# sdmiller/cpu_tsdf

Measured on AMD Instinct MI355X. Metric: integrateCloud throughput, Scene A turntable depth frames, 640x480 -> voxel grid, higher is better.
Workload: dtype f32

## Files before the change

cpu_tsdf_amd/csrc/tsdf_buffer.h:

```cpp
#pragma once

#include <hip/hip_runtime.h>
#include <stdint.h>

typedef __amdgpu_buffer_rsrc_t rsrc_t;
typedef unsigned u4 __attribute__((ext_vector_type(4)));

#ifndef TSDF_STREAM_LD_AUX
#define TSDF_STREAM_LD_AUX 2
#endif
#ifndef TSDF_STREAM_ST_AUX
#define TSDF_STREAM_ST_AUX 2
#endif

static __device__ __forceinline__ rsrc_t make_rsrc(const void *p, unsigned bytes) {
  return __builtin_amdgcn_make_buffer_rsrc(const_cast<void *>(p), (short)0, (int)bytes, 0x00020000);
}
static __device__ __forceinline__ uint32_t bload32(rsrc_t r, unsigned voff, unsigned soff) {
  return __builtin_amdgcn_raw_buffer_load_b32(r, (int)voff, (int)soff, 0);
}
static __device__ __forceinline__ u4 bload128(rsrc_t r, unsigned voff, unsigned soff) {
  return __builtin_amdgcn_raw_buffer_load_b128(r, (int)voff, (int)soff, TSDF_STREAM_LD_AUX);
}
static __device__ __forceinline__ void bstore32(rsrc_t r, unsigned voff, unsigned soff, uint32_t v) {
  __builtin_amdgcn_raw_buffer_store_b32(v, r, (int)voff, (int)soff, TSDF_STREAM_ST_AUX);
}
static __device__ __forceinline__ uint32_t bload8(rsrc_t r, unsigned voff, unsigned soff) {
  return (uint32_t)__builtin_amdgcn_raw_buffer_load_b8(r, (int)voff, (int)soff, 0) & 0xffu;
}
static __device__ __forceinline__ void bstore128(rsrc_t r, unsigned voff, unsigned soff, u4 v) {
  __builtin_amdgcn_raw_buffer_store_b128(v, r, (int)voff, (int)soff, TSDF_STREAM_ST_AUX);
}

typedef int i4_rsrc __attribute__((ext_vector_type(4)));
__device__ unsigned tsdf_struct_buffer_load_u32(i4_rsrc rsrc, int vindex, int voffset, int soffset, int aux)
    __asm("llvm.amdgcn.struct.buffer.load.i32");

static __device__ __forceinline__ i4_rsrc make_rsrc_2d(const void *p, unsigned row_bytes, unsigned rows) {
  const unsigned long long a = (unsigned long long)p;
  i4_rsrc r;
  r.x = (int)(a & 0xffffffffull);
  r.y = (int)(((a >> 32) & 0xffffull) | ((unsigned long long)(row_bytes & 0x3fffu) << 16));
  r.z = (int)rows;
  r.w = 0x00020000;
  return r;
}
```

cpu_tsdf_amd/csrc/tsdf_common.h:

```cpp
#pragma once

#include <hip/hip_runtime.h>
#include <stdint.h>
#include <cmath>
#include <string>
#include <vector>

#include "tsdf_hip.h"

struct tsdf_hip_pipeline;
struct tsdf_hip_multi;
struct tsdf_occ_state;
struct tsdf_meshpost_state;
struct tsdf_flatten_state;
struct tsdf_esdf_state;

struct tsdf_hip_volume {
  tsdf_hip_multi *multi = nullptr;
  tsdf_params p;
  int device = 0;
  int nx = 0, ny = 0, nz = 0;
  int z_begin = 0, z_end = 0;
  int z_first = 0;
  int nz_alloc = 0;
  int64_t pitch = 0;
  int levels[3] = {0, 0, 0};
  float *d = nullptr, *w = nullptr;
  uint32_t *rgb = nullptr;
  uint8_t *k8 = nullptr;
  float *cn[4] = {nullptr, nullptr, nullptr, nullptr};
  float *lab_lut = nullptr;
  float4 *lab_img = nullptr;
  float *vm = nullptr;
  int32_t *vn = nullptr;
  int expf_fused_r = 0;
  float alloc_probe_ms[8] = {-1.f, -1.f, -1.f, -1.f, -1.f, -1.f, -1.f, -1.f};
  int alloc_tried = 0, alloc_chosen = 0;
  int packed = 0;
  unsigned kmax = 0;
  int weight_by_depth = 0, weight_by_variance = 0;
  float *ctr[3] = {nullptr, nullptr, nullptr};
  std::vector<float> h_ctr[3];
  float *frame_depth = nullptr;
  uint32_t *frame_bgra = nullptr;
  char *bounce = nullptr;
  hipEvent_t bounce_ev[2] = {nullptr, nullptr};
  bool bounce_busy[2] = {false, false};
  unsigned bounce_turn = 0;
  double *cam64 = nullptr;
  tsdf_hip_pipeline *pipe = nullptr;
  int frame_staged = 0;
  uint8_t *band = nullptr;
  int band_fx = 0, band_fy = 0;
  bool band_exact = false;
  int rest_state = 0;
  uint32_t rest_bits = 0;
  unsigned long long last_implied = 0, last_read_bytes = 0;
  bool last_implied_on = false;
  uint8_t *live = nullptr;
  size_t live_cap = 0;
  uint32_t *row_iv = nullptr;
  size_t row_iv_cap = 0;
  bool ctr_increasing[3] = {false, false, false};
  unsigned long long *counter = nullptr;
  unsigned long long last_observed = 0, last_changed_bytes = 0;
  bool ref_cull = false;
  float cull_planes[24] = {0};
  int last_launch[4] = {0, 0, 0, 0};
  bool pair_pending = false;
  bool pair_fused = false;
  unsigned long long pair_first_observed = 0, pair_first_changed = 0, pair_first_implied = 0, pair_first_read = 0;
  int count_slots = 0;
  bool count_ran = false;
  hipStream_t stream = nullptr;
  float *mc_verts = nullptr;
  uint8_t *mc_rgb = nullptr;
  uint64_t *mc_cell = nullptr;
  uint64_t mc_ntri = 0;
  bool mc_valid = false;
  size_t mc_cap = 0;
  bool mc_has_rgb = false;
  uint64_t *mc_keys = nullptr, *mc_vals = nullptr;
  size_t mc_cells_cap = 0;
  uint8_t *mc_need = nullptr;
  size_t mc_need_cap = 0;
  hipEvent_t mc_ev[4] = {nullptr, nullptr, nullptr, nullptr};
  float mc_ms[3] = {0.f, 0.f, 0.f};
  uint64_t mc_ncells = 0;
  uint64_t mc_d_bytes = 0;
  bool mc_skipped = false;
  bool mc_counts_pass = false;
  bool mc_halo_vouched = false;
  hipEvent_t align_ev[2] = {nullptr, nullptr};
  uint64_t align_stats[4] = {0, 0, 0, 0};
  hipEvent_t shift_ev[2] = {nullptr, nullptr};
  bool shift_timed = false;
  uint64_t shift_stats[3] = {0, 0, 0};
  hipEvent_t merge_ev[3] = {nullptr, nullptr, nullptr};
  bool merge_timed = false;
  unsigned long long *merge_count = nullptr;
  uint64_t merge_stats[3] = {0, 0, 0};
  bool merge_count_pending = false;
  void *scratch = nullptr;
  size_t scratch_bytes = 0;
  tsdf_occ_state *occ = nullptr;
  tsdf_meshpost_state *mp = nullptr;
  tsdf_flatten_state *fl = nullptr;
  tsdf_esdf_state *esdf = nullptr;
};

void tsdf_multi_free(tsdf_hip_volume *v);
int tsdf_multi_reset(tsdf_handle h);
int tsdf_multi_synchronize(tsdf_handle h);
int tsdf_multi_set_weighting(tsdf_handle h, int by_depth, int by_variance);
int tsdf_multi_set_reference_cull(tsdf_handle h, const float planes[24]);
int tsdf_multi_variance_block(tsdf_handle h, bool down, int x0, int y0, int z0, int nx, int ny, int nz, float *M, int32_t *nsample);
int tsdf_multi_integrate(tsdf_handle h, const float *depth, const uint8_t *bgra, const float T[12], uint64_t *n_observed,
                         bool asynchronous);
int tsdf_multi_integrate_device(tsdf_handle h, const float *d_depth, const uint32_t *d_bgra, const float T[12],
                                uint64_t *n_observed);
int tsdf_multi_organize(tsdf_handle h, const float *xyz, size_t xyz_stride, const uint8_t *bgra, size_t bgra_stride, size_t n,
                        float cloud_units, int zero_nans, const double world_to_cam[12], float *depth_out, uint8_t *bgra_out,
                        uint64_t *n_valid);
int tsdf_multi_integrate_staged(tsdf_handle h, const float T[12], uint64_t *n_observed);
int tsdf_multi_last_count_detail(tsdf_handle h, uint64_t out[2]);
int tsdf_multi_last_read_detail(tsdf_handle h, uint64_t out[3]);
int tsdf_multi_block(tsdf_handle h, bool down, int x0, int y0, int z0, int nx, int ny, int nz, float *d, float *w, uint8_t *rgb);
int tsdf_multi_sample(tsdf_handle h, const float *xyz, size_t n, float *val, float *grad, float *hess, uint8_t *ok);
int tsdf_multi_align_system(tsdf_handle h, const float *xyz, size_t n, const double vol_from_src[12], float min_weight, float r_max,
                            double out[29], uint8_t *used, float *xyz_vol);
int tsdf_multi_lookup_rgb(tsdf_handle h, const float *xyz, size_t n, uint8_t *rgb, uint8_t *found);
int tsdf_multi_raycast(tsdf_handle h, const float rot[9], const float origin[3], int downsample, const double *inv, float *out);
int tsdf_multi_march(tsdf_handle h, float w_min, int color_mode, uint64_t *n_tri);
int tsdf_multi_march_fetch(tsdf_handle h, float *verts, uint8_t *rgb, uint64_t *cell);
int tsdf_multi_march_timing(tsdf_handle h, float ms[3], uint64_t *n_cells);
int tsdf_multi_march_stats(tsdf_handle h, uint64_t out[4]);
tsdf_handle tsdf_multi_first(tsdf_handle h);
tsdf_handle tsdf_multi_slab(tsdf_handle h, int k);
int tsdf_multi_march_cleanup(tsdf_handle h, float face_dist, int min_neighbors, uint64_t *n_tri);
void tsdf_multi_mesh(tsdf_handle h, const float **verts, const uint8_t **rgb, const uint64_t **cell);
int tsdf_multi_flush(tsdf_handle h);
int tsdf_multi_set_frame_pairing(tsdf_handle h, int on);
int tsdf_multi_shift(tsdf_handle h, const int32_t shift[3]);
int tsdf_multi_integrate_device2(tsdf_handle h, const float *da, const uint32_t *ca, const float TA[12], const float *planes_a, const float *db,
                                 const uint32_t *cb, const float TB[12], const float *planes_b, uint64_t *n_observed, int32_t *fused);
#define TSDF_NOT_ON_MULTI(h, what)                                                                          \
  do {                                                                                                      \
    if ((h) && (h)->multi) {                                                                                \
      tsdf_set_error(what " works on ONE slab handle; this handle is a multi-GPU set (tsdf_hip_create_multi)"); \
      return TSDF_HIP_E_UNSUPPORTED;                                                                        \
    }                                                                                                       \
  } while (0)

int tsdf_integrate_launch(tsdf_handle h, const float *d_depth, const uint32_t *d_bgra, const float T[12], bool count);
int tsdf_integrate_collect(tsdf_handle h, uint64_t *n_observed);
int tsdf_integrate_launch2(tsdf_handle h, const float *dA, const uint32_t *cA, const float TA[12], const float *planesA,
                           const float *dB, const uint32_t *cB, const float TB[12], const float *planesB, bool count, bool *fused);
int tsdf_integrate_collect2(tsdf_handle h, uint64_t n_observed[2]);

#define TSDF_MAX_SLABS 64
#define TSDF_RAY_FIN_INTS 9
unsigned tsdf_ray_list_share(int64_t n_rays, int rank, int world);
int tsdf_ray_list_begin(tsdf_handle s, const float rot[9], const float origin[3], int downsample, int rank, int world,
                        int32_t *d_list, unsigned *count);
int tsdf_ray_list_advance(tsdf_handle s, const float rot[9], const float origin[3], int downsample, int rank, int world,
                          int32_t *d_list, unsigned count, unsigned *d_incomplete);
int tsdf_ray_list_route(tsdf_handle s, const int32_t *d_list, unsigned count, int n_slab, const int *z_end,
                        unsigned *d_counters, int32_t *d_outbox, int32_t *d_finbox);
int tsdf_ray_deliver(tsdf_handle s, const int32_t *d_fin, unsigned count, float *d_out, int64_t n_pix, const double *inv);

void tsdf_set_error(const std::string &msg);
int tsdf_hip_fail(hipError_t e, const char *what, const char *file, int line);

#define TSDF_HIP_TRY(expr)                                              \
  do {                                                                  \
    hipError_t _e = (expr);                                             \
    if (_e != hipSuccess) return tsdf_hip_fail(_e, #expr, __FILE__, __LINE__); \
  } while (0)

struct TsdfDeviceScope {
  int prev = -1;
  hipError_t err;
  explicit TsdfDeviceScope(int dev) {
    err = hipGetDevice(&prev);
    if (err != hipSuccess || prev == dev)
      prev = -1;
    else
      err = hipSetDevice(dev);
  }
  ~TsdfDeviceScope() {
    if (prev >= 0) (void)hipSetDevice(prev);
  }
  TsdfDeviceScope(const TsdfDeviceScope &) = delete;
  TsdfDeviceScope &operator=(const TsdfDeviceScope &) = delete;
};
#define TSDF_ON_DEVICE(dev)          \
  TsdfDeviceScope _device_scope(dev); \
  TSDF_HIP_TRY(_device_scope.err)
int tsdf_pipeline_flush(tsdf_hip_volume *v);
#define TSDF_ENTER(h)                                  \
  TSDF_ON_DEVICE((h)->device);                         \
  if ((h)->pair_pending) {                             \
    const int _rc_flush = tsdf_pipeline_flush(h);      \
    if (_rc_flush) return _rc_flush;                   \
  }

void tsdf_build_centers(int res, float size, std::vector<float> &out, int *levels);
static inline void tsdf_lab_curve(float lut[256]) {
  for (int v = 0; v < 256; ++v) {
    float f = ((float)v / 255.);
    if (f > 0.0405)
      f = std::pow(((f + 0.055) / 1.055), 2.4);
    else
      f /= 12.92;
    f *= 100;
    lut[v] = f;
  }
}

static inline uint8_t tsdf_u8_of_float(float v) {
  const int i = (v > -2147483904.f && v < 2147483648.f) ? (int)v : (int)0x80000000;
  return (uint8_t)(i & 255);
}
static inline uint32_t tsdf_lab2rgb_host(float L, float A, float B) {
  float Y = (L + 16) / 116.;
  float X = A / 500. + Y;
  float Z = Y - (B / 200.);
  if (std::pow((double)X, 3.0) > 0.008856) X = std::pow((double)X, 3.0); else X = (X - 16 / 116.) / 7.787;
  if (std::pow((double)Y, 3.0) > 0.008856) Y = std::pow((double)Y, 3.0); else Y = (Y - 16 / 116.) / 7.787;
  if (std::pow((double)Z, 3.0) > 0.008856) Z = std::pow((double)Z, 3.0); else Z = (Z - 16 / 116.) / 7.787;
  X *= 95.047;
  Y *= 100.;
  Z *= 108.883;
  X /= 100;
  Y /= 100;
  Z /= 100;
  float rf = X * +3.2406 + Y * -1.5372 + Z * -0.4986;
  float gf = X * -0.9689 + Y * +1.8758 + Z * +0.0415;
  float bf = X * +0.0557 + Y * -0.2040 + Z * +1.0570;
  if (rf > 0.0031308) rf = 1.055 * std::pow(static_cast<double>(rf), 1. / 2.4) - 0.055; else rf *= 12.92;
  if (gf > 0.0031308) gf = 1.055 * std::pow(static_cast<double>(gf), 1. / 2.4) - 0.055; else gf *= 12.92;
  if (bf > 0.0031308) bf = 1.055 * std::pow(static_cast<double>(bf), 1. / 2.4) - 0.055; else bf *= 12.92;
  return (uint32_t)tsdf_u8_of_float(rf * 255) | ((uint32_t)tsdf_u8_of_float(gf * 255) << 8) | ((uint32_t)tsdf_u8_of_float(bf * 255) << 16);
}
void tsdf_lab2rgb_host_many(const float *L, const float *A, const float *B, size_t n, uint32_t *out);
int tsdf_lab_exact_colors(tsdf_hip_volume *v, const int64_t *d_idx, size_t n, uint32_t *host_rgb, bool write_plane);

static inline float tsdf_node_size(const tsdf_params &p, int axis) {
  const int r = p.res[0];
  const bool cubic_pow2 = r > 0 && (r & (r - 1)) == 0 && p.res[1] == r && p.res[2] == r;
  return cubic_pow2 ? p.size[0] : p.size[axis];
}
static inline float tsdf_voxel_edge(const tsdf_params &p) { return p.size[0] / p.res[0]; }
int tsdf_ensure_scratch(tsdf_hip_volume *v, size_t bytes);
int tsdf_to_host(tsdf_hip_volume *v, void *dst, const void *dev_src, size_t bytes);
int tsdf_to_device(tsdf_hip_volume *v, void *dev_dst, const void *src, size_t bytes);
bool tsdf_is_pinned_host(const void *p);
void tsdf_pipeline_destroy(tsdf_hip_volume *v);
void tsdf_occupied_release(tsdf_hip_volume *v);
void tsdf_meshpost_release(tsdf_hip_volume *v);
void tsdf_flatten_release(tsdf_hip_volume *v);
void tsdf_flatten_invalidate(tsdf_hip_volume *v);
void tsdf_occupied_invalidate(tsdf_hip_volume *v);
void tsdf_esdf_release(tsdf_hip_volume *v);
void tsdf_esdf_drop(tsdf_hip_volume *v);
void tsdf_esdf_invalidate(tsdf_hip_volume *v);
int tsdf_shift_planes(tsdf_hip_volume *v, int sx, int sy, int sz, int dz0, int dz1);
int tsdf_shift_band(tsdf_hip_volume *v, int sx, int sy, int sz);
int tsdf_shift_mark(tsdf_hip_volume *v, int which);
void tsdf_shift_clamp(const tsdf_hip_volume *v, const int32_t shift[3], int s[3]);
void tsdf_shift_count(int nx, int ny, int nz, const int s[3], uint64_t *kept, uint64_t *reset);

struct TsdfTuning {
  int rows_per_block;
  int blocks_per_cu;
  int fast_projection;
  int mc_flush_at;
  int mc_skip;
  int cull;
  int vol_chunk;
  int plain_kernel;
  int alloc_tries;
  int allin;
  int refcull_plain;
  int live_log2tx;
  int zfast;
  int fuse2;
  int implied_d;
  int pipe;
  int lab_chunk;
};
const TsdfTuning &tsdf_tuning();
int tsdf_vol_chunk();

struct PlaneView {
  const float *d, *w;
  const uint32_t *rgb;
  const uint8_t *k8;
  float wmax;
  unsigned kmax;
  int packed;
};

static inline PlaneView tsdf_plane_view(const tsdf_hip_volume *v) {
  return PlaneView{v->d, v->w, v->rgb, v->k8, v->p.max_weight, v->kmax, v->packed};
}

static __device__ __forceinline__ float tsdf_decode_w(unsigned k, float wmax) {
  const float kf = (float)k;
  return kf > wmax ? wmax : kf;
}

static __device__ __forceinline__ bool tsdf_encode_w(float w, float wmax, unsigned kmax, unsigned &k) {
  if (w == wmax) {
    k = kmax;
    return true;
  }
  if (w >= 0.f && w < (float)kmax && w == floorf(w)) {
    k = (unsigned)w;
    return true;
  }
  k = 0;
  return false;
}

static __device__ __forceinline__ float tsdf_load_w(const PlaneView &v, int64_t i) {
  if (!v.packed) return v.w[i];
  const unsigned k = v.rgb ? (v.rgb[i] >> 24) : (unsigned)v.k8[i];
  return tsdf_decode_w(k, v.wmax);
}

static __device__ __forceinline__ uint32_t tsdf_load_rgb(const PlaneView &v, int64_t i) {
  return v.rgb[i] & 0xffffffu;
}

static inline __host__ __device__ int64_t tsdf_index(int64_t pitch, int ny, int z_first, int x, int y,
                                                      int zg) {
  return ((int64_t)(zg - z_first) * ny + y) * pitch + x;
}
```

cpu_tsdf_amd/csrc/tsdf_core.hip:

```cpp
#include <math.h>

#include <string>
#include <stdlib.h>
#include <stdio.h>

#include <algorithm>
#include <thread>
#include <string.h>

#include "tsdf_common.h"
#ifdef TSDF_HIP_TEST_HOOKS
#include "tsdf_hip_test.h"
#endif

static thread_local std::string g_last_error;

void tsdf_set_error(const std::string &msg) { g_last_error = msg; }

int tsdf_hip_fail(hipError_t e, const char *what, const char *file, int line) {
  char buf[512];
  snprintf(buf, sizeof buf, "%s:%d: %s -> %s", file, line, what, hipGetErrorString(e));
  g_last_error = buf;
  (void)hipGetLastError();
  return e == hipErrorOutOfMemory ? TSDF_HIP_E_NOMEM : TSDF_HIP_E_HIP;
}

extern "C" const char *tsdf_hip_last_error(void) { return g_last_error.c_str(); }

extern "C" const char *tsdf_hip_error_string(int code) {
  switch (code) {
    case TSDF_HIP_OK: return "ok";
    case TSDF_HIP_E_INVALID: return "invalid argument";
    case TSDF_HIP_E_NOMEM: return "out of device memory";
    case TSDF_HIP_E_HIP: return "HIP runtime error";
    case TSDF_HIP_E_NODEVICE: return "no HIP device";
    case TSDF_HIP_E_UNSUPPORTED: return "unsupported";
    case TSDF_HIP_E_IO: return "file error";
    case TSDF_HIP_ALIGN_NO_POINTS: return "alignment: no point passed the gate";
    case TSDF_HIP_ALIGN_RANK_DEFICIENT: return "alignment: the cloud does not constrain all six freedoms";
  }
  return "unknown";
}

static int env_int(const char *name, int dflt) {
  const char *e = getenv(name);
  return (e && *e) ? atoi(e) : dflt;
}

static TsdfTuning &tuning_storage() {
  static TsdfTuning t = {std::max(1, env_int("TSDF_HIP_ROWS_PER_BLOCK", 64)),
                         std::max(1, env_int("TSDF_HIP_BLOCKS_PER_CU", 8)),
                         env_int("TSDF_HIP_FAST_PROJECTION", -1), env_int("TSDF_HIP_MC_FLUSH_AT", 512), env_int("TSDF_HIP_MC_SKIP", 1),
                         env_int("TSDF_HIP_CULL", 1), std::max(1, env_int("TSDF_HIP_VOL_CHUNK", 256)),
                         env_int("TSDF_HIP_PLAIN_KERNEL", 0), env_int("TSDF_HIP_ALLOC_TRIES", 3), env_int("TSDF_HIP_ALLIN", 1),
                         env_int("TSDF_HIP_REFCULL_PLAIN", 0), env_int("TSDF_HIP_LIVE_LOG2TX", 5), env_int("TSDF_HIP_ZFAST", 1), env_int("TSDF_HIP_FUSE2", 1), env_int("TSDF_HIP_IMPLIED_D", 1),
                         env_int("TSDF_HIP_PIPE", 1), std::max(1, env_int("TSDF_HIP_LAB_CHUNK", 16 << 20))};
  return t;
}

const TsdfTuning &tsdf_tuning() { return tuning_storage(); }

int tsdf_vol_chunk() {
  const int live = env_int("TSDF_HIP_VOL_CHUNK", 0);
  return live > 0 ? live : tsdf_tuning().vol_chunk;
}

#ifdef TSDF_HIP_TEST_HOOKS
extern "C" int tsdf_hip_set_tuning(const char *name, int value) {
  if (!name) return TSDF_HIP_E_INVALID;
  TsdfTuning &t = tuning_storage();
  const std::string n(name);
  if (n == "rows_per_block")
    t.rows_per_block = std::max(1, value);
  else if (n == "blocks_per_cu")
    t.blocks_per_cu = std::max(1, value);
  else if (n == "fast_projection")
    t.fast_projection = value;
  else if (n == "mc_flush_at")
    t.mc_flush_at = value;
  else if (n == "mc_skip")
    t.mc_skip = value;
  else if (n == "cull")
    t.cull = value;
  else if (n == "vol_chunk")
    t.vol_chunk = std::max(1, value);
  else if (n == "plain_kernel")
    t.plain_kernel = value;
  else if (n == "alloc_tries")
    t.alloc_tries = std::max(1, value);
  else if (n == "allin")
    t.allin = value;
  else if (n == "refcull_plain")
    t.refcull_plain = value;
  else if (n == "fuse2")
    t.fuse2 = value;
  else if (n == "implied_d")
    t.implied_d = value;
  else if (n == "pipe")
    t.pipe = value;
  else if (n == "live_log2tx")
    t.live_log2tx = value;
  else if (n == "zfast")
    t.zfast = value;
  else if (n == "lab_chunk")
    t.lab_chunk = std::max(1, value);
  else
    return TSDF_HIP_E_INVALID;
  return TSDF_HIP_OK;
}
#endif

extern "C" int tsdf_hip_abi_version(void) { return TSDF_HIP_ABI_VERSION; }

extern "C" int tsdf_hip_host_alloc(size_t bytes, void **out) {
  if (!out || !bytes) return TSDF_HIP_E_INVALID;
  *out = nullptr;
  TSDF_HIP_TRY(hipHostMalloc(out, bytes, hipHostMallocPortable));
  return TSDF_HIP_OK;
}

extern "C" int tsdf_hip_host_free(void *p) {
  if (!p) return TSDF_HIP_OK;
  TSDF_HIP_TRY(hipHostFree(p));
  return TSDF_HIP_OK;
}

extern "C" int tsdf_hip_device_count(void) {
  int n = 0;
  if (hipGetDeviceCount(&n) != hipSuccess) {
    (void)hipGetLastError();
    return 0;
  }
  return n;
}

extern "C" void tsdf_hip_default_params(tsdf_params *p) {
  memset(p, 0, sizeof *p);
  p->res[0] = p->res[1] = p->res[2] = 512;
  p->size[0] = p->size[1] = p->size[2] = 3.0f;
  p->max_dist_pos = 0.03f;
  p->max_dist_neg = 0.03f;
  p->max_weight = 100.f;
  p->min_sensor_dist = 0.3f;
  p->max_sensor_dist = 3.0f;
  p->fx = p->fy = 525.;
  p->cx = 320;
  p->cy = 240;
  p->image_width = 640;
  p->image_height = 480;
  p->integrate_color = 0;
  p->xform_order = TSDF_XFORM_PCL_SSE;
  p->z_begin = p->z_end = 0;
  p->halo = 0;
  p->device = -1;
  p->layout = TSDF_LAYOUT_AUTO;
  p->color_mode = TSDF_COLOR_RGB;
}

static int ilog2_exact(int v) {
  if (v <= 0 || (v & (v - 1))) return -1;
  int l = 0;
  while ((1 << l) < v) ++l;
  return l;
}

void tsdf_build_centers(int res, float size, std::vector<float> &out, int *levels) {
  out.resize(res);
  const int L = ilog2_exact(res);
  *levels = L;
  if (L >= 0) {
    for (int i = 0; i < res; ++i) {
      float c = 0.f;
      float s = size;
      for (int l = L - 1; l >= 0; --l) {
        const float off = s / 4;
        c = ((i >> l) & 1) ? c + off : c - off;
        s = s / 2;
      }
      out[i] = c;
    }
  } else {
    const float off = size / 2.0;
    for (int i = 0; i < res; ++i) out[i] = (float)((i + 0.5) * size / (double)res - off);
  }
}

static __global__ void __launch_bounds__(256)
k_fill_u32(uint32_t *__restrict__ p, uint32_t value, int64_t n4 ) {
  const uint4 v4 = make_uint4(value, value, value, value);
  uint4 *q = reinterpret_cast<uint4 *>(p);
  for (int64_t i = (int64_t)blockIdx.x * blockDim.x + threadIdx.x; i < n4;
       i += (int64_t)gridDim.x * blockDim.x)
    q[i] = v4;
}

static int fill_u32(tsdf_hip_volume *v, void *p, uint32_t value, int64_t n) {
  const int64_t n4 = n / 4;
  int64_t blocks = (n4 + 255) / 256;
  if (blocks > 256 * 16) blocks = 256 * 16;
  if (blocks < 1) blocks = 1;
  hipLaunchKernelGGL(k_fill_u32, dim3((unsigned)blocks), dim3(256), 0, v->stream, (uint32_t *)p, value, n4);
  TSDF_HIP_TRY(hipGetLastError());
  return TSDF_HIP_OK;
}

int tsdf_ensure_scratch(tsdf_hip_volume *v, size_t bytes) {
  if (bytes <= v->scratch_bytes) return TSDF_HIP_OK;
  if (v->scratch) {
    TSDF_HIP_TRY(hipStreamSynchronize(v->stream));
    TSDF_HIP_TRY(hipFree(v->scratch));
    v->scratch = nullptr;
    v->scratch_bytes = 0;
  }
  TSDF_HIP_TRY(hipMalloc(&v->scratch, bytes));
  v->scratch_bytes = bytes;
  return TSDF_HIP_OK;
}

void tsdf_lab2rgb_host_many(const float *L, const float *A, const float *B, size_t n, uint32_t *out) {
  const unsigned hw = std::max(1u, std::min(64u, std::thread::hardware_concurrency()));
  const unsigned nt = n < 4096 ? 1u : hw;
  auto work = [&](size_t lo, size_t hi) {
    for (size_t i = lo; i < hi; ++i) out[i] = tsdf_lab2rgb_host(L[i], A[i], B[i]);
  };
  if (nt == 1) return work(0, n);
  std::vector<std::thread> th;
  for (unsigned t = 0; t < nt; ++t) th.emplace_back(work, n * t / nt, n * (t + 1) / nt);
  for (auto &t : th) t.join();
}

static __global__ void __launch_bounds__(256)
k_lab_gather(const int64_t *__restrict__ idx, size_t n, const float *__restrict__ L, const float *__restrict__ A,
             const float *__restrict__ B, float *__restrict__ out) {
  const size_t i = (size_t)blockIdx.x * blockDim.x + threadIdx.x;
  if (i >= n) return;
  const int64_t v = idx[i];
  out[i] = v >= 0 ? L[v] : 0.f;
  out[n + i] = v >= 0 ? A[v] : 0.f;
  out[2 * n + i] = v >= 0 ? B[v] : 0.f;
}

static __global__ void __launch_bounds__(256)
k_rgb_scatter(const int64_t *__restrict__ idx, size_t n, const uint32_t *__restrict__ words, uint32_t *__restrict__ plane) {
  const size_t i = (size_t)blockIdx.x * blockDim.x + threadIdx.x;
  if (i >= n) return;
  const int64_t v = idx[i];
  if (v >= 0) plane[v] = (plane[v] & 0xff000000u) | (words[i] & 0xffffffu);
}

int tsdf_lab_exact_colors(tsdf_hip_volume *v, const int64_t *d_idx, size_t n, uint32_t *host_rgb, bool write_plane) {
  if (!n) return TSDF_HIP_OK;
  if (!v->lab_img || !v->cn[0] || !v->cn[1] || !v->cn[2]) return TSDF_HIP_E_INVALID;
  const size_t chunk = (size_t)tsdf_tuning().lab_chunk;
  float *d_lab = nullptr;
  uint32_t *d_words = nullptr;
  const size_t m = std::min(n, chunk);
  TSDF_HIP_TRY(hipMalloc(&d_lab, m * 3 * sizeof(float)));
  if (write_plane && hipMalloc(&d_words, m * sizeof(uint32_t)) != hipSuccess) {
    (void)hipFree(d_lab);
    return tsdf_hip_fail(hipErrorOutOfMemory, "hipMalloc", __FILE__, __LINE__);
  }
  std::vector<float> lab(m * 3);
  std::vector<uint32_t> words(m);
  int rc = TSDF_HIP_OK;
  for (size_t off = 0; off < n && !rc; off += chunk) {
    const size_t c = std::min(chunk, n - off);
    hipLaunchKernelGGL(k_lab_gather, dim3((unsigned)((c + 255) / 256)), dim3(256), 0, v->stream, d_idx + off, c, v->cn[0], v->cn[1],
                       v->cn[2], d_lab);
    if ((rc = tsdf_to_host(v, lab.data(), d_lab, c * 3 * sizeof(float)))) break;
    tsdf_lab2rgb_host_many(lab.data(), lab.data() + c, lab.data() + 2 * c, c, words.data());
    if (host_rgb) memcpy(host_rgb + off, words.data(), c * sizeof(uint32_t));
    if (write_plane) {
      if ((rc = tsdf_to_device(v, d_words, words.data(), c * sizeof(uint32_t)))) break;
      hipLaunchKernelGGL(k_rgb_scatter, dim3((unsigned)((c + 255) / 256)), dim3(256), 0, v->stream, d_idx + off, c, d_words, v->rgb);
      if (hipStreamSynchronize(v->stream) != hipSuccess) rc = TSDF_HIP_E_HIP;
    }
  }
  (void)hipFree(d_lab);
  if (d_words) (void)hipFree(d_words);
  return rc;
}

static const size_t kBounceChunk = 2u << 20;

static int bounce_ready(tsdf_hip_volume *v) {
  if (!v->bounce) {
    TSDF_HIP_TRY(hipHostMalloc((void **)&v->bounce, 2 * kBounceChunk, hipHostMallocDefault));
    for (int i = 0; i < 2; ++i) TSDF_HIP_TRY(hipEventCreateWithFlags(&v->bounce_ev[i], hipEventDisableTiming));
  }
  return TSDF_HIP_OK;
}

static int bounce_wait(tsdf_hip_volume *v, int slot) {
  if (v->bounce_busy[slot]) {
    TSDF_HIP_TRY(hipEventSynchronize(v->bounce_ev[slot]));
    v->bounce_busy[slot] = false;
  }
  return TSDF_HIP_OK;
}

bool tsdf_is_pinned_host(const void *p) {
  hipPointerAttribute_t attr;
  if (hipPointerGetAttributes(&attr, p) != hipSuccess) {
    (void)hipGetLastError();
    return false;
  }
  return attr.type == hipMemoryTypeHost;
}

int tsdf_to_host(tsdf_hip_volume *v, void *dst, const void *dev_src, size_t bytes) {
  if (!bytes) return TSDF_HIP_OK;
  if (bytes >= (64u << 10) && tsdf_is_pinned_host(dst)) {
    TSDF_HIP_TRY(hipMemcpyAsync(dst, dev_src, bytes, hipMemcpyDeviceToHost, v->stream));
    TSDF_HIP_TRY(hipStreamSynchronize(v->stream));
    return TSDF_HIP_OK;
  }
  int rc = bounce_ready(v);
  if (rc) return rc;
  const size_t chunks = (bytes + kBounceChunk - 1) / kBounceChunk;
  const unsigned turn = v->bounce_turn;
  v->bounce_turn += (unsigned)chunks;
  for (size_t k = 0; k <= chunks; ++k) {
    if (k < chunks) {
      const int slot = (int)((turn + k) & 1);
      if ((rc = bounce_wait(v, slot))) return rc;
      const size_t off = k * kBounceChunk, len = std::min(kBounceChunk, bytes - off);
      TSDF_HIP_TRY(hipMemcpyAsync(v->bounce + slot * kBounceChunk, (const char *)dev_src + off, len, hipMemcpyDeviceToHost,
                                  v->stream));
      TSDF_HIP_TRY(hipEventRecord(v->bounce_ev[slot], v->stream));
      v->bounce_busy[slot] = true;
    }
    if (k > 0) {
      const int slot = (int)((turn + k - 1) & 1);
      if ((rc = bounce_wait(v, slot))) return rc;
      const size_t off = (k - 1) * kBounceChunk, len = std::min(kBounceChunk, bytes - off);
      memcpy((char *)dst + off, v->bounce + slot * kBounceChunk, len);
    }
  }
  return TSDF_HIP_OK;
}

int tsdf_to_device(tsdf_hip_volume *v, void *dev_dst, const void *src, size_t bytes) {
  if (!bytes) return TSDF_HIP_OK;
  if (bytes >= (64u << 10) && tsdf_is_pinned_host(src)) {
    TSDF_HIP_TRY(hipMemcpyAsync(dev_dst, src, bytes, hipMemcpyHostToDevice, v->stream));
    TSDF_HIP_TRY(hipStreamSynchronize(v->stream));
    return TSDF_HIP_OK;
  }
  int rc = bounce_ready(v);
  if (rc) return rc;
  const size_t chunks = (bytes + kBounceChunk - 1) / kBounceChunk;
  const unsigned turn = v->bounce_turn;
  v->bounce_turn += (unsigned)chunks;
  for (size_t k = 0; k < chunks; ++k) {
    const int slot = (int)((turn + k) & 1);
    if ((rc = bounce_wait(v, slot))) return rc;
    const size_t off = k * kBounceChunk, len = std::min(kBounceChunk, bytes - off);
    memcpy(v->bounce + slot * kBounceChunk, (const char *)src + off, len);
    TSDF_HIP_TRY(hipMemcpyAsync((char *)dev_dst + off, v->bounce + slot * kBounceChunk, len, hipMemcpyHostToDevice, v->stream));
    TSDF_HIP_TRY(hipEventRecord(v->bounce_ev[slot], v->stream));
    v->bounce_busy[slot] = true;
  }
  return TSDF_HIP_OK;
}

static void free_volume(tsdf_hip_volume *v) {
  if (!v) return;
  tsdf_occupied_release(v);
  tsdf_meshpost_release(v);
  tsdf_flatten_release(v);
  tsdf_esdf_release(v);
  if (v->multi) tsdf_multi_free(v);
  TsdfDeviceScope scope(v->device);
  tsdf_pipeline_destroy(v);
  if (v->d) (void)hipFree(v->d);
  if (v->w) (void)hipFree(v->w);
  if (v->rgb) (void)hipFree(v->rgb);
  if (v->k8) (void)hipFree(v->k8);
  for (int c = 0; c < 4; ++c)
    if (v->cn[c]) (void)hipFree(v->cn[c]);
  if (v->vm) (void)hipFree(v->vm);
  if (v->vn) (void)hipFree(v->vn);
  if (v->lab_lut) (void)hipFree(v->lab_lut);
  if (v->lab_img) (void)hipFree(v->lab_img);
  for (int a = 0; a < 3; ++a)
    if (v->ctr[a]) (void)hipFree(v->ctr[a]);
  if (v->frame_depth) (void)hipFree(v->frame_depth);
  if (v->bounce) (void)hipHostFree(v->bounce);
  for (int i = 0; i < 2; ++i)
    if (v->bounce_ev[i]) (void)hipEventDestroy(v->bounce_ev[i]);
  if (v->cam64) (void)hipFree(v->cam64);
  if (v->live) (void)hipFree(v->live);
  if (v->row_iv) (void)hipFree(v->row_iv);
  if (v->band) (void)hipFree(v->band);
  if (v->counter) (void)hipFree(v->counter);
  if (v->mc_verts) (void)hipFree(v->mc_verts);
  if (v->mc_rgb) (void)hipFree(v->mc_rgb);
  if (v->mc_cell) (void)hipFree(v->mc_cell);
  if (v->mc_keys) (void)hipFree(v->mc_keys);
  if (v->mc_vals) (void)hipFree(v->mc_vals);
  if (v->mc_need) (void)hipFree(v->mc_need);
  for (int i = 0; i < 4; ++i)
    if (v->mc_ev[i]) (void)hipEventDestroy(v->mc_ev[i]);
  for (int i = 0; i < 2; ++i)
    if (v->align_ev[i]) (void)hipEventDestroy(v->align_ev[i]);
  for (int i = 0; i < 2; ++i)
    if (v->shift_ev[i]) (void)hipEventDestroy(v->shift_ev[i]);
  for (int i = 0; i < 3; ++i)
    if (v->merge_ev[i]) (void)hipEventDestroy(v->merge_ev[i]);
  if (v->merge_count) (void)hipFree(v->merge_count);
  if (v->scratch) (void)hipFree(v->scratch);
  delete v;
}

struct PlaneSet {
  float *d = nullptr, *w = nullptr;
  uint32_t *rgb = nullptr;
  uint8_t *k8 = nullptr;
};

static __global__ void __launch_bounds__(256)
k_probe_rmw(uint4 *__restrict__ a, uint4 *__restrict__ b, uint4 *__restrict__ c, int64_t n4, unsigned zero) {
  typedef unsigned v4u __attribute__((ext_vector_type(4)));
  v4u *pa = reinterpret_cast<v4u *>(a), *pb = reinterpret_cast<v4u *>(b), *pc = reinterpret_cast<v4u *>(c);
  for (int64_t i = (int64_t)blockIdx.x * blockDim.x + threadIdx.x; i < n4; i += (int64_t)gridDim.x * blockDim.x) {
    v4u x = __builtin_nontemporal_load(pa + i);
    x ^= zero;
    __builtin_nontemporal_store(x, pa + i);
    if (b) {
      v4u y = __builtin_nontemporal_load(pb + i);
      y ^= zero;
      __builtin_nontemporal_store(y, pb + i);
    }
    if (c) {
      v4u z = __builtin_nontemporal_load(pc + i);
      z ^= zero;
      __builtin_nontemporal_store(z, pc + i);
    }
  }
}

static void release_planes(PlaneSet &s) {
  if (s.d) (void)hipFree(s.d);
  if (s.w) (void)hipFree(s.w);
  if (s.rgb) (void)hipFree(s.rgb);
  if (s.k8) (void)hipFree(s.k8);
  s = PlaneSet();
}

static float probe_planes(const PlaneSet &s, int64_t n, hipStream_t stream) {
  hipEvent_t e0 = nullptr, e1 = nullptr;
  if (hipEventCreate(&e0) != hipSuccess || hipEventCreate(&e1) != hipSuccess) return -1.f;
  float ms = -1.f;
  const int64_t n4 = n / 4;
  const unsigned grid = 256u * (unsigned)tsdf_tuning().blocks_per_cu;
  bool ok = true;
  for (int pass = 0; pass < 2 && ok; ++pass) {
    ok &= hipEventRecord(e0, stream) == hipSuccess;
    hipLaunchKernelGGL(k_probe_rmw, dim3(grid), dim3(256), 0, stream, (uint4 *)s.d, (uint4 *)s.w, (uint4 *)s.rgb, n4, 0u);
    ok &= hipGetLastError() == hipSuccess;
    ok &= hipEventRecord(e1, stream) == hipSuccess;
    ok &= hipEventSynchronize(e1) == hipSuccess;
    if (ok) ok &= hipEventElapsedTime(&ms, e0, e1) == hipSuccess;
  }
  (void)hipEventDestroy(e0);
  (void)hipEventDestroy(e1);
  return ok ? ms : -1.f;
}

extern "C" int tsdf_hip_reference_cull_is_noop(const tsdf_params *p) {
  if (!p || !(p->fx > 0.0) || !(p->fy > 0.0) || p->image_width <= 0 || p->image_height <= 0) return 0;
  if (!(p->max_sensor_dist > 0.f) || !(p->max_sensor_dist < 1e15f)) return 0;
  const double W = p->image_width, H = p->image_height;
  const double th = tan(1.1 * atan(0.5 * W / p->fx)) * (1.0 - 1e-5), tv = tan(1.1 * atan(0.5 * H / p->fy)) * (1.0 - 1e-5);
  if (!(th > 0.0) || !(tv > 0.0)) return 0;
  return (p->cx + 1.0) / p->fx <= th && (W - p->cx) / p->fx <= th && (p->cy + 1.0) / p->fy <= tv && (H - p->cy) / p->fy <= tv;
}

extern "C" int tsdf_hip_reference_cull_planes(const tsdf_params *p, const double trans[16], float planes[24]) {
  if (!p || !trans || !planes) return TSDF_HIP_E_INVALID;
  struct V3 { float v[3]; };
  auto axis = [&](int col, float sign) { V3 o; for (int r = 0; r < 3; ++r) o.v[r] = sign * (float)trans[4 * r + col]; return o; };
  const V3 view = axis(2, 1.f), up = axis(1, -1.f), right = axis(0, 1.f), T = axis(3, 1.f);
  const float hfov = (float)(1.1 * 2 * fabs(atan((double)(0.5 * p->image_width / p->fx)) * 180 / M_PI));
  const float vfov = (float)(1.1 * 2 * fabs(atan((double)(0.5 * p->image_height / p->fy)) * 180 / M_PI));
  const float vrad = (float)(vfov * M_PI / 180), hrad = (float)(hfov * M_PI / 180);
  const float dist[2] = {p->max_sensor_dist, p->min_sensor_dist};
  V3 centre[2], corner[2][4];
  for (int f = 0; f < 2; ++f) {
    const float hgt = (float)(2 * tan((double)(vrad / 2)) * dist[f]), wid = (float)(2 * tan((double)(hrad / 2)) * dist[f]);
    for (int i = 0; i < 3; ++i) {
      const float c = T.v[i] + view.v[i] * dist[f], u = up.v[i] * hgt / 2, r = right.v[i] * wid / 2;
      centre[f].v[i] = c;
      corner[f][0].v[i] = c + u - r;
      corner[f][1].v[i] = c + u + r;
      corner[f][2].v[i] = c - u - r;
      corner[f][3].v[i] = c - u + r;
    }
  }
  auto minus = [](const V3 &a, const V3 &b) { V3 o; for (int i = 0; i < 3; ++i) o.v[i] = a.v[i] - b.v[i]; return o; };
  auto put = [&](int k, const V3 &e1, const V3 &e2, const V3 &through) {
    const float n[3] = {e1.v[1] * e2.v[2] - e1.v[2] * e2.v[1], e1.v[2] * e2.v[0] - e1.v[0] * e2.v[2], e1.v[0] * e2.v[1] - e1.v[1] * e2.v[0]};
    planes[4 * k] = n[0], planes[4 * k + 1] = n[1], planes[4 * k + 2] = n[2];
    planes[4 * k + 3] = -(through.v[0] * n[0] + (through.v[1] * n[1] + through.v[2] * n[2]));
  };
  const V3 a = minus(corner[0][2], T), b = minus(corner[0][3], T), c = minus(corner[0][1], T), d = minus(corner[0][0], T);
  put(0, d, a, T);
  put(1, b, c, T);
  put(2, c, d, T);
  put(3, a, b, T);
  put(4, minus(corner[0][2], corner[0][3]), minus(corner[0][1], corner[0][3]), centre[0]);
  put(5, minus(corner[1][1], corner[1][3]), minus(corner[1][2], corner[1][3]), centre[1]);
  return TSDF_HIP_OK;
}

extern "C" int tsdf_hip_create(const tsdf_params *p, tsdf_handle *out) {
  if (!p || !out) return TSDF_HIP_E_INVALID;
  *out = nullptr;
  for (int a = 0; a < 3; ++a)
    if (p->res[a] <= 0 || !(p->size[a] > 0.f)) {
      tsdf_set_error("resolution and grid size must be positive");
      return TSDF_HIP_E_INVALID;
    }
  if (p->image_width <= 0 || p->image_height <= 0 || !(p->max_dist_neg > 0.f) || p->halo < 0 ||
      (p->xform_order != TSDF_XFORM_PCL_SSE && p->xform_order != TSDF_XFORM_LEFT_TO_RIGHT) ||
      p->layout < TSDF_LAYOUT_AUTO || p->layout > TSDF_LAYOUT_PACKED ||
      p->color_mode < TSDF_COLOR_RGB || p->color_mode > TSDF_COLOR_LAB) {
    tsdf_set_error("bad image size / truncation / halo / xform_order / layout / color_mode");
    return TSDF_HIP_E_INVALID;
  }
  const bool lab = p->integrate_color && p->color_mode == TSDF_COLOR_LAB;
  const bool rgbn = (p->integrate_color && p->color_mode == TSDF_COLOR_RGB_NORMALIZED) || lab;
  if (rgbn && p->layout == TSDF_LAYOUT_PACKED) {
    tsdf_set_error("RGB_NORMALIZED / LAB colour keeps float weights: no PACKED layout");
    return TSDF_HIP_E_UNSUPPORTED;
  }
  const bool packable = !rgbn && p->max_weight >= 0.f && p->max_weight <= 255.f;
  if (p->layout == TSDF_LAYOUT_PACKED && !packable) {
    tsdf_set_error("the PACKED layout needs 0 <= max_weight <= 255");
    return TSDF_HIP_E_UNSUPPORTED;
  }
  int zb = p->z_begin, ze = p->z_end;
  if (zb == 0 && ze == 0) ze = p->res[2];
  if (zb < 0 || ze > p->res[2] || zb >= ze) {
    tsdf_set_error("z slab outside the grid");
    return TSDF_HIP_E_INVALID;
  }
  if (tsdf_hip_device_count() <= 0) {
    tsdf_set_error("no HIP device visible");
    return TSDF_HIP_E_NODEVICE;
  }
  int dev = p->device;
  if (dev < 0) TSDF_HIP_TRY(hipGetDevice(&dev));
  TSDF_ON_DEVICE(dev);

  tsdf_hip_volume *v = new tsdf_hip_volume;
  v->p = *p;
  v->p.z_begin = zb;
  v->p.z_end = ze;
  v->device = dev;
  v->nx = p->res[0];
  v->ny = p->res[1];
  v->nz = p->res[2];
  v->z_begin = zb;
  v->z_end = ze;
  v->z_first = zb - p->halo < 0 ? 0 : zb - p->halo;
  const int z_last = ze + p->halo > v->nz ? v->nz : ze + p->halo;
  v->nz_alloc = z_last - v->z_first;
  v->pitch = ((int64_t)v->nx + 3) / 4 * 4;
  const int64_t n = v->pitch * v->ny * v->nz_alloc;
  v->packed = p->layout == TSDF_LAYOUT_PACKED || (p->layout == TSDF_LAYOUT_AUTO && packable);
  v->p.layout = v->packed ? TSDF_LAYOUT_PACKED : TSDF_LAYOUT_F32W;
  v->kmax = v->packed ? (unsigned)ceilf(p->max_weight) : 0u;

  int rc = TSDF_HIP_OK;
  auto bail = [&](int code) {
    free_volume(v);
    return code;
  };
#define TRY_OR_BAIL(expr)                                                  \
  do {                                                                     \
    hipError_t _e = (expr);                                                \
    if (_e != hipSuccess) return bail(tsdf_hip_fail(_e, #expr, __FILE__, __LINE__)); \
  } while (0)
  auto alloc_planes = [&](PlaneSet &s) -> hipError_t {
    hipError_t e = hipMalloc(&s.d, n * sizeof(float));
    if (e == hipSuccess && !v->packed) e = hipMalloc(&s.w, n * sizeof(float));
    if (e == hipSuccess && p->integrate_color) e = hipMalloc(&s.rgb, n * sizeof(uint32_t));
    if (e == hipSuccess && v->packed && !p->integrate_color) e = hipMalloc(&s.k8, n);
    if (e != hipSuccess) release_planes(s);
    return e;
  };
  PlaneSet best;
  TRY_OR_BAIL(alloc_planes(best));
  {
    const size_t plane_bytes = (size_t)n * (4 + (v->packed ? 0 : 4) + (p->integrate_color ? 4 : 0) + (v->packed && !p->integrate_color ? 1 : 0));
    const int tries = plane_bytes >= ((size_t)4 << 30) ? std::max(1, tsdf_tuning().alloc_tries) : 1;
    float best_ms = tries > 1 ? probe_planes(best, n, v->stream) : -1.f;
    v->alloc_probe_ms[0] = best_ms;
    v->alloc_tried = 1;
    const double swept = (double)n * (4 + (v->packed ? 0 : 4) + (p->integrate_color ? 4 : 0));
    auto rate_tbps = [&](float ms) { return ms > 0.f ? 2.0 * swept / ((double)ms * 1e9) : 0.0; };
    for (int t = 1; t < std::min(8, 2 * tries) && best_ms > 0.f && tries > 1; ++t) {
      if (rate_tbps(best_ms) >= 5.55) break;
      if (t >= tries && rate_tbps(best_ms) >= 5.15) break;
      size_t free_b = 0, total_b = 0;
      if (hipMemGetInfo(&free_b, &total_b) != hipSuccess || free_b < plane_bytes + ((size_t)2 << 30)) break;
      PlaneSet cand;
      if (alloc_planes(cand) != hipSuccess) {
        (void)hipGetLastError();
        break;
      }
      const float ms = probe_planes(cand, n, v->stream);
      v->alloc_probe_ms[t < 8 ? t : 7] = ms;
      v->alloc_tried = t + 1;
      if (ms > 0.f && ms < best_ms) {
        release_planes(best);
        best = cand;
        best_ms = ms;
        v->alloc_chosen = t;
      } else {
        release_planes(cand);
      }
    }
  }
  v->d = best.d;
  v->w = best.w;
  v->rgb = best.rgb;
  v->k8 = best.k8;
  if (rgbn)
    for (int c = 0; c < (lab ? 3 : 4); ++c) TRY_OR_BAIL(hipMalloc(&v->cn[c], n * sizeof(float)));
  if (lab) {
    float lut[256];
    tsdf_lab_curve(lut);
    TRY_OR_BAIL(hipMalloc(&v->lab_lut, sizeof lut));
    TRY_OR_BAIL(hipMemcpy(v->lab_lut, lut, sizeof lut, hipMemcpyHostToDevice));
    TRY_OR_BAIL(hipMalloc(&v->lab_img, (size_t)p->image_width * p->image_height * sizeof(float4)));
  }
  for (int a = 0; a < 3; ++a) {
    tsdf_build_centers(p->res[a], tsdf_node_size(*p, a), v->h_ctr[a], &v->levels[a]);
    v->ctr_increasing[a] = true;
    for (size_t i = 1; i < v->h_ctr[a].size(); ++i) v->ctr_increasing[a] &= v->h_ctr[a][i - 1] < v->h_ctr[a][i];
    std::vector<float> padded(v->h_ctr[a]);
    padded.resize((size_t)p->res[a] + 4, NAN);
    TRY_OR_BAIL(hipMalloc(&v->ctr[a], padded.size() * sizeof(float)));
    TRY_OR_BAIL(hipMemcpy(v->ctr[a], padded.data(), padded.size() * sizeof(float), hipMemcpyHostToDevice));
  }
  const size_t npx = (size_t)p->image_width * p->image_height;
  TRY_OR_BAIL(hipMalloc(&v->frame_depth, 2 * npx * sizeof(float)));
  v->frame_bgra = reinterpret_cast<uint32_t *>(v->frame_depth + npx);
  {
    const double cam[4] = {p->fx, p->fy, p->cx, p->cy};
    TRY_OR_BAIL(hipMalloc(&v->cam64, sizeof cam));
    TRY_OR_BAIL(hipMemcpy(v->cam64, cam, sizeof cam, hipMemcpyHostToDevice));
  }
  v->band_fx = (v->nx + 63) / 64;
  v->band_fy = (v->ny + 3) / 4;
  TRY_OR_BAIL(hipMalloc(&v->band, (size_t)v->band_fx * v->band_fy * v->nz_alloc));
  TRY_OR_BAIL(hipMalloc(&v->counter, 4096 * sizeof(unsigned long long)));
  TRY_OR_BAIL(hipMemset(v->counter, 0, 4096 * sizeof(unsigned long long)));
#undef TRY_OR_BAIL
  rc = tsdf_hip_reset(v);
  if (rc != TSDF_HIP_OK) return bail(rc);
  *out = v;
  return TSDF_HIP_OK;
}

extern "C" int tsdf_hip_reset(tsdf_handle h) {
  if (!h) return TSDF_HIP_E_INVALID;
  if (h->multi) return tsdf_multi_reset(h);
  TSDF_ENTER(h);
  const int64_t n = h->pitch * h->ny * h->nz_alloc;
  const float minus_one = -1.f;
  uint32_t bits;
  memcpy(&bits, &minus_one, 4);
  int rc = fill_u32(h, h->d, bits, n);
  if (rc) return rc;
  if (h->w) rc = fill_u32(h, h->w, 0u, n);
  if (rc) return rc;
  if (h->k8) TSDF_HIP_TRY(hipMemsetAsync(h->k8, 0, (size_t)n, h->stream));
  if (h->rgb) rc = fill_u32(h, h->rgb, 0u, n);
  if (rc) return rc;
  for (int c = 0; c < 4 && !rc; ++c)
    if (h->cn[c]) rc = fill_u32(h, h->cn[c], 0u, n);
  if (rc) return rc;
  if (h->vm) rc = fill_u32(h, reinterpret_cast<float *>(h->vm), 0u, n);
  if (!rc && h->vn) rc = fill_u32(h, reinterpret_cast<float *>(h->vn), 0u, n);
  if (rc) return rc;
  TSDF_HIP_TRY(hipMemsetAsync(h->band, 0, (size_t)h->band_fx * h->band_fy * h->nz_alloc, h->stream));
  h->band_exact = true;
  h->rest_state = 0;
  h->frame_staged = 0;
  TSDF_HIP_TRY(hipStreamSynchronize(h->stream));
  tsdf_esdf_drop(h);
  return TSDF_HIP_OK;
}

extern "C" int tsdf_hip_destroy(tsdf_handle h) {
  if (!h) return TSDF_HIP_E_INVALID;
  TsdfDeviceScope scope(h->device);
  (void)hipStreamSynchronize(h->stream);
  free_volume(h);
  return TSDF_HIP_OK;
}

extern "C" int tsdf_hip_set_stream(tsdf_handle h, void *hip_stream) {
  if (!h) return TSDF_HIP_E_INVALID;
  TSDF_NOT_ON_MULTI(h, "tsdf_hip_set_stream (a stream belongs to one device)");
  {
    TSDF_ENTER(h);
  }
  h->stream = (hipStream_t)hip_stream;
  return TSDF_HIP_OK;
}

extern "C" int tsdf_hip_synchronize(tsdf_handle h) {
  if (!h) return TSDF_HIP_E_INVALID;
  if (h->multi) return tsdf_multi_synchronize(h);
  TSDF_ENTER(h);
  TSDF_HIP_TRY(hipStreamSynchronize(h->stream));
  return TSDF_HIP_OK;
}

extern "C" int tsdf_hip_centers(tsdf_handle h, int axis, float *out) {
  if (!h || axis < 0 || axis > 2 || !out) return TSDF_HIP_E_INVALID;
  memcpy(out, h->h_ctr[axis].data(), h->h_ctr[axis].size() * sizeof(float));
  return TSDF_HIP_OK;
}

extern "C" int tsdf_hip_alloc_probe(tsdf_handle h, float ms[8], int32_t *chosen) {
  if (!h) return 0;
  const tsdf_hip_volume *s = h->multi ? tsdf_multi_first(h) : h;
  if (ms)
    for (int i = 0; i < 8; ++i) ms[i] = s->alloc_probe_ms[i];
  if (chosen) *chosen = s->alloc_chosen;
  return s->alloc_tried;
}

extern "C" int tsdf_hip_layout(tsdf_handle h) {
  return !h ? -1 : (h->packed ? TSDF_LAYOUT_PACKED : TSDF_LAYOUT_F32W);
}

extern "C" int tsdf_hip_device_planes(tsdf_handle h, float **d, float **w, uint32_t **rgb, int64_t *pitch,
                                      int32_t *z_first, int32_t *nz_alloc) {
  if (!h) return TSDF_HIP_E_INVALID;
  TSDF_NOT_ON_MULTI(h, "tsdf_hip_device_planes");
  {
    TSDF_ENTER(h);
  }
  h->band_exact = false;
  if (d) *d = h->d;
  if (w) *w = h->w;
  if (rgb) *rgb = h->rgb;
  if (pitch) *pitch = h->pitch;
  if (z_first) *z_first = h->z_first;
  if (nz_alloc) *nz_alloc = h->nz_alloc;
  return TSDF_HIP_OK;
}

struct BlockArgs {
  int x0, y0, zl0;
  int bx, by, bz;
  int ny;
  int64_t pitch;
};

template <bool TO_BLOCK>
static __global__ void __launch_bounds__(256)
k_block_f32(BlockArgs a, float *__restrict__ vol, float *__restrict__ blk) {
  const int64_t n = (int64_t)a.bx * a.by * a.bz;
  for (int64_t i = (int64_t)blockIdx.x * blockDim.x + threadIdx.x; i < n; i += (int64_t)gridDim.x * blockDim.x) {
    const int x = (int)(i % a.bx);
    const int64_t r = i / a.bx;
    const int y = (int)(r % a.by);
    const int z = (int)(r / a.by);
    const int64_t vi = ((int64_t)(a.zl0 + z) * a.ny + (a.y0 + y)) * a.pitch + (a.x0 + x);
    if (TO_BLOCK)
      blk[i] = vol[vi];
    else
      vol[vi] = blk[i];
  }
}

template <bool TO_BLOCK>
static __global__ void __launch_bounds__(256)
k_block_w(BlockArgs a, PlaneView pv, float *__restrict__ blk, unsigned *__restrict__ bad) {
  const int64_t n = (int64_t)a.bx * a.by * a.bz;
  for (int64_t i = (int64_t)blockIdx.x * blockDim.x + threadIdx.x; i < n; i += (int64_t)gridDim.x * blockDim.x) {
    const int x = (int)(i % a.bx);
    const int64_t r = i / a.bx;
    const int y = (int)(r % a.by);
    const int z = (int)(r / a.by);
    const int64_t vi = ((int64_t)(a.zl0 + z) * a.ny + (a.y0 + y)) * a.pitch + (a.x0 + x);
    if (TO_BLOCK) {
      blk[i] = tsdf_load_w(pv, vi);
    } else if (!pv.packed) {
      const_cast<float *>(pv.w)[vi] = blk[i];
    } else {
      unsigned k;
      if (!tsdf_encode_w(blk[i], pv.wmax, pv.kmax, k)) {
        atomicAdd(bad, 1u);
      } else if (pv.rgb) {
        uint32_t *c = const_cast<uint32_t *>(pv.rgb) + vi;
// ... 360 lines not shown
```

cpu_tsdf_amd/csrc/tsdf_integrate.hip:

```cpp
#include <limits.h>
#include <string.h>
#include <math.h>

#include <algorithm>
#include <cmath>
#include <type_traits>

#include "tsdf_common.h"
#include "tsdf_div.h"
#include "tsdf_buffer.h"
#ifdef TSDF_HIP_TEST_HOOKS
#include "tsdf_hip_test.h"
#endif

#ifndef TSDF_WPE_MAX
#define TSDF_WPE_MAX 8
#endif
#ifndef TSDF_WPE_PACKED
#define TSDF_WPE_PACKED 7
#endif
#ifndef TSDF_WPE_PACKED_COLOR
#define TSDF_WPE_PACKED_COLOR 8
#endif
#ifndef TSDF_WPE_GENERAL
// ... 131 lines not shown
  if (abstop >= (0x42b00000u >> 20)) {
    if (ix == 0xff800000u) return 0.f;
    if (abstop >= (0x7f800000u >> 20)) return x + x;
    if (x > 0x1.62e42ep6f) return INFINITY;
    if (x < -0x1.9fe368p6f) return 0.f;
    if (x < -0x1.9d1d9ep6f) return 0x1p-149f;
  }
  const double N = 32., InvLn2N = 0x1.71547652b82fep+0 * N, SHIFT = 0x1.8p+52;
  const double C0 = 0x1.c6af84b912394p-5 / N / N / N, C1 = 0x1.ebfce50fac4f3p-3 / N / N, C2 = 0x1.62e42ff0c52d6p-1 / N;
  const double xd = (double)x;
  double z = InvLn2N * xd;
  double kd = z + SHIFT;
  const uint64_t ki = (uint64_t)__double_as_longlong(kd);
  kd -= SHIFT;
  const double r = fused_r ? __builtin_fma(InvLn2N, xd, -kd) : z - kd;
  const uint64_t t = k_exp2f_tab[ki & 31u] + (ki << 47);
  const double s = __longlong_as_double((long long)t);
  z = C0 * r + C1;
  const double r2 = r * r;
  double y = C2 * r + 1.;
  y = z * r2 + y;
  y = y * s;
  return (float)y;
}

static __device__ __forceinline__ bool reference_cull_keeps(const IntegrateArgs &a, float x, float y, float z) {
  bool keep = true;
#pragma unroll
  for (int k = 0; k < 6; ++k) {
    const float *pl = a.cull + 4 * k;
    keep = keep && ((x * pl[0] + y * pl[1]) + (z * pl[2] + 1.0f * pl[3]) <= 0.f);
  }
  return keep;
}

static __device__ __forceinline__ float div32_fast(float a, const Rcp32 &r) {
  const float q0 = a * r.y;
  const float r0 = __builtin_fmaf(r.nb, q0, a);
  const float q1 = __builtin_fmaf(r0, r.y, q0);
  const float r1 = __builtin_fmaf(r.nb, q1, a);
  return __builtin_fmaf(r1, r.y, q1);
}

static __device__ __forceinline__ bool numerator_ok(float v) {
  const float m = fabsf(v);
  return (m >= 0x1p-100f && m <= 0x1p40f) || __float_as_uint(v) == 0u;
}

template <bool COLOR>
static __device__ __forceinline__ void add_observation_ieee(float &d, float &w, uint32_t &rgb, float dn,
                                                            uint32_t bgra, float wmax) {
  const float wn = 1.f;
  const float wsum = w + wn;
  if (COLOR) {
    uint32_t out = 0;
#pragma unroll
    for (int ch = 0; ch < 3; ++ch) {
      const float c_old = (float)((rgb >> (8 * ch)) & 255u);
      const float c_new = (float)((bgra >> (16 - 8 * ch)) & 255u);
      const float num = w * c_old + wn * c_new;
      out |= ((uint32_t)(uint8_t)(num / wsum)) << (8 * ch);
    }
    rgb = out;
  }
  d = (d * w + dn * wn) / wsum;
  w = wsum;
  if (w > wmax) w = wmax;
}

template <bool COLOR, bool DIST = true>
static __device__ __forceinline__ void add_observation_fast(float &d, float &w, uint32_t &rgb, float dn,
                                                            uint32_t bgra, float wmax, const Rcp32 &rs, uint32_t base = 0u,
                                                            const float *hy_tab = nullptr) {
  const float wsum = w + 1.f;
  if (COLOR) {
    const float hy = hy_tab ? *hy_tab : __builtin_fmaf(0.5f, rs.y, -0.5f);
    const float t0 = __builtin_fmaf(__builtin_fmaf(w, (float)(rgb & 255u), (float)((bgra >> 16) & 255u)), rs.y, hy);
    const float t1 = __builtin_fmaf(__builtin_fmaf(w, (float)((rgb >> 8) & 255u), (float)((bgra >> 8) & 255u)), rs.y, hy);
    const float t2 = __builtin_fmaf(__builtin_fmaf(w, (float)((rgb >> 16) & 255u), (float)(bgra & 255u)), rs.y, hy);
    rgb = __builtin_amdgcn_cvt_pk_u8_f32(t0, 0u, __builtin_amdgcn_cvt_pk_u8_f32(t1, 1u, __builtin_amdgcn_cvt_pk_u8_f32(t2, 2u, base)));
  }
  if (DIST) d = div32_fast(d * w + dn, rs);
  w = wsum;
  if (w > wmax) w = wmax;
}

static __device__ __forceinline__ bool update_is_safe(float d, float w, float dn) {
  const bool w_ok = fabsf(w - 512.f) <= 512.f && __builtin_amdgcn_fractf(w) == 0.f;
  return w_ok && numerator_ok(d * w + dn);
}


struct BlockCoords {
  unsigned bx, by, bz, gdx, gdy;
};
static __device__ __forceinline__ BlockCoords tsdf_block_coords(int zfast) {
  BlockCoords c;
  c.by = blockIdx.y, c.gdy = gridDim.y;
  c.bx = zfast ? blockIdx.z : blockIdx.x;
  c.bz = zfast ? blockIdx.x : blockIdx.z;
  c.gdx = zfast ? gridDim.z : gridDim.x;
  return c;
}

static __device__ __forceinline__ void tsdf_flags_before(const IntegrateArgs &a, const BlockCoords &bc, const uint8_t *band,
                                                         uint8_t *s_bin, unsigned tid) {
  const int row0 = (int)bc.by * a.rpb * a.TY;
  const int rows = min(a.rpb * a.TY, a.ny - row0);
  const int lf = max(0, a.log2TX - 4), fxb = 1 << lf;
  const int yg0 = (a.y_abs0 + row0) >> 2, yg1 = (a.y_abs0 + row0 + max(rows, 1) - 1) >> 2;
  const int xc0 = (a.x_abs0 + (int)bc.bx * a.TX * 4) >> 6;
  const int n_fl = (yg1 - yg0 + 1) << lf;
  const int n_all = ((a.rpb * a.TY + 3) >> 2) << lf;
  for (int i = (int)tid; i < n_all; i += 256) {
    const int yg = yg0 + (i >> lf), xc = xc0 + (i & (fxb - 1));
    s_bin[i] = i < n_fl && yg < a.band_fy && xc < a.band_fx ? band[((int64_t)(a.zl0 + (int)bc.bz) * a.band_fy + yg) * a.band_fx + xc] : (uint8_t)0;
  }
}
static __device__ __forceinline__ uint64_t tsdf_quiet_passes(const IntegrateArgs &a, const uint8_t *s_bin, unsigned tid) {
  const int lane = (int)(tid & 63u), w0 = (int)(tid & ~63u);
  const int fxb = max(1, a.TX >> 4);
  const int rows_w = max(1, 64 >> a.log2TX), ncell = max(1, min(a.TX, 64) >> 4);
  const int ty0 = w0 >> a.log2TX, c0 = (w0 & (a.TX - 1)) >> 4;
  bool q = lane < a.rpb;
  if (q) {
    for (int rr = 0; rr < rows_w; ++rr)
      for (int c = 0; c < ncell; ++c) q &= s_bin[((ty0 + rr + lane * a.TY) >> 2) * fxb + c0 + c] == 0;
  }
  return __builtin_amdgcn_ballot_w64(q);
}

struct __attribute__((aligned(16))) KEntry {
  float w;
  float y;
  float hy;
  uint32_t k1;
};
static __device__ __forceinline__ KEntry tsdf_ktab_entry(const IntegrateArgs &a, unsigned k) {
  KEntry e;
  e.w = __builtin_fminf((float)k, a.wmax);
  e.y = rcp32_prepare((float)(k + 1u)).y;
  e.hy = __builtin_fmaf(0.5f, e.y, -0.5f);
  e.k1 = min(k << 24, a.kcap) + a.kinc;
  return e;
}
#define TSDF_BAND_DECL                                                                                     \
  __shared__ __attribute__((aligned(16))) uint8_t s_band_sets[4][1024];                                    \
  reinterpret_cast<u4 *>(&s_band_sets[0][0])[tid] = (u4){0u, 0u, 0u, 0u}
#define TSDF_BAND(i) s_band_sets[threadIdx.x >> 6][i]
#define TSDF_BAND_FIRST ((int)(tid & 63u))
#define TSDF_BAND_STEP 64
#define TSDF_WPE_OF(ORDER, COLOR, FASTPROJ, COUNT, PACKED, ALLIN) \
  ((ALLIN) && !(COUNT) && (PACKED) && (COLOR) && (FASTPROJ) ? TSDF_WPE_PACKED_COLOR : (ALLIN) && !(COUNT) && ((PACKED) || !(COLOR)) ? TSDF_WPE_PACKED : TSDF_WPE_GENERAL)
template <int ORDER, bool COLOR, bool FASTPROJ, bool COUNT, bool PACKED, bool ALLIN = false, bool LIVE = false>
static __global__ void __launch_bounds__(256) __attribute__((amdgpu_waves_per_eu(TSDF_WPE_OF(ORDER, COLOR, FASTPROJ, COUNT, PACKED, ALLIN) < TSDF_WPE_MAX ? TSDF_WPE_OF(ORDER, COLOR, FASTPROJ, COUNT, PACKED, ALLIN) : TSDF_WPE_MAX, TSDF_WPE_MAX)))
k_integrate(const IntegrateArgs a, float *__restrict__ D, float *__restrict__ Wt, uint32_t *__restrict__ RGB,
            uint8_t *__restrict__ K8, const float *__restrict__ depth, const double *__restrict__ cam,
            const float *__restrict__ ctrx, const float *__restrict__ ctry, const float *__restrict__ ctrz,
            unsigned long long *__restrict__ n_obs, const uint8_t *__restrict__ live, uint8_t *__restrict__ band,
            const uint32_t *__restrict__ row_iv) {
  static_assert(!(ALLIN && LIVE), "the ALLIN instance knows no row intervals");
  const BlockCoords bc = tsdf_block_coords(a.zfast);
  bool strad = false;
  if (LIVE) {
    const unsigned flag = live[bc.bx + bc.gdx * (bc.by + bc.gdy * bc.bz)];
    if (flag == 0u) return;
    strad = flag == 2u;
  }
  const unsigned tid = threadIdx.x;
  __shared__ f2 s_rcp[256];
  __shared__ f4 s_yt[256];
  constexpr bool F2 = ALLIN && FASTPROJ;
  constexpr bool LEAN_K1 = PACKED && COLOR;
  __shared__ f4 s_cx[F2 ? 256 : 1];
  __shared__ uint32_t s_iv[LIVE ? 256 : 1];
  TSDF_BAND_DECL;
  if (PACKED) {
    const KEntry e = tsdf_ktab_entry(a, tid);
    s_rcp[tid] = (f2){e.y, e.hy};
  }
  {
    const int yy = (int)bc.by * a.rpb * a.TY + (int)tid;
    {
      const float cy_ = ctry[yy < a.ny ? yy : a.ny - 1], cz_ = ctrz[a.z_global0 + (int)bc.bz];
      f4 t = {0.f, 0.f, 0.f, 0.f};
#pragma unroll
      for (int q = 0; q < 3; ++q)
        t[q] = ORDER == TSDF_XFORM_PCL_SSE ? cy_ * a.m[4 * q + 1] + (cz_ * a.m[4 * q + 2] + a.m[4 * q + 3]) : a.m[4 * q + 1] * cy_;
      s_yt[tid] = t;
    }
    if (F2) {
      const int xq_ = (int)bc.bx * a.TX + (int)(tid & (unsigned)(a.TX - 1));
      if (xq_ < a.qpr) s_cx[tid] = *reinterpret_cast<const f4 *>(ctrx + xq_ * 4);
    }
    if (LIVE && strad) s_iv[tid] = yy < a.ny ? row_iv[(int64_t)bc.bz * a.ny + yy] : 0u;
  }
  __shared__ uint8_t s_bin[PACKED ? 1024 : 1];
  if (PACKED && a.implied_d) tsdf_flags_before(a, bc, band, s_bin, tid);
  __syncthreads();
  const uint64_t quiet = PACKED && a.implied_d ? tsdf_quiet_passes(a, s_bin, tid) : 0ull;
  const int tx = (int)(tid & (unsigned)(a.TX - 1));
  const int ty = (int)(tid >> a.log2TX);
  const int xq = (int)bc.bx * a.TX + tx;
  const int zl = (int)bc.bz;
  const Rcp32 rneg = rcp32_prepare(a.neg);
  unsigned cnt = 0, chg = 0, imp = 0, rdb = 0;
  const int row0 = (int)bc.by * a.rpb * a.TY;
  const int rows = min(a.rpb * a.TY, a.ny - row0);
  const int64_t e0 = ((int64_t)(a.zl0 + zl) * a.plane_rows + row0) * a.pitch;
  const unsigned span = (unsigned)rows * (unsigned)a.pitch;
  const rsrc_t rsD = make_rsrc(D + e0, span * 4u);
  const rsrc_t rsW = make_rsrc(PACKED ? D : Wt + e0, PACKED ? 0u : span * 4u);
  const rsrc_t rsC = make_rsrc(COLOR ? RGB + e0 : (uint32_t *)D, COLOR ? span * 4u : 0u);
  const rsrc_t rsK = make_rsrc(PACKED && !COLOR ? K8 + e0 : (uint8_t *)D, PACKED && !COLOR ? span : 0u);
  const unsigned npix = (unsigned)a.W * (unsigned)a.H;
  const rsrc_t rsF = make_rsrc(depth, COLOR ? a.bgra_off + npix * 4u : npix * 4u);
  const i4_rsrc rsFi = make_rsrc_2d(depth, 4u, 0xffffffffu);
  if (xq < a.qpr) {
    const int x4 = xq * 4;
    const float cz = ctrz[a.z_global0 + zl];
    const float4 cx4 = *reinterpret_cast<const float4 *>(ctrx + x4);
    const float cxs[4] = {cx4.x, cx4.y, cx4.z, cx4.w};
    float px_[4][3], zt[3];
#pragma unroll
    for (int r = 0; r < 3; ++r) {
#pragma unroll
      for (int j = 0; j < 4; ++j) px_[j][r] = cxs[j] * a.m[4 * r];
      zt[r] = ORDER == TSDF_XFORM_PCL_SSE ? cz * a.m[4 * r + 2] + a.m[4 * r + 3] : a.m[4 * r + 2] * cz;
    }
    const unsigned voff = (unsigned)(ty * (int)a.pitch + x4) * 4u;
    const unsigned row_step = (unsigned)a.TY * (unsigned)a.pitch * 4u;
    bool pred_obs = true;
    for (int r = 0; r < a.rpb; ++r) {
      const int y = row0 + ty + r * a.TY;
      if (y >= a.ny) break;
      unsigned iv_lo = 0u, iv_len = 0u;
      if (LIVE && strad) {
        const uint32_t iv = s_iv[ty + r * a.TY];
        iv_lo = iv & 0xffffu, iv_len = iv >> 16;
        if (!((unsigned)(x4 + 3) - iv_lo < iv_len + 3u)) continue;
      }
      const unsigned soff = (unsigned)r * row_step;
      const f4 ytv = s_yt[ty + r * a.TY];
      const float yt[3] = {ytv.x, ytv.y, ytv.z};
      float px[4][3];
      if constexpr (!F2) {
        float cxr[4] = {cxs[0], cxs[1], cxs[2], cxs[3]};
#pragma unroll
        for (int j = 0; j < 4; ++j) asm volatile("" : "+v"(cxr[j]));
#pragma unroll
        for (int q = 0; q < 3; ++q)
#pragma unroll
          for (int j = 0; j < 4; ++j) px[j][q] = cxr[j] * a.m[4 * q];
      }
      auto transform = [&](int j, int q) -> float {
        if (ORDER == TSDF_XFORM_PCL_SSE) return px[j][q] + yt[q];
        return ((px[j][q] + yt[q]) + zt[q]) + a.m[4 * q + 3];
      };
      int pix[4];
      float gzs[4];
      bool any = false, lowz = false;
      if constexpr (F2) {
        asm volatile("" ::: "memory");
        project_quad_allin<ORDER>(a, a.m, cam, s_cx[tid], ytv, zt, pix, gzs);
      } else {
      unsigned amb_mask = 0;
      uint32_t margin[4] = {0u, 0u, 0u, 0u};
#pragma unroll
      for (int j = 0; j < 4; ++j) {
        const float gx = transform(j, 0), gy = transform(j, 1), gz = transform(j, 2);
        const bool in = ALLIN || (gz > a.zlo && !(gz > a.zmax) && (!LIVE || !strad || (unsigned)(x4 + j) - iv_lo < iv_len));
        gzs[j] = gz;
        if (!ALLIN) lowz |= in && gz < 0x1p-14f;
        int p;
        if (FASTPROJ) {
          bool amb;
          p = project_fast<ALLIN>(a, gx, gy, gz, amb, &margin[j]);
          if (amb && in) amb_mask |= 1u << j;
        } else {
          p = project_exact(a, cam, gx, gy, in ? gz : 1.f);
        }
        pix[j] = in ? p : -1;
        any |= in;
      }
      if (!ALLIN && !any) continue;
      if (ALLIN && FASTPROJ) {
        const uint32_t hb = __float_as_uint(a.hb_max);
        if (!(min(min(margin[0], margin[1]), min(margin[2], margin[3])) > hb)) {
#pragma unroll
          for (int j = 0; j < 4; ++j)
            if (!(margin[j] > hb)) amb_mask |= 1u << j;
        }
      }
      if (FASTPROJ && amb_mask) {
#pragma unroll
        for (int j = 0; j < 4; ++j)
          if (amb_mask >> j & 1u) pix[j] = project_exact(a, cam, transform(j, 0), transform(j, 1), transform(j, 2));
      }
      }
      constexpr bool EARLY = PACKED;
      const bool d_read = !PACKED || !(r < 64 && (quiet >> r & 1ull));
      u4 d4;
      asm volatile("" : "=v"(d4));
      u4 w4 = {0u, 0u, 0u, 0u}, c4 = {0u, 0u, 0u, 0u};
      uint32_t k4 = 0u;
      const bool ask_early = EARLY && pred_obs;
      if (ask_early) {
        if (d_read) d4 = bload128(rsD, voff, soff);
        if (COLOR) c4 = bload128(rsC, voff, soff);
        if (!COLOR) k4 = bload32(rsK, voff >> 2, soff >> 2);
        if (COUNT) rdb += (d_read ? 16u : 0u) + (COLOR ? 16u : 4u);
      }
      float zs[4];
      uint32_t cs[4] = {0u, 0u, 0u, 0u};
#pragma unroll
      for (int j = 0; j < 4; ++j) {
        if (ALLIN) {
          zs[j] = __uint_as_float(tsdf_struct_buffer_load_u32(rsFi, pix[j], 0, 0, TSDF_GATHER_AUX));
          if (COLOR) cs[j] = tsdf_struct_buffer_load_u32(rsFi, pix[j], 0, (int)a.bgra_off, TSDF_GATHER_AUX);
        } else {
          zs[j] = __uint_as_float(bload32(rsF, (unsigned)pix[j] << 2, 0u));
          if (COLOR) cs[j] = bload32(rsF, (unsigned)pix[j] << 2, a.bgra_off);
        }
      }
      float dn[4], raw[4];
      bool act[4];
      any = false;
      bool any_div = false;
#pragma unroll
      for (int j = 0; j < 4; ++j) {
        raw[j] = zs[j] - gzs[j];
        act[j] = (ALLIN || pix[j] >= 0) && raw[j] >= -a.neg;
        dn[j] = a.pos_over_neg;
        any |= act[j];
      }
      if (__builtin_fminf(__builtin_fminf(raw[0], raw[1]), __builtin_fminf(raw[2], raw[3])) <= a.pos) {
#pragma unroll
        for (int j = 0; j < 4; ++j) any_div |= act[j] && !(raw[j] > a.pos);
      }
      if (COLOR) asm volatile("" ::"v"(cs[0]), "v"(cs[1]), "v"(cs[2]), "v"(cs[3]));
      if (EARLY) {
        if (COLOR)
          asm volatile("" ::"v"(d4), "v"(c4));
        else
          asm volatile("" ::"v"(d4), "v"(k4));
      }
      const bool asked_early = ask_early;
      pred_obs = any;
      if (!any) continue;
      if (EARLY && !asked_early) {
        if (d_read) d4 = bload128(rsD, voff, soff);
        if (COLOR) c4 = bload128(rsC, voff, soff);
        if (!COLOR) k4 = bload32(rsK, voff >> 2, soff >> 2);
        if (COUNT) rdb += (d_read ? 16u : 0u) + (COLOR ? 16u : 4u);
      }
      if (any_div) {
#pragma unroll
        for (int j = 0; j < 4; ++j) dn[j] = raw[j] > a.pos ? a.pos_over_neg : div32_fast(raw[j], rneg);
      }
      if (lowz || !a.neg_in_window) {
        asm volatile("");
#pragma unroll
        for (int j = 0; j < 4; ++j)
          if (act[j] && !(raw[j] > a.pos)) dn[j] = raw[j] / a.neg;
      }
      if (!EARLY) {
        if (d_read) d4 = bload128(rsD, voff, soff);
        if (!PACKED) w4 = bload128(rsW, voff, soff);
        if (COLOR) c4 = bload128(rsC, voff, soff);
        if (PACKED && !COLOR) k4 = bload32(rsK, voff >> 2, soff >> 2);
        if (COUNT) rdb += (d_read ? 16u : 0u) + (!PACKED ? 16u : 0u) + (COLOR ? 16u : 0u) + (PACKED && !COLOR ? 4u : 0u);
      }
      uint32_t d0u[4] = {d4.x, d4.y, d4.z, d4.w};
      const uint32_t c0[4] = {c4.x, c4.y, c4.z, c4.w};
      const uint32_t w0u[4] = {w4.x, w4.y, w4.z, w4.w};
      float d0[4], w0[4];
      uint32_t kw[4];
      float dv[4], wv[4];
      uint32_t cv[4], k1[4];
      float khy[4] = {0.f, 0.f, 0.f, 0.f};
#pragma unroll
      for (int j = 0; j < 4; ++j) {
        d0[j] = __uint_as_float(d0u[j]);
        w0[j] = __uint_as_float(w0u[j]);
        kw[j] = 0u;
        k1[j] = 0u;
        if (PACKED) {
          kw[j] = COLOR ? c0[j] : (k4 << (24 - 8 * j));
          if (ALLIN) {
            w0[j] = (float)(kw[j] >> 24);
            if (COLOR) asm volatile("" : "+v"(w0[j]));
          } else {
            w0[j] = __builtin_fminf((float)(kw[j] >> 24), a.wmax);
          }
          k1[j] = LEAN_K1 ? min(kw[j], a.kcap | 0xffffffu) + a.kinc : min(kw[j] & 0xff000000u, a.kcap) + a.kinc;
        }
      }
      bool safe = true;
      if (!PACKED) {
#pragma unroll
        for (int j = 0; j < 4; ++j) safe &= !act[j] || update_is_safe(d0[j], w0[j], dn[j]);
      }
      bool d_moves = true;
      if (PACKED && a.hinge_fixed) {
        bool off_hinge = any_div;
        if (d_read) {
#pragma unroll
          for (int j = 0; j < 4; ++j) off_hinge |= (ALLIN || act[j]) && d0u[j] != __float_as_uint(a.pos_over_neg);
        } else {
#pragma unroll
          for (int j = 0; j < 4; ++j) off_hinge |= (ALLIN || act[j]) && kw[j] < 0x01000000u;
          if (ALLIN && !COLOR) off_hinge = any_div || ((k4 - 0x01010101u) & ~k4 & 0x80808080u) != 0u;
        }
        d_moves = __builtin_amdgcn_ballot_w64(off_hinge) != 0ull;
      }
      if (PACKED && !d_read && d_moves) {
#pragma unroll
        for (int j = 0; j < 4; ++j) {
          d0u[j] = kw[j] < 0x01000000u ? 0xbf800000u : __float_as_uint(a.pos_over_neg);
          d0[j] = __uint_as_float(d0u[j]);
        }
      }
      bool d_touched = false;
      if (safe) {
        Rcp32 rs[4];
#pragma unroll
        for (int j = 0; j < 4; ++j) dv[j] = d0[j], wv[j] = w0[j], cv[j] = c0[j];
        if (COLOR || !PACKED || d_moves)
#pragma unroll
        for (int j = 0; j < 4; ++j) {
          if (PACKED) {
            rs[j].nb = -(w0[j] + 1.f);
            const f2 yh = s_rcp[kw[j] >> 24];
            rs[j].y = yh.x, khy[j] = yh.y;
          } else {
            rs[j] = rcp32_prepare(w0[j] + 1.f);
          }
          add_observation_fast<COLOR, false>(dv[j], wv[j], cv[j], dn[j], cs[j], a.wmax, rs[j], COLOR ? k1[j] : 0u, PACKED ? &khy[j] : nullptr);
        }
        if (d_moves) {
          d_touched = true;
          if (any_div) TSDF_BAND(((ty + r * a.TY) >> 2) * max(1, a.TX >> 4) + (tx >> 4)) = 1;
#pragma unroll
          for (int j = 0; j < 4; ++j) dv[j] = div32_fast(d0[j] * w0[j] + dn[j], rs[j]);
          if (PACKED) {
#pragma unroll
            for (int j = 0; j < 4; ++j)
              safe &= !act[j] || ((ALLIN || a.wmax_is_int || kw[j] < (a.kmax << 24)) && __builtin_amdgcn_classf(dv[j], 0x108));
          }
        }
      }
      if (!safe) {
        d_touched = true;
        if (any_div) TSDF_BAND(((ty + r * a.TY) >> 2) * max(1, a.TX >> 4) + (tx >> 4)) = 1;
        asm volatile("");
#pragma unroll
        for (int j = 0; j < 4; ++j) {
          dv[j] = d0[j];
          wv[j] = w0[j];
          cv[j] = c0[j] & 0xffffffu;
          add_observation_ieee<COLOR>(dv[j], wv[j], cv[j], dn[j], cs[j], a.wmax);
          if (COLOR) cv[j] |= k1[j] & 0xff000000u;
        }
      }
      uint32_t diff_w = 0u, diff_c = 0u, k4n = 0u;
      uint32_t wn_u[4];
      const uint32_t c_before[4] = {c0[0], c0[1], c0[2], c0[3]};
      if (d_touched) {
        uint32_t diff_d = 0u, dn_u[4];
#pragma unroll
// ... 129 lines not shown
        asm volatile("" : "=v"(R.d4));
      R.k4 = bload32(rsK, voff >> 2, soff >> 2);
#pragma unroll
      for (int j = 0; j < 4; ++j) R.z[j] = tsdf_struct_buffer_load_u32(rsFi, pix[j], 0, 0, TSDF_GATHER_AUX);
      if (COUNT) rdb += (d_read ? 16u : 0u) + 4u;
    };

    auto consume = [&](const int r, const PipeRow &R) {
      const unsigned soff = (unsigned)r * row_step;
      const bool d_read = !(r < 64 && (quiet >> r & 1ull));
      float raw[4];
      bool act[4];
      bool any = false;
#pragma unroll
      for (int j = 0; j < 4; ++j) {
        raw[j] = __uint_as_float(R.z[j]) - R.gz[j];
        act[j] = raw[j] >= -a.neg;
        any |= act[j];
      }
      if (__builtin_amdgcn_ballot_w64(any) == 0ull) return;
      bool any_div = false;
      if (__builtin_fminf(__builtin_fminf(raw[0], raw[1]), __builtin_fminf(raw[2], raw[3])) <= a.pos) {
#pragma unroll
        for (int j = 0; j < 4; ++j) any_div |= act[j] && !(raw[j] > a.pos);
      }
      const uint32_t k4 = R.k4;
      uint32_t d0u[4] = {R.d4.x, R.d4.y, R.d4.z, R.d4.w};
      bool off_hinge = any_div;
      if (d_read) {
#pragma unroll
        for (int j = 0; j < 4; ++j) off_hinge |= d0u[j] != pbits;
      } else {
        off_hinge |= ((k4 - 0x01010101u) & ~k4 & 0x80808080u) != 0u;
      }
      const bool d_moves = __builtin_amdgcn_ballot_w64(any && off_hinge) != 0ull;
      const uint32_t km2 = a.kmax * 0x00010001u;
      const uint32_t te = ((k4 & 0x00ff00ffu) | 0x01000100u) - km2, to = (((k4 >> 8) & 0x00ff00ffu) | 0x01000100u) - km2;
      const uint32_t lt = ((~te >> 8) & 0x00010001u) | (((~to >> 8) & 0x00010001u) << 8);
      const uint32_t actb = (act[0] ? 0x00000001u : 0u) | (act[1] ? 0x00000100u : 0u) | (act[2] ? 0x00010000u : 0u) | (act[3] ? 0x01000000u : 0u);
      const uint32_t k4n = k4 + (lt & actb);
      if (d_moves) {
        float dn[4];
#pragma unroll
        for (int j = 0; j < 4; ++j) dn[j] = a.pos_over_neg;
        if (any_div) {
#pragma unroll
          for (int j = 0; j < 4; ++j) dn[j] = raw[j] > a.pos ? a.pos_over_neg : div32_fast(raw[j], rneg);
        }
        float d0[4], w0[4], dv[4];
        uint32_t kw[4];
#pragma unroll
        for (int j = 0; j < 4; ++j) {
          kw[j] = k4 << (24 - 8 * j);
          w0[j] = (float)(kw[j] >> 24);
          if (!d_read) d0u[j] = kw[j] < 0x01000000u ? 0xbf800000u : pbits;
          d0[j] = __uint_as_float(d0u[j]);
        }
        if (any_div) TSDF_BAND(((ty + r * a.TY) >> 2) * max(1, a.TX >> 4) + (tx >> 4)) = 1;
        bool safe = true;
#pragma unroll
        for (int j = 0; j < 4; ++j) {
          Rcp32 rs;
          rs.nb = -(w0[j] + 1.f);
          rs.y = s_rcp[kw[j] >> 24].x;
          dv[j] = div32_fast(d0[j] * w0[j] + dn[j], rs);
          safe &= !act[j] || __builtin_amdgcn_classf(dv[j], 0x108);
        }
        if (!safe) {
          asm volatile("");
#pragma unroll
          for (int j = 0; j < 4; ++j) {
            float wv = w0[j];
            uint32_t cv = 0u;
            dv[j] = d0[j];
            add_observation_ieee<false>(dv[j], wv, cv, dn[j], 0u, a.wmax);
          }
        }
        uint32_t diff_d = 0u, dn_u[4];
#pragma unroll
        for (int j = 0; j < 4; ++j) {
          dn_u[j] = act[j] ? __float_as_uint(dv[j]) : d0u[j];
          diff_d |= dn_u[j] ^ d0u[j];
          if (COUNT) chg += dn_u[j] != d0u[j] ? 4u : 0u;
        }
        if (diff_d) bstore128(rsD, voff, soff, (u4){dn_u[0], dn_u[1], dn_u[2], dn_u[3]});
      }
      if (COUNT) {
#pragma unroll
        for (int j = 0; j < 4; ++j) {
          cnt += act[j] ? 1u : 0u;
          imp += act[j] && !d_read ? 1u : 0u;
        }
        const uint32_t x = k4n ^ k4;
        chg += (unsigned)__popc((x | (x >> 1) | (x >> 2) | (x >> 3) | (x >> 4) | (x >> 5) | (x >> 6) | (x >> 7)) & 0x01010101u);
      }
      if (k4n != k4) bstore32(rsK, voff >> 2, soff >> 2, k4n);
    };

    PipeRow A, B;
    const int nr = rows / a.TY;
    issue(0, A);
    int r = 0;
    for (; r + 2 < nr; r += 2) {
      issue(r + 1, B);
      consume(r, A);
      issue(r + 2, A);
      consume(r + 1, B);
    }
    if (r + 1 < nr) {
      issue(r + 1, B);
      consume(r, A);
      consume(r + 1, B);
    } else {
      consume(r, A);
    }
  }
  if (band) {
    const int lf = max(0, a.log2TX - 4), fxb = 1 << lf;
    const int yg0 = (a.y_abs0 + row0) >> 2, yg1 = (a.y_abs0 + row0 + max(rows, 1) - 1) >> 2;
    const int xc0 = (a.x_abs0 + (int)bc.bx * a.TX * 4) >> 6;
    const int n_fl = (yg1 - yg0 + 1) << lf;
    for (int i = TSDF_BAND_FIRST; i < n_fl; i += TSDF_BAND_STEP) {
      const int yg = yg0 + (i >> lf), xc = xc0 + (i & (fxb - 1));
      if (TSDF_BAND(i) && yg < a.band_fy && xc < a.band_fx) band[((int64_t)(a.zl0 + zl) * a.band_fy + yg) * a.band_fx + xc] = 1;
    }
  }
  if (COUNT) {
    __shared__ unsigned s_cnt, s_chg, s_imp, s_rdb;
    if (tid == 0) s_cnt = s_chg = s_imp = s_rdb = 0;
    __syncthreads();
    if (cnt) atomicAdd(&s_cnt, cnt);
    if (chg) atomicAdd(&s_chg, chg);
    if (imp) atomicAdd(&s_imp, imp);
    if (rdb) atomicAdd(&s_rdb, rdb);
    __syncthreads();
    if (tid == 0 && (s_cnt || s_rdb)) {
      const unsigned b = bc.bx + bc.by * bc.gdx + bc.bz * bc.gdx * bc.gdy;
      if (s_cnt) atomicAdd(n_obs + (b & 1023u), (unsigned long long)s_cnt);
      if (s_chg) atomicAdd(n_obs + 1024u + (b & 1023u), (unsigned long long)s_chg);
      if (s_imp) atomicAdd(n_obs + 2048u + (b & 1023u), (unsigned long long)s_imp);
      if (s_rdb) atomicAdd(n_obs + 3072u + (b & 1023u), (unsigned long long)s_rdb);
    }
  }
}

struct PipeRowC {
  float gz[4];
  uint32_t z[4];
  uint32_t cs[4];
  u4 c4;
  u4 d4;
};

template <int ORDER, bool COUNT>
static __global__ void __launch_bounds__(256) __attribute__((amdgpu_waves_per_eu(TSDF_WPE_PIPEC < TSDF_WPE_MAX ? TSDF_WPE_PIPEC : TSDF_WPE_MAX, TSDF_WPE_MAX)))
k_integrate_pc(const IntegrateArgs a, float *__restrict__ D, uint32_t *__restrict__ RGB, const float *__restrict__ depth,
               const double *__restrict__ cam, const float *__restrict__ ctrx, const float *__restrict__ ctry,
               const float *__restrict__ ctrz, unsigned long long *__restrict__ n_obs, uint8_t *__restrict__ band) {
  const BlockCoords bc = tsdf_block_coords(a.zfast);
  const unsigned tid = threadIdx.x;
  __shared__ f2 s_rcp[256];
  __shared__ f4 s_yt[256];
  __shared__ f4 s_cx[256];
  __shared__ uint8_t s_bin[1024];
  TSDF_BAND_DECL;
  {
    const KEntry e = tsdf_ktab_entry(a, tid);
    s_rcp[tid] = (f2){e.y, e.hy};
    const int yy = (int)bc.by * a.rpb * a.TY + (int)tid;
    const float cy_ = ctry[yy < a.ny ? yy : a.ny - 1], cz_ = ctrz[a.z_global0 + (int)bc.bz];
    f4 t = {0.f, 0.f, 0.f, 0.f};
#pragma unroll
    for (int q = 0; q < 3; ++q)
      t[q] = ORDER == TSDF_XFORM_PCL_SSE ? cy_ * a.m[4 * q + 1] + (cz_ * a.m[4 * q + 2] + a.m[4 * q + 3]) : a.m[4 * q + 1] * cy_;
    s_yt[tid] = t;
    const int xq_ = (int)bc.bx * a.TX + (int)(tid & (unsigned)(a.TX - 1));
    if (xq_ < a.qpr) s_cx[tid] = *reinterpret_cast<const f4 *>(ctrx + xq_ * 4);
  }
  if (a.implied_d) tsdf_flags_before(a, bc, band, s_bin, tid);
  __syncthreads();
  const uint64_t quiet = a.implied_d ? tsdf_quiet_passes(a, s_bin, tid) : 0ull;
  const int tx = (int)(tid & (unsigned)(a.TX - 1));
  const int ty = (int)(tid >> a.log2TX);
  const int xq = (int)bc.bx * a.TX + tx;
  const int zl = (int)bc.bz;
  const Rcp32 rneg = rcp32_prepare(a.neg);
  unsigned cnt = 0, chg = 0, imp = 0, rdb = 0;
  const int row0 = (int)bc.by * a.rpb * a.TY;
  const int rows = min(a.rpb * a.TY, a.ny - row0);
  const int64_t e0 = ((int64_t)(a.zl0 + zl) * a.plane_rows + row0) * a.pitch;
  const unsigned span = (unsigned)rows * (unsigned)a.pitch;
  const rsrc_t rsD = make_rsrc(D + e0, span * 4u);
  const rsrc_t rsC = make_rsrc(RGB + e0, span * 4u);
  const i4_rsrc rsFi = make_rsrc_2d(depth, 4u, 0xffffffffu);
  const uint32_t pbits = __float_as_uint(a.pos_over_neg);
  if (xq < a.qpr) {
    const int x4 = xq * 4;
    const float cz = ctrz[a.z_global0 + zl];
    float zt[3];
#pragma unroll
    for (int q = 0; q < 3; ++q) zt[q] = ORDER == TSDF_XFORM_PCL_SSE ? cz * a.m[4 * q + 2] + a.m[4 * q + 3] : a.m[4 * q + 2] * cz;
    const unsigned voff = (unsigned)(ty * (int)a.pitch + x4) * 4u;
    const unsigned row_step = (unsigned)a.TY * (unsigned)a.pitch * 4u;
    bool obs_a = true, obs_b = true;

    auto issue = [&](const int r, PipeRowC &R, const bool pred) {
      const f4 ytv = s_yt[ty + r * a.TY];
      asm volatile("" ::: "memory");
      int pix[4];
      project_quad_allin<ORDER>(a, a.m, cam, s_cx[tid], ytv, zt, pix, R.gz);
      const unsigned soff = (unsigned)r * row_step;
      const bool d_read = !(r < 64 && (quiet >> r & 1ull));
      const unsigned offp = pred ? voff : 0x7ffffff0u;
      R.d4 = bload128(rsD, d_read ? offp : 0x7ffffff0u, soff);
      R.c4 = bload128(rsC, offp, soff);
#pragma unroll
      for (int j = 0; j < 4; ++j) {
        R.z[j] = tsdf_struct_buffer_load_u32(rsFi, pix[j], 0, 0, TSDF_GATHER_AUX);
        R.cs[j] = tsdf_struct_buffer_load_u32(rsFi, pix[j], 0, (int)a.bgra_off, TSDF_GATHER_AUX);
      }
      if (COUNT) rdb += pred ? (d_read ? 32u : 16u) : 0u;
    };

    auto consume = [&](const int r, PipeRowC &R, const bool pred, bool &obs_out) {
      const unsigned soff = (unsigned)r * row_step;
      const bool d_read = !(r < 64 && (quiet >> r & 1ull));
      float raw[4];
      bool act[4];
      bool any = false;
#pragma unroll
      for (int j = 0; j < 4; ++j) {
        raw[j] = __uint_as_float(R.z[j]) - R.gz[j];
        act[j] = raw[j] >= -a.neg;
        any |= act[j];
      }
      obs_out = any;
      if (__builtin_amdgcn_ballot_w64(any) == 0ull) return;
      if (any && !pred) {
        if (d_read) R.d4 = bload128(rsD, voff, soff);
        R.c4 = bload128(rsC, voff, soff);
        if (COUNT) rdb += d_read ? 32u : 16u;
        asm volatile("" ::"v"(R.d4), "v"(R.c4));
      }
      bool any_div = false;
      if (__builtin_fminf(__builtin_fminf(raw[0], raw[1]), __builtin_fminf(raw[2], raw[3])) <= a.pos) {
#pragma unroll
        for (int j = 0; j < 4; ++j) any_div |= act[j] && !(raw[j] > a.pos);
      }
      const uint32_t c0[4] = {R.c4.x, R.c4.y, R.c4.z, R.c4.w};
      uint32_t d0u[4] = {R.d4.x, R.d4.y, R.d4.z, R.d4.w};
      bool off_hinge = any_div;
      if (d_read) {
#pragma unroll
        for (int j = 0; j < 4; ++j) off_hinge |= d0u[j] != pbits;
      } else {
#pragma unroll
        for (int j = 0; j < 4; ++j) off_hinge |= c0[j] < 0x01000000u;
      }
      const bool d_moves = __builtin_amdgcn_ballot_w64(any && off_hinge) != 0ull;
      uint32_t cv[4];
#pragma unroll
      for (int j = 0; j < 4; ++j) {
        float w = (float)(c0[j] >> 24);
        asm volatile("" : "+v"(w));
        const uint32_t k1 = min(c0[j], a.kcap | 0xffffffu) + a.kinc;
        const f2 yh = s_rcp[c0[j] >> 24];
        Rcp32 rs;
        rs.nb = -(w + 1.f);
        rs.y = yh.x;
        const float hy = yh.y;
        float dd = 0.f;
        cv[j] = c0[j];
        add_observation_fast<true, false>(dd, w, cv[j], 0.f, R.cs[j], a.wmax, rs, k1, &hy);
      }
      if (d_moves) {
        float d0[4], dn[4], dv[4], w0[4];
#pragma unroll
        for (int j = 0; j < 4; ++j) {
          if (!d_read) d0u[j] = c0[j] < 0x01000000u ? 0xbf800000u : pbits;
          d0[j] = __uint_as_float(d0u[j]);
          dn[j] = a.pos_over_neg;
          w0[j] = (float)(c0[j] >> 24);
        }
        if (any_div) {
          TSDF_BAND(((ty + r * a.TY) >> 2) * max(1, a.TX >> 4) + (tx >> 4)) = 1;
#pragma unroll
          for (int j = 0; j < 4; ++j) dn[j] = raw[j] > a.pos ? a.pos_over_neg : div32_fast(raw[j], rneg);
        }
        bool safe = true;
#pragma unroll
        for (int j = 0; j < 4; ++j) {
          Rcp32 rs;
          rs.nb = -(w0[j] + 1.f);
          rs.y = s_rcp[c0[j] >> 24].x;
          dv[j] = div32_fast(d0[j] * w0[j] + dn[j], rs);
          safe &= !act[j] || __builtin_amdgcn_classf(dv[j], 0x108);
        }
        if (!safe) {
          asm volatile("");
#pragma unroll
          for (int j = 0; j < 4; ++j) {
            float wv = w0[j];
            dv[j] = d0[j];
            cv[j] = c0[j] & 0xffffffu;
            add_observation_ieee<true>(dv[j], wv, cv[j], dn[j], R.cs[j], a.wmax);
            cv[j] |= (min(c0[j], a.kcap | 0xffffffu) + a.kinc) & 0xff000000u;
          }
        }
        uint32_t diff_d = 0u, dn_u[4];
#pragma unroll
        for (int j = 0; j < 4; ++j) {
          dn_u[j] = act[j] ? __float_as_uint(dv[j]) : d0u[j];
          diff_d |= dn_u[j] ^ d0u[j];
          if (COUNT) chg += dn_u[j] != d0u[j] ? 4u : 0u;
        }
        if (diff_d) bstore128(rsD, voff, soff, (u4){dn_u[0], dn_u[1], dn_u[2], dn_u[3]});
      }
      uint32_t diff_c = 0u;
#pragma unroll
      for (int j = 0; j < 4; ++j) {
        cv[j] = act[j] ? cv[j] : c0[j];
        diff_c |= cv[j] ^ c0[j];
        if (COUNT) {
          cnt += act[j] ? 1u : 0u;
          imp += act[j] && !d_read ? 1u : 0u;
          chg += cv[j] != c0[j] ? 4u : 0u;
        }
      }
      if (diff_c) bstore128(rsC, voff, soff, (u4){cv[0], cv[1], cv[2], cv[3]});
    };

    PipeRowC A, B;
    const int nr = rows / a.TY;
    issue(0, A, true);
    int r = 0;
    for (; r + 2 < nr; r += 2) {
      const bool pb = obs_b;
      issue(r + 1, B, pb);
      const bool pa = obs_a;
      consume(r, A, pa, obs_a);
      const bool pa2 = obs_a;
      issue(r + 2, A, pa2);
      consume(r + 1, B, pb, obs_b);
    }
    if (r + 1 < nr) {
      const bool pb = obs_b;
      issue(r + 1, B, pb);
      const bool pa = obs_a;
      consume(r, A, pa, obs_a);
      consume(r + 1, B, pb, obs_b);
    } else {
      const bool pa = obs_a;
      consume(r, A, pa, obs_a);
    }
  }
  if (band) {
    const int lf = max(0, a.log2TX - 4), fxb = 1 << lf;
    const int yg0 = (a.y_abs0 + row0) >> 2, yg1 = (a.y_abs0 + row0 + max(rows, 1) - 1) >> 2;
    const int xc0 = (a.x_abs0 + (int)bc.bx * a.TX * 4) >> 6;
    const int n_fl = (yg1 - yg0 + 1) << lf;
    for (int i = TSDF_BAND_FIRST; i < n_fl; i += TSDF_BAND_STEP) {
      const int yg = yg0 + (i >> lf), xc = xc0 + (i & (fxb - 1));
      if (TSDF_BAND(i) && yg < a.band_fy && xc < a.band_fx) band[((int64_t)(a.zl0 + zl) * a.band_fy + yg) * a.band_fx + xc] = 1;
    }
  }
  if (COUNT) {
    __shared__ unsigned s_cnt, s_chg, s_imp, s_rdb;
    if (tid == 0) s_cnt = s_chg = s_imp = s_rdb = 0;
    __syncthreads();
    if (cnt) atomicAdd(&s_cnt, cnt);
    if (chg) atomicAdd(&s_chg, chg);
    if (imp) atomicAdd(&s_imp, imp);
    if (rdb) atomicAdd(&s_rdb, rdb);
    __syncthreads();
    if (tid == 0 && (s_cnt || s_rdb)) {
      const unsigned b = bc.bx + bc.by * bc.gdx + bc.bz * bc.gdx * bc.gdy;
      if (s_cnt) atomicAdd(n_obs + (b & 1023u), (unsigned long long)s_cnt);
      if (s_chg) atomicAdd(n_obs + 1024u + (b & 1023u), (unsigned long long)s_chg);
      if (s_imp) atomicAdd(n_obs + 2048u + (b & 1023u), (unsigned long long)s_imp);
      if (s_rdb) atomicAdd(n_obs + 3072u + (b & 1023u), (unsigned long long)s_rdb);
    }
  }
}

struct Frame2 {
  float m[12];
  unsigned bgra_off;
};

template <int ORDER, bool COLOR, bool COUNT>
static __global__ void __launch_bounds__(256) __attribute__((amdgpu_waves_per_eu(TSDF_WPE_K2, TSDF_WPE_MAX)))
k_integrate2(const IntegrateArgs a, const Frame2 fb, float *__restrict__ D, uint32_t *__restrict__ RGB, uint8_t *__restrict__ K8,
             const float *__restrict__ depthA, const float *__restrict__ depthB, const double *__restrict__ cam,
             const float *__restrict__ ctrx, const float *__restrict__ ctry, const float *__restrict__ ctrz,
             unsigned long long *__restrict__ n_obs, uint8_t *__restrict__ band) {
  const unsigned tid = threadIdx.x;
  const BlockCoords bc = tsdf_block_coords(a.zfast);
  __shared__ KEntry s_tab[256];
  __shared__ f4 s_ytA[256], s_ytB[256];
  __shared__ f4 s_cx[256];
  TSDF_BAND_DECL;
  s_tab[tid] = tsdf_ktab_entry(a, tid);
  {
    const int yy = (int)bc.by * a.rpb * a.TY + (int)tid;
    const float cy_ = ctry[yy < a.ny ? yy : a.ny - 1], cz_ = ctrz[a.z_global0 + (int)bc.bz];
    f4 tA = {0.f, 0.f, 0.f, 0.f}, tB = {0.f, 0.f, 0.f, 0.f};
#pragma unroll
    for (int q = 0; q < 3; ++q) {
      tA[q] = ORDER == TSDF_XFORM_PCL_SSE ? cy_ * a.m[4 * q + 1] + (cz_ * a.m[4 * q + 2] + a.m[4 * q + 3]) : a.m[4 * q + 1] * cy_;
      tB[q] = ORDER == TSDF_XFORM_PCL_SSE ? cy_ * fb.m[4 * q + 1] + (cz_ * fb.m[4 * q + 2] + fb.m[4 * q + 3]) : fb.m[4 * q + 1] * cy_;
    }
    s_ytA[tid] = tA, s_ytB[tid] = tB;
    const int xq_ = (int)bc.bx * a.TX + (int)(tid & (unsigned)(a.TX - 1));
    if (xq_ < a.qpr) s_cx[tid] = *reinterpret_cast<const f4 *>(ctrx + xq_ * 4);
  }
  __syncthreads();
  const int tx = (int)(tid & (unsigned)(a.TX - 1));
  const int ty = (int)(tid >> a.log2TX);
  const int xq = (int)bc.bx * a.TX + tx;
  const int zl = (int)bc.bz;
  const Rcp32 rneg = rcp32_prepare(a.neg);
  unsigned cnt = 0, chg = 0, cntA = 0, cntB = 0, rdb = 0;
  const int row0 = (int)bc.by * a.rpb * a.TY;
  const int rows = min(a.rpb * a.TY, a.ny - row0);
  const int64_t e0 = ((int64_t)(a.zl0 + zl) * a.plane_rows + row0) * a.pitch;
  const unsigned span = (unsigned)rows * (unsigned)a.pitch;
  const rsrc_t rsD = make_rsrc(D + e0, span * 4u);
  const rsrc_t rsC = make_rsrc(COLOR ? RGB + e0 : (uint32_t *)D, COLOR ? span * 4u : 0u);
  const rsrc_t rsK = make_rsrc(!COLOR ? K8 + e0 : (uint8_t *)D, !COLOR ? span : 0u);
  const i4_rsrc rsFA = make_rsrc_2d(depthA, 4u, 0xffffffffu), rsFB = make_rsrc_2d(depthB, 4u, 0xffffffffu);
  const uint32_t hinge_bits = __float_as_uint(a.pos_over_neg);
  if (xq < a.qpr) {
    const int x4 = xq * 4;
    const float cz = ctrz[a.z_global0 + zl];
    float ztA[3], ztB[3];
#pragma unroll
    for (int q = 0; q < 3; ++q) ztA[q] = a.m[4 * q + 2] * cz, ztB[q] = fb.m[4 * q + 2] * cz;
    const unsigned voff = (unsigned)(ty * (int)a.pitch + x4) * 4u;
    const unsigned row_step = (unsigned)a.TY * (unsigned)a.pitch * 4u;
    struct RowLoads {
      float zsA[4], zsB[4], gzA[4], gzB[4];
      uint32_t csA[4], csB[4];
      u4 d4, c4;
      uint32_t k4;
    };
    auto issue = [&](int r, RowLoads &L) {
      const unsigned soff = (unsigned)r * row_step;
      int pixA[4], pixB[4];
      asm volatile("" ::: "memory");
      project_quad_allin<ORDER>(a, a.m, cam, s_cx[tid], s_ytA[ty + r * a.TY], ztA, pixA, L.gzA);
      project_quad_allin<ORDER>(a, fb.m, cam, s_cx[tid], s_ytB[ty + r * a.TY], ztB, pixB, L.gzB);
#pragma unroll
      for (int j = 0; j < 4; ++j) {
        L.zsA[j] = __uint_as_float(tsdf_struct_buffer_load_u32(rsFA, pixA[j], 0, 0, TSDF_GATHER_AUX));
        L.csA[j] = COLOR ? tsdf_struct_buffer_load_u32(rsFA, pixA[j], 0, (int)a.bgra_off, TSDF_GATHER_AUX) : 0u;
      }
#pragma unroll
      for (int j = 0; j < 4; ++j) {
        L.zsB[j] = __uint_as_float(tsdf_struct_buffer_load_u32(rsFB, pixB[j], 0, 0, TSDF_GATHER_AUX));
        L.csB[j] = COLOR ? tsdf_struct_buffer_load_u32(rsFB, pixB[j], 0, (int)fb.bgra_off, TSDF_GATHER_AUX) : 0u;
      }
      L.d4 = bload128(rsD, voff, soff);
      L.c4 = (u4){0u, 0u, 0u, 0u};
      L.k4 = 0u;
      if (COLOR) L.c4 = bload128(rsC, voff, soff);
      if (!COLOR) L.k4 = bload32(rsK, voff >> 2, soff >> 2);
      if (COUNT) rdb += 16u + (COLOR ? 16u : 4u);
    };
    auto retire = [&](int r, const RowLoads &L) {
      const unsigned soff = (unsigned)r * row_step;
      if (COLOR)
        asm volatile("" ::"v"(L.csA[0]), "v"(L.csA[1]), "v"(L.csA[2]), "v"(L.csA[3]), "v"(L.csB[0]), "v"(L.csB[1]), "v"(L.csB[2]),
                     "v"(L.csB[3]), "v"(L.d4), "v"(L.c4));
      else
        asm volatile("" ::"v"(L.d4), "v"(L.k4));
      auto finish = [&](const float (&zs)[4], const float (&gzs)[4], float (&dn)[4]) -> unsigned {
        unsigned obs = 0;
        float raw[4];
#pragma unroll
        for (int j = 0; j < 4; ++j) {
          raw[j] = zs[j] - gzs[j];
          const bool act = raw[j] >= -a.neg;
          dn[j] = a.pos_over_neg;
          obs |= act ? 1u << j : 0u;
          obs |= act && !(raw[j] > a.pos) ? 16u : 0u;
        }
        if (obs & 16u) {
#pragma unroll
          for (int j = 0; j < 4; ++j) dn[j] = raw[j] > a.pos ? a.pos_over_neg : div32_fast(raw[j], rneg);
        }
        if (!a.neg_in_window) {
          asm volatile("");
#pragma unroll
          for (int j = 0; j < 4; ++j)
            if ((obs >> j & 1u) && !(raw[j] > a.pos)) dn[j] = raw[j] / a.neg;
        }
        return obs;
      };
      float dnA[4], dnB[4];
      const unsigned obsA = finish(L.zsA, L.gzA, dnA);
      const unsigned obsB = finish(L.zsB, L.gzB, dnB);
      if (!((obsA | obsB) & 15u)) return;
      const u4 d4 = L.d4, c4 = L.c4;
      const uint32_t k4 = L.k4;
      const uint32_t d0u[4] = {d4.x, d4.y, d4.z, d4.w};
      const uint32_t c0[4] = {c4.x, c4.y, c4.z, c4.w};
      uint32_t du[4], kw[4];
#pragma unroll
      for (int j = 0; j < 4; ++j) {
        kw[j] = COLOR ? c0[j] : ((k4 << (24 - 8 * j)) & 0xff000000u);
        du[j] = d0u[j];
      }
      auto apply = [&](unsigned obs, const float (&dn)[4], const uint32_t (&cs)[4]) {
        if (!(obs & 15u)) return;
        const bool any_div = (obs & 16u) != 0u;
        float d0[4], w0[4], dv[4], wv[4], ky[4], khy[4];
        uint32_t cv[4], k1[4];
#pragma unroll
        for (int j = 0; j < 4; ++j) {
          d0[j] = __uint_as_float(du[j]);
          const KEntry e = s_tab[kw[j] >> 24];
          w0[j] = e.w, ky[j] = e.y, khy[j] = e.hy, k1[j] = e.k1;
        }
        bool d_moves = true;
        if (a.hinge_fixed) {
          bool off_hinge = any_div;
#pragma unroll
          for (int j = 0; j < 4; ++j) off_hinge |= du[j] != hinge_bits;
          d_moves = __builtin_amdgcn_ballot_w64(off_hinge) != 0ull;
        }
        bool safe = true, d_touched = false;
        {
          Rcp32 rs[4];
#pragma unroll
          for (int j = 0; j < 4; ++j) {
            dv[j] = d0[j];
            wv[j] = w0[j];
            cv[j] = kw[j];
            rs[j].nb = -(w0[j] + 1.f);
            rs[j].y = ky[j];
            add_observation_fast<COLOR, false>(dv[j], wv[j], cv[j], dn[j], cs[j], a.wmax, rs[j], COLOR ? k1[j] : 0u, &khy[j]);
          }
          if (d_moves) {
            d_touched = true;
            if (any_div) TSDF_BAND(((ty + r * a.TY) >> 2) * max(1, a.TX >> 4) + (tx >> 4)) = 1;
#pragma unroll
            for (int j = 0; j < 4; ++j) dv[j] = div32_fast(d0[j] * w0[j] + dn[j], rs[j]);
#pragma unroll
            for (int j = 0; j < 4; ++j) safe &= !(obs >> j & 1u) || __builtin_amdgcn_classf(dv[j], 0x108);
          }
        }
        if (!safe) {
          asm volatile("");
#pragma unroll
          for (int j = 0; j < 4; ++j) {
            dv[j] = d0[j];
            wv[j] = w0[j];
            cv[j] = kw[j] & 0xffffffu;
            add_observation_ieee<COLOR>(dv[j], wv[j], cv[j], dn[j], cs[j], a.wmax);
            if (COLOR) cv[j] |= k1[j];
          }
        }
#pragma unroll
        for (int j = 0; j < 4; ++j) {
          const bool act = (obs >> j & 1u) != 0u;
          if (d_touched) du[j] = act ? __float_as_uint(dv[j]) : du[j];
          kw[j] = act ? (COLOR ? cv[j] : k1[j]) : kw[j];
        }
      };
      apply(obsA, dnA, L.csA);
      apply(obsB, dnB, L.csB);
      uint32_t diff_d = 0u, diff_c = 0u, k4n = 0u;
#pragma unroll
      for (int j = 0; j < 4; ++j) {
        diff_d |= du[j] ^ d0u[j];
        if (COLOR) diff_c |= kw[j] ^ c0[j];
        if (!COLOR) k4n |= (kw[j] & 0xff000000u) >> (24 - 8 * j);
        cnt += ((obsA | obsB) >> j & 1u);
        if (COUNT) cntA += (obsA >> j & 1u), cntB += (obsB >> j & 1u);
        if (COUNT) chg += (du[j] != d0u[j] ? 4u : 0u) + (COLOR && kw[j] != c0[j] ? 4u : 0u);
      }
      if (COUNT && !COLOR) chg += (unsigned)__popc(((k4n ^ k4) | ((k4n ^ k4) >> 1) | ((k4n ^ k4) >> 2) | ((k4n ^ k4) >> 3) |
                                                   ((k4n ^ k4) >> 4) | ((k4n ^ k4) >> 5) | ((k4n ^ k4) >> 6) | ((k4n ^ k4) >> 7)) & 0x01010101u);
      if (diff_d) bstore128(rsD, voff, soff, (u4){du[0], du[1], du[2], du[3]});
      if (COLOR && diff_c) bstore128(rsC, voff, soff, (u4){kw[0], kw[1], kw[2], kw[3]});
      if (!COLOR && k4n != k4) bstore32(rsK, voff >> 2, soff >> 2, k4n);
    };
    const int left = a.ny - row0 - ty;
    const int nrows = left <= 0 ? 0 : min(a.rpb, (left + a.TY - 1) / a.TY);
    for (int r = 0; r < nrows; ++r) {
      RowLoads L;
      issue(r, L);
      retire(r, L);
    }
  }
  if (band) {
    const int lf = max(0, a.log2TX - 4), fxb = 1 << lf;
    const int yg0 = (a.y_abs0 + row0) >> 2, yg1 = (a.y_abs0 + row0 + max(rows, 1) - 1) >> 2;
    const int xc0 = (a.x_abs0 + (int)bc.bx * a.TX * 4) >> 6;
    const int n_fl = (yg1 - yg0 + 1) << lf;
    for (int i = TSDF_BAND_FIRST; i < n_fl; i += TSDF_BAND_STEP) {
      const int yg = yg0 + (i >> lf), xc = xc0 + (i & (fxb - 1));
      if (TSDF_BAND(i) && yg < a.band_fy && xc < a.band_fx) band[((int64_t)(a.zl0 + zl) * a.band_fy + yg) * a.band_fx + xc] = 1;
    }
  }
  if (COUNT) {
    __shared__ unsigned s_cnt, s_chg, s_cntA, s_cntB, s_rdb;
    if (tid == 0) s_cnt = s_chg = s_cntA = s_cntB = s_rdb = 0;
    __syncthreads();
    if (cnt) atomicAdd(&s_cnt, cnt);
    if (chg) atomicAdd(&s_chg, chg);
    if (cntA) atomicAdd(&s_cntA, cntA);
    if (cntB) atomicAdd(&s_cntB, cntB);
// ... 514 lines not shown

template <class Args>
static void fill_camera(Args &c, const tsdf_params &p, const float T[12]) {
  for (int i = 0; i < 12; ++i) c.m[i] = T[i];
  c.fx = p.fx, c.fy = p.fy, c.cx = p.cx, c.cy = p.cy;
  c.zlo = p.min_sensor_dist > 0 ? p.min_sensor_dist : 0;
  c.zmax = p.max_sensor_dist;
  c.W = p.image_width, c.H = p.image_height;
}

static bool fast_projection_ok(const IntegrateHost &a, bool color, bool force = false) {
  const int knob = tsdf_tuning().fast_projection;
  (void)color;
  const bool want = force || knob != 0;
  return want && std::isfinite(a.band_u) && std::isfinite(a.band_v) &&
         a.band_u < 0.05f && a.band_v < 0.05f && fabs(a.fx) < 1e6 && fabs(a.fy) < 1e6 && a.a.W < (1 << 23) &&
         a.a.H < (1 << 23);
}

static int implied_distances(tsdf_handle h, const IntegrateArgs &a, bool flags_kept) {
  if (!flags_kept) return 0;
  uint32_t bits;
  memcpy(&bits, &a.pos_over_neg, 4);
  if (!(h->packed && a.hinge_fixed && h->kmax >= 1u))
    h->rest_state = 2;
  else if (h->rest_state == 0)
    h->rest_state = 1, h->rest_bits = bits;
  else if (h->rest_state == 1 && h->rest_bits != bits)
    h->rest_state = 2;
  return h->rest_state == 1 && tsdf_tuning().implied_d ? 1 : 0;
}


static bool observable_index_box(const tsdf_hip_volume *h, const float T[12], int lo[3], int hi[3], bool *empty) {
  const tsdf_params &p = h->p;
  *empty = false;
  if (!(p.max_sensor_dist > 0.f)) {
    *empty = true;
    return true;
  }
  if (!std::isfinite(p.max_sensor_dist) || !(p.fx > 0) || !(p.fy > 0) || !std::isfinite(p.cx) || !std::isfinite(p.cy))
    return false;
  double A[9], t[3];
  for (int r = 0; r < 3; ++r) {
    for (int c = 0; c < 3; ++c) A[3 * r + c] = T[4 * r + c];
    t[r] = T[4 * r + 3];
  }
  const double det = A[0] * (A[4] * A[8] - A[5] * A[7]) - A[1] * (A[3] * A[8] - A[5] * A[6]) + A[2] * (A[3] * A[7] - A[4] * A[6]);
  double scale = 0;
  for (int i = 0; i < 9; ++i) scale = std::max(scale, fabs(A[i]));
  if (!std::isfinite(det) || !(fabs(det) > 1e-9 * scale * scale * scale)) return false;
  const double inv[9] = {(A[4] * A[8] - A[5] * A[7]) / det, (A[2] * A[7] - A[1] * A[8]) / det, (A[1] * A[5] - A[2] * A[4]) / det,
                         (A[5] * A[6] - A[3] * A[8]) / det, (A[0] * A[8] - A[2] * A[6]) / det, (A[2] * A[3] - A[0] * A[5]) / det,
                         (A[3] * A[7] - A[4] * A[6]) / det, (A[1] * A[6] - A[0] * A[7]) / det, (A[0] * A[4] - A[1] * A[3]) / det};
  const double zf = (double)p.max_sensor_dist * (1.0 + 1e-6) + 1e-9;
  double mn[3] = {1e300, 1e300, 1e300}, mx[3] = {-1e300, -1e300, -1e300}, big = 0;
  for (int k = 0; k < 5; ++k) {
    double g[3] = {0, 0, 0};
    if (k < 4) {
      const double u = (k & 1) ? p.image_width + 1.0 : -2.0, v = (k & 2) ? p.image_height + 1.0 : -2.0;
      g[0] = (u - p.cx) / p.fx * zf;
      g[1] = (v - p.cy) / p.fy * zf;
      g[2] = zf;
    }
    for (int r = 0; r < 3; ++r) {
      const double c = inv[3 * r] * (g[0] - t[0]) + inv[3 * r + 1] * (g[1] - t[1]) + inv[3 * r + 2] * (g[2] - t[2]);
      if (!std::isfinite(c)) return false;
      mn[r] = std::min(mn[r], c);
      mx[r] = std::max(mx[r], c);
      big = std::max(big, fabs(c));
    }
  }
  for (int a = 0; a < 3; ++a) {
    const std::vector<float> &ctr = h->h_ctr[a];
    const int n = (int)ctr.size();
    const double margin = 2.0 * (double)p.size[a] / (double)p.res[a] + 1e-5 * (big + fabs((double)p.size[a]));
    if (mx[a] + margin < (double)ctr.front() || mn[a] - margin > (double)ctr.back()) *empty = true;
    lo[a] = (int)(std::lower_bound(ctr.begin(), ctr.end(), (float)(mn[a] - margin)) - ctr.begin());
    hi[a] = (int)(std::upper_bound(ctr.begin(), ctr.end(), (float)(mx[a] + margin)) - ctr.begin()) - 1;
    if (lo[a] > 0) --lo[a];
    if (hi[a] < n - 1) ++hi[a];
    if (lo[a] > hi[a]) *empty = true;
  }
  return true;
}

static bool zlo_margin_ok(const float T[12], const tsdf_hip_volume *h) {
  double big = 0, zmin = 1e300;
  for (int k = 0; k < 8; ++k) {
    const double x = h->h_ctr[0][(k & 1) ? h->nx - 1 : 0], y = h->h_ctr[1][(k & 2) ? h->ny - 1 : 0],
                 z = h->h_ctr[2][(k & 4) ? h->z_end - 1 : h->z_begin];
    for (int r = 0; r < 3; ++r) {
      const double g = fabs((double)T[4 * r] * x) + fabs((double)T[4 * r + 1] * y) + fabs((double)T[4 * r + 2] * z) + fabs((double)T[4 * r + 3]);
      big = std::max(big, g);
    }
    zmin = std::min(zmin, (double)T[8] * x + (double)T[9] * y + (double)T[10] * z + (double)T[11]);
  }
  const double err = 8.0 * 6e-8 * big;
  const double f = std::max(fabs(h->p.fx), fabs(h->p.fy));
  return err < 1e-4 && zmin > 0.05 && f * err * (1.0 + big / zmin) / zmin < 0.05;
}

static bool reference_cull_keeps_whole_slab(const tsdf_hip_volume *h, const float *planes) {
  for (int k = 0; k < 6; ++k) {
    const float *pl = planes + 4 * k;
    double worst = -1e300, mag = 0;
    for (int c = 0; c < 8; ++c) {
      const double x = h->h_ctr[0][(c & 1) ? h->nx - 1 : 0], y = h->h_ctr[1][(c & 2) ? h->ny - 1 : 0],
                   z = h->h_ctr[2][(c & 4) ? h->z_end - 1 : h->z_begin];
      const double v = (double)pl[0] * x + (double)pl[1] * y + (double)pl[2] * z + (double)pl[3];
      if (!std::isfinite(v)) return false;
      worst = std::max(worst, v);
      mag = std::max(mag, fabs((double)pl[0] * x) + fabs((double)pl[1] * y) + fabs((double)pl[2] * z) + fabs((double)pl[3]));
    }
    if (!(worst + 8.0 * 4.0 * 5.97e-8 * mag <= 0.0)) return false;
  }
  return true;
}

static bool row_intervals_usable(const tsdf_hip_volume *h, bool planes) {
  if (h->pitch > 0xfff0 || !h->ctr_increasing[0]) return false;
  if (planes)
    for (int i = 0; i < 24; ++i)
      if (!(fabsf(h->cull_planes[i]) < 1e30f)) return false;
  return true;
}

static bool slab_all_inside(const tsdf_hip_volume *h, const float T[12]) {
  const tsdf_params &p = h->p;
  bool all_inside = true;
  for (int k = 0; k < 8 && all_inside; ++k) {
    const double x = h->h_ctr[0][(k & 1) ? h->nx - 1 : 0], y = h->h_ctr[1][(k & 2) ? h->ny - 1 : 0],
                 z = h->h_ctr[2][(k & 4) ? h->z_end - 1 : h->z_begin];
    double g[3];
    for (int r = 0; r < 3; ++r) g[r] = (double)T[4 * r] * x + (double)T[4 * r + 1] * y + (double)T[4 * r + 2] * z + (double)T[4 * r + 3];
    const double u = p.fx * g[0] / g[2] + p.cx, v = p.fy * g[1] / g[2] + p.cy;
    const double zlo = p.min_sensor_dist > 0 ? p.min_sensor_dist : 0;
    all_inside = g[2] > zlo + 1e-3 && g[2] > 1e-3 && g[2] < p.max_sensor_dist - 1e-3 && u > 1 && u < p.image_width - 2 && v > 1 &&
                 v < p.image_height - 2;
  }
  return all_inside;
}

static bool frame_bgra_offset(const tsdf_params &p, const float *d_depth, const uint32_t *d_bgra, unsigned *off) {
  *off = 0;
  if (!p.integrate_color) return true;
  const size_t npx = (size_t)p.image_width * p.image_height;
  const char *zd = (const char *)d_depth, *cb = (const char *)d_bgra;
  if (!(cb >= zd + npx * 4 && (size_t)(cb - zd) + npx * 4 < (1ull << 31))) return false;
  *off = (unsigned)(cb - zd);
  return true;
}

static int stage_frame(tsdf_handle h, const float **d_depth, const uint32_t *d_bgra, unsigned *bgra_off) {
  if (frame_bgra_offset(h->p, *d_depth, d_bgra, bgra_off)) return TSDF_HIP_OK;
  const size_t npx = (size_t)h->p.image_width * h->p.image_height;
  h->frame_staged = 0;
  if (*d_depth != h->frame_depth)
    TSDF_HIP_TRY(hipMemcpyAsync(h->frame_depth, *d_depth, npx * 4, hipMemcpyDeviceToDevice, h->stream));
  if (d_bgra != h->frame_bgra)
    TSDF_HIP_TRY(hipMemcpyAsync(h->frame_bgra, d_bgra, npx * 4, hipMemcpyDeviceToDevice, h->stream));
  *d_depth = h->frame_depth;
  *bgra_off = (unsigned)(npx * 4);
  return TSDF_HIP_OK;
}

static int zfast_for(const tsdf_params &p, unsigned gx) {
  const size_t frame_bytes = (size_t)p.image_width * p.image_height * (p.integrate_color ? 8 : 4);
  return tsdf_tuning().zfast < 0 ? (frame_bytes > (3u << 20) && gx <= 65535u) : (tsdf_tuning().zfast != 0 && gx <= 65535u);
}

static uint8_t *band_flags_for(tsdf_handle h, const IntegrateArgs &a) {
  uint8_t *band = h->band_exact && ((a.rpb * a.TY) & 3) == 0 && (a.y_abs0 & 3) == 0 ? h->band : nullptr;
  if (!band) h->band_exact = false;
  return band;
}

static bool pipelined_rows_apply(tsdf_handle h, const IntegrateArgs &a, bool color, bool fastproj, bool allin, bool live) {
  return (tsdf_tuning().pipe & (color ? 2 : 1)) && fastproj && allin && !live && h->packed && a.hinge_fixed && a.neg_in_window &&
         a.ny % a.TY == 0;
}

static int launch_plain_family(tsdf_handle h, const IntegrateArgs &a, unsigned gz, int plain_mode, const float *d_depth,
                               const uint32_t *d_bgra, const float T[12], bool count) {
  const tsdf_params &p = h->p;
  if (plain_mode && ((h->packed && plain_mode != 3) || h->cn[0])) {
    tsdf_set_error("weight_by_depth needs the F32W layout and TSDF_COLOR_RGB");
    return TSDF_HIP_E_UNSUPPORTED;
  }
  if (count) TSDF_HIP_TRY(hipMemsetAsync(h->counter, 0, 1024 * sizeof(unsigned long long), h->stream));
  const bool pose_ok = pose_is_finite(T);
  if (pose_ok) {
    const dim3 grid((unsigned)((h->pitch + 255) / 256), (unsigned)h->ny, gz), block(256);
    if (grid.y > 65535u) {
      tsdf_set_error("grid too large for one launch");
      return TSDF_HIP_E_UNSUPPORTED;
    }
    unsigned long long *n_obs = count ? h->counter : nullptr;
    const bool sse = p.xform_order == TSDF_XFORM_PCL_SSE, by_depth = plain_mode == 2;
    if (plain_mode) {
      float *vm = h->weight_by_variance ? h->vm : nullptr;
      int32_t *vn = h->weight_by_variance ? h->vn : nullptr;
      with_consts(
          [&](auto SSE, auto COLOR, auto BY_DEPTH, auto PACKED) {
            if constexpr (!(BY_DEPTH && PACKED))
              hipLaunchKernelGGL((k_integrate_plain<xform_order_of(SSE), COLOR, BY_DEPTH, PACKED>), grid, block, 0, h->stream, a,
                                 h->d, h->w, h->rgb, h->k8, vm, vn, d_depth, d_bgra, h->cam64, h->ctr[0], h->ctr[1], h->ctr[2], n_obs);
          },
          sse, p.integrate_color != 0, by_depth, !by_depth && h->packed);
    } else if (h->lab_img) {
      const int npx = p.image_width * p.image_height;
      hipLaunchKernelGGL(k_lab_image, dim3((unsigned)((npx + 255) / 256)), dim3(256), 0, h->stream, d_bgra, h->lab_lut, h->lab_img, npx);
      with_consts(
          [&](auto SSE) {
            hipLaunchKernelGGL((k_integrate_lab<xform_order_of(SSE)>), grid, block, 0, h->stream, a, h->d, h->w, h->rgb, h->cn[0],
                               h->cn[1], h->cn[2], d_depth, h->lab_img, h->cam64, h->ctr[0], h->ctr[1], h->ctr[2], n_obs);
          },
          sse);
    } else {
      with_consts(
          [&](auto SSE) {
            hipLaunchKernelGGL((k_integrate_rgbn<xform_order_of(SSE)>), grid, block, 0, h->stream, a, h->d, h->w, h->rgb, h->cn[0],
                               h->cn[1], h->cn[2], h->cn[3], d_depth, d_bgra, h->cam64, h->ctr[0], h->ctr[1], h->ctr[2], n_obs);
          },
          sse);
    }
    TSDF_HIP_TRY(hipGetLastError());
  }
  h->count_slots = count ? 1024 : 0;
  h->count_ran = pose_ok;
  return TSDF_HIP_OK;
}

struct LaunchPlan {
  IntegrateArgs a;
  unsigned gx, gy, gz;
  float *D, *Wt;
  uint32_t *RGB;
  uint8_t *K8;
  const float *ctrx, *ctry;
  const uint8_t *live;
  bool nothing_observable;
};

static LaunchPlan whole_slab_plan(tsdf_handle h, const IntegrateHost &hh) {
  LaunchPlan pl;
  const IntegrateArgs &a = pl.a = hh.a;
  pl.gx = (unsigned)((a.qpr + a.TX - 1) / a.TX);
  pl.gy = (unsigned)((a.ny + a.rpb * a.TY - 1) / (a.rpb * a.TY));
  pl.gz = (unsigned)hh.planes;
  pl.D = h->d, pl.Wt = h->w, pl.RGB = h->rgb, pl.K8 = h->k8;
  pl.ctrx = h->ctr[0], pl.ctry = h->ctr[1];
  pl.live = nullptr;
  pl.nothing_observable = false;
  return pl;
}

struct LaunchKind {
  bool all_inside;
  bool allin;
  bool live;
};

static LaunchKind launch_kind(tsdf_handle h, const float T[12], const IntegrateArgs &a, bool rc, bool rc_rows) {
  LaunchKind k = {false, false, false};
  if (tsdf_tuning().cull) {
    k.all_inside = tsdf_tuning().cull != 2 && slab_all_inside(h, T);
    k.allin = k.all_inside && tsdf_tuning().allin && (h->nx & 3) == 0 && zlo_margin_ok(T, h) &&
              (!h->packed || (a.wmax_is_int && (float)h->kmax == h->p.max_weight));
  }
  if (rc) k.allin = false;
  k.live = (tsdf_tuning().cull && !k.all_inside && row_intervals_usable(h, false)) || rc_rows;
  return k;
}

static void narrow_live_blocks(LaunchPlan &pl) {
  IntegrateArgs &a = pl.a;
  const int ltx = std::max(4, std::min(8, tsdf_tuning().live_log2tx));
  if (a.TX <= (1 << ltx)) return;
  a.TX = 1 << ltx, a.log2TX = ltx, a.TY = 256 >> ltx;
  a.rpb = std::max(1, std::min(2 * tsdf_tuning().rows_per_block, 64) / a.TY);
  pl.gx = (unsigned)((a.qpr + a.TX - 1) / a.TX);
  pl.gy = (unsigned)((a.ny + a.rpb * a.TY - 1) / (a.rpb * a.TY));
}

static void shrink_to_index_box(tsdf_handle h, const float T[12], LaunchPlan &pl) {
  IntegrateArgs &a = pl.a;
  int lo[3], hi[3];
  bool empty = false;
  if (!observable_index_box(h, T, lo, hi, &empty)) return;
  lo[2] = std::max(lo[2], h->z_begin);
  hi[2] = std::min(hi[2], h->z_end - 1);
  if (empty || lo[2] > hi[2]) {
    pl.nothing_observable = true;
    return;
  }
  const int bxv = a.TX * 4, byr = a.rpb * a.TY;
  const int bx0 = lo[0] / bxv, bx1 = hi[0] / bxv, by0 = lo[1] / byr, by1 = hi[1] / byr;
  const int x_off = bx0 * bxv, y_off = by0 * byr, z_off = lo[2] - h->z_begin;
  const int64_t e_off = (int64_t)y_off * h->pitch + x_off;
  pl.D += e_off;
  if (pl.Wt) pl.Wt += e_off;
  if (pl.RGB) pl.RGB += e_off;
  if (pl.K8) pl.K8 += e_off;
  pl.ctrx += x_off;
  pl.ctry += y_off;
  a.qpr -= x_off / 4;
  a.ny -= y_off;
  a.x_abs0 = x_off;
  a.y_abs0 = y_off;
  a.z_global0 += z_off;
  a.zl0 += z_off;
  pl.gx = (unsigned)(bx1 - bx0 + 1);
  pl.gy = (unsigned)(by1 - by0 + 1);
  pl.gz = (unsigned)(hi[2] - lo[2] + 1);
}

static int grow_live_scratch(tsdf_handle h, size_t nb, size_t nrows) {
  if (nb <= h->live_cap && nrows <= h->row_iv_cap) return TSDF_HIP_OK;
  TSDF_HIP_TRY(hipStreamSynchronize(h->stream));
  if (nb > h->live_cap) {
    if (h->live) TSDF_HIP_TRY(hipFree(h->live));
    h->live = nullptr, h->live_cap = 0;
    TSDF_HIP_TRY(hipMalloc(&h->live, nb));
    h->live_cap = nb;
  }
  if (nrows > h->row_iv_cap) {
    if (h->row_iv) TSDF_HIP_TRY(hipFree(h->row_iv));
    h->row_iv = nullptr, h->row_iv_cap = 0;
    TSDF_HIP_TRY(hipMalloc(&h->row_iv, nrows * sizeof(uint32_t)));
    h->row_iv_cap = nrows;
  }
  return TSDF_HIP_OK;
}

static int launch_rows_and_cull(tsdf_handle h, const float T[12], bool rc_rows, LaunchPlan &pl) {
  IntegrateArgs &a = pl.a;
  const int rows = a.ny = std::min(a.ny, (int)pl.gy * a.rpb * a.TY);
  CullArgs c;
  fill_camera(c, h->p, T);
  c.nx = h->nx - (int)(pl.ctrx - h->ctr[0]), c.ny = rows, c.z_global0 = a.z_global0;
  c.bx_vox = a.TX * 4, c.by_rows = a.rpb * a.TY;
  c.gx = (int)pl.gx, c.gy = (int)pl.gy, c.gz = (int)pl.gz;
  RowArgs ra;
  fill_camera(ra, h->p, T);
  ra.nx = std::min(c.nx, (int)pl.gx * a.TX * 4), ra.ny = rows, ra.nz = (int)pl.gz, ra.z_global0 = a.z_global0;
  ra.rc = rc_rows ? 1 : 0;
  for (int i = 0; i < 24; ++i) ra.cull[i] = rc_rows ? h->cull_planes[i] : 0.f;
  const size_t nb = (size_t)pl.gx * pl.gy * pl.gz, nrows = (size_t)rows * pl.gz;
  if (const int e = grow_live_scratch(h, nb, nrows)) return e;
  const dim3 row_grid((unsigned)((nrows + 255) / 256)), block(256);
  if (ra.nx <= TSDF_ROWS_LDS_NX)
    hipLaunchKernelGGL(k_rows<true>, row_grid, block, 0, h->stream, ra, pl.ctrx, pl.ctry, h->ctr[2], h->row_iv);
  else
    hipLaunchKernelGGL(k_rows<false>, row_grid, block, 0, h->stream, ra, pl.ctrx, pl.ctry, h->ctr[2], h->row_iv);
  hipLaunchKernelGGL(k_cull, dim3((unsigned)((nb + 255) / 256)), block, 0, h->stream, c, pl.ctrx, pl.ctry, h->ctr[2], h->row_iv, h->live);
  TSDF_HIP_TRY(hipGetLastError());
  pl.live = h->live;
  return TSDF_HIP_OK;
}

static int plan_live(tsdf_handle h, const float T[12], bool all_inside, bool rc_rows, LaunchPlan &pl) {
  if (!all_inside) narrow_live_blocks(pl);
  if (tsdf_tuning().cull && !all_inside) shrink_to_index_box(h, T, pl);
  if (pl.gy > 65535u) {
    tsdf_set_error("grid too large for one launch");
    return TSDF_HIP_E_UNSUPPORTED;
  }
  return pl.nothing_observable ? TSDF_HIP_OK : launch_rows_and_cull(h, T, rc_rows, pl);
}

static void dispatch_fast(tsdf_handle h, const LaunchPlan &pl, const float *d_depth, bool count, bool fastproj, bool allin,
                          bool pipe, uint8_t *band_arg) {
  const IntegrateArgs &a = pl.a;
  const dim3 grid(a.zfast ? pl.gz : pl.gx, pl.gy, a.zfast ? pl.gx : pl.gz), block(256);
  const bool sse = h->p.xform_order == TSDF_XFORM_PCL_SSE, color = h->p.integrate_color != 0;
  if (pipe) {
    with_consts(
        [&](auto SSE, auto COUNT) {
          if (color)
            hipLaunchKernelGGL((k_integrate_pc<xform_order_of(SSE), COUNT>), grid, block, 0, h->stream, a, pl.D, pl.RGB, d_depth,
                               h->cam64, pl.ctrx, pl.ctry, h->ctr[2], h->counter, band_arg);
          else
            hipLaunchKernelGGL((k_integrate_p<xform_order_of(SSE), COUNT>), grid, block, 0, h->stream, a, pl.D, pl.K8, d_depth,
                               h->cam64, pl.ctrx, pl.ctry, h->ctr[2], h->counter, band_arg);
        },
        sse, count);
    return;
  }
  with_consts(
      [&](auto SSE, auto COLOR, auto FASTPROJ, auto COUNT, auto PACKED, auto ALLIN, auto LIVE) {
        if constexpr (!(ALLIN && (!FASTPROJ || LIVE)))
          hipLaunchKernelGGL((k_integrate<xform_order_of(SSE), COLOR, FASTPROJ, COUNT, PACKED, ALLIN, LIVE>), grid, block, 0,
                             h->stream, a, pl.D, pl.Wt, pl.RGB, pl.K8, d_depth, h->cam64, pl.ctrx, pl.ctry, h->ctr[2], h->counter,
                             pl.live, band_arg, h->row_iv);
      },
      sse, color, fastproj, count, h->packed, allin, pl.live != nullptr);
}

static int validate_launch(tsdf_handle h, const LaunchPlan &pl, const uint32_t *d_bgra) {
  if (pl.gy > 65535u || pl.gz > 65535u) {
    tsdf_set_error("grid too large for one launch");
    return TSDF_HIP_E_UNSUPPORTED;
  }
  if (h->p.integrate_color && !d_bgra) {
    tsdf_set_error("integrate_color is set but no colour image was given");
    return TSDF_HIP_E_INVALID;
  }
  if (h->weight_by_variance && (!h->vm || !h->vn || h->packed || h->cn[0])) {
    tsdf_set_error("weight_by_variance_ (hpp:203-204) needs the per-voxel M_ / nsample_ planes: F32W layout, TSDF_COLOR_RGB");
    return TSDF_HIP_E_UNSUPPORTED;
  }
  return TSDF_HIP_OK;
}

int tsdf_integrate_launch(tsdf_handle h, const float *d_depth, const uint32_t *d_bgra, const float T[12], bool count) {
  h->count_slots = 0;
  h->count_ran = false;
  const IntegrateHost hh = make_args(h, T);
  LaunchPlan pl = whole_slab_plan(h, hh);
  IntegrateArgs &a = pl.a;
  if (const int e = validate_launch(h, pl, d_bgra)) return e;
  const bool rc = h->ref_cull && !reference_cull_keeps_whole_slab(h, h->cull_planes);
  const bool rc_rows = rc && !h->cn[0] && !tsdf_tuning().refcull_plain && row_intervals_usable(h, true);
  const int plain_mode = h->weight_by_depth ? 2 : h->weight_by_variance ? 4 : (rc && !rc_rows && !h->cn[0]) ? 3 : (tsdf_tuning().plain_kernel && !h->packed && !h->cn[0] ? 1 : 0);
  a.ref_cull = rc ? 1 : 0;
  if (plain_mode || h->cn[0]) {
    h->band_exact = false;
    return launch_plain_family(h, a, pl.gz, plain_mode, d_depth, d_bgra, T, count);
  }
  if (const int e = stage_frame(h, &d_depth, d_bgra, &a.bgra_off)) return e;
  const LaunchKind kind = launch_kind(h, T, a, rc, rc_rows);
  if (kind.live)
    if (const int e = plan_live(h, T, kind.all_inside, rc_rows, pl)) return e;
  if (count) TSDF_HIP_TRY(hipMemsetAsync(h->counter, 0, 4096 * sizeof(unsigned long long), h->stream));
  const bool pose_ok = pose_is_finite(T);
  const bool fastproj = fast_projection_ok(hh, h->p.integrate_color != 0);
  h->last_launch[0] = h->last_launch[1] = h->last_launch[2] = h->last_launch[3] = 0;
  uint8_t *band_arg = band_flags_for(h, a);
  a.implied_d = implied_distances(h, a, band_arg != nullptr);
  h->last_implied_on = a.implied_d != 0;
  if (pose_ok && !pl.nothing_observable) {
    const bool live = pl.live != nullptr, allin = fastproj && kind.allin && !live;
    const bool pipe = pipelined_rows_apply(h, a, h->p.integrate_color != 0, fastproj, kind.allin, live);
    a.zfast = zfast_for(h->p, pl.gx);
    h->last_launch[0] = (allin ? 1 : 0) | (pipe ? 0x100 : 0);
    h->last_launch[1] = fastproj;
    h->last_launch[2] = live ? (rc_rows ? 2 : 1) : 0;
    h->last_launch[3] = (int)std::min<uint64_t>((uint64_t)pl.gx * pl.gy * pl.gz, 0x7fffffffu);
    dispatch_fast(h, pl, d_depth, count, fastproj, allin, pipe, band_arg);
    TSDF_HIP_TRY(hipGetLastError());
  }
  h->count_slots = count ? 4096 : 0;
  h->count_ran = pose_ok && !pl.nothing_observable;
  return TSDF_HIP_OK;
}

int tsdf_integrate_collect(tsdf_handle h, uint64_t *n_observed) {
  if (!h->count_slots) {
    tsdf_set_error("tsdf_integrate_collect without a counting launch");
    return TSDF_HIP_E_INVALID;
  }
  unsigned long long c[4096];
  const int slots = h->count_slots;
  TSDF_HIP_TRY(hipMemcpyAsync(c, h->counter, (size_t)slots * sizeof(unsigned long long), hipMemcpyDeviceToHost, h->stream));
  TSDF_HIP_TRY(hipStreamSynchronize(h->stream));
  unsigned long long sum = 0, changed = 0, implied = 0, read_bytes = 0;
  for (int i = 0; i < 1024; ++i) sum += c[i];
  for (int i = 1024; i < slots && i < 2048; ++i) changed += c[i];
  for (int i = 2048; i < slots && i < 3072; ++i) implied += c[i];
  for (int i = 3072; i < slots; ++i) read_bytes += c[i];
  h->last_observed = h->count_ran ? sum : 0;
  h->last_changed_bytes = h->count_ran ? changed : 0;
  h->last_implied = h->count_ran ? implied : 0;
  h->last_read_bytes = h->count_ran ? read_bytes : 0;
  h->count_slots = 0;
  if (n_observed) *n_observed = h->last_observed;
  return TSDF_HIP_OK;
}

static int launch_integrate(tsdf_handle h, const float *d_depth, const uint32_t *d_bgra, const float T[12],
                            uint64_t *n_observed) {
  const int rc = tsdf_integrate_launch(h, d_depth, d_bgra, T, n_observed != nullptr);
  if (rc || !n_observed) return rc;
  return tsdf_integrate_collect(h, n_observed);
}

static bool fusable_pose(tsdf_handle h, const IntegrateHost &hh, const float T[12], const float *planes) {
  if (!pose_is_finite(T)) return false;
  if (planes && !reference_cull_keeps_whole_slab(h, planes)) return false;
  return slab_all_inside(h, T) && zlo_margin_ok(T, h) && fast_projection_ok(hh, h->p.integrate_color != 0);
}

int tsdf_integrate_launch2(tsdf_handle h, const float *dA, const uint32_t *cA, const float TA[12], const float *planesA_,
                           const float *dB, const uint32_t *cB, const float TB[12], const float *planesB_, bool count, bool *fused) {
  float planes_copy[2][24];
  const float *planesA = nullptr, *planesB = nullptr;
  if (planesA_) memcpy(planes_copy[0], planesA_, sizeof planes_copy[0]), planesA = planes_copy[0];
  if (planesB_) memcpy(planes_copy[1], planesB_, sizeof planes_copy[1]), planesB = planes_copy[1];
  const tsdf_params &p = h->p;
  const bool color = p.integrate_color != 0;
  if (color && (!cA || !cB)) {
    tsdf_set_error("integrate_color is set but no colour image was given");
    return TSDF_HIP_E_INVALID;
  }
  const IntegrateHost hh = make_args(h, TA);
  LaunchPlan pl = whole_slab_plan(h, hh);
  IntegrateArgs &a = pl.a;
  Frame2 fb;
  for (int i = 0; i < 12; ++i) fb.m[i] = TB[i];
  const bool pipe_wins = !color && tsdf_tuning().fuse2 == 1 && pipelined_rows_apply(h, a, color, true, true, false);
  const bool ok = tsdf_tuning().fuse2 && !pipe_wins && tsdf_tuning().cull == 1 && tsdf_tuning().allin && h->packed && !h->cn[0] && !h->weight_by_depth &&
                  !h->weight_by_variance && !tsdf_tuning().plain_kernel && (h->nx & 3) == 0 && a.wmax_is_int && (float)h->kmax == p.max_weight &&
                  pl.gy <= 65535u && pl.gz <= 65535u && pl.gz > 0 && frame_bgra_offset(p, dA, cA, &a.bgra_off) &&
                  frame_bgra_offset(p, dB, cB, &fb.bgra_off) && fusable_pose(h, hh, TA, planesA) && fusable_pose(h, hh, TB, planesB);
  if (fused) *fused = ok;
  if (!ok) {
    int rc = tsdf_hip_set_reference_cull(h, planesA);
    if (!rc) rc = tsdf_integrate_launch(h, dA, cA, TA, count);
    if (!rc && count) {
      uint64_t n = 0;
      rc = tsdf_integrate_collect(h, &n);
      h->pair_first_observed = n, h->pair_first_changed = h->last_changed_bytes, h->pair_first_implied = h->last_implied;
      h->pair_first_read = h->last_read_bytes;
    }
    if (!rc) rc = tsdf_hip_set_reference_cull(h, planesB);
    if (!rc) rc = tsdf_integrate_launch(h, dB, cB, TB, count);
    h->pair_fused = false;
    return rc;
  }
  h->ref_cull = planesB != nullptr;
  for (int i = 0; i < 24; ++i) h->cull_planes[i] = planesB ? planesB[i] : 0.f;
  h->count_slots = 0;
  h->count_ran = false;
  if (count) TSDF_HIP_TRY(hipMemsetAsync(h->counter, 0, 3072 * sizeof(unsigned long long), h->stream));
  uint8_t *band_arg = band_flags_for(h, a);
  (void)implied_distances(h, a, band_arg != nullptr);
  a.implied_d = 0;
  h->last_implied_on = false;
  h->last_launch[0] = 2, h->last_launch[1] = 1, h->last_launch[2] = 0;
  h->last_launch[3] = (int)std::min<uint64_t>((uint64_t)pl.gx * pl.gy * pl.gz, 0x7fffffffu);
  a.zfast = zfast_for(p, pl.gx);
  const dim3 grid(a.zfast ? pl.gz : pl.gx, pl.gy, a.zfast ? pl.gx : pl.gz), block(256);
  with_consts(
      [&](auto SSE, auto COLOR, auto COUNT) {
        hipLaunchKernelGGL((k_integrate2<xform_order_of(SSE), COLOR, COUNT>), grid, block, 0, h->stream, a, fb, h->d, h->rgb, h->k8,
                           dA, dB, h->cam64, h->ctr[0], h->ctr[1], h->ctr[2], h->counter, band_arg);
      },
      p.xform_order == TSDF_XFORM_PCL_SSE, color, count);
  TSDF_HIP_TRY(hipGetLastError());
  h->count_slots = count ? 3072 : 0;
  h->count_ran = true;
  h->pair_fused = true;
  return TSDF_HIP_OK;
}

int tsdf_integrate_collect2(tsdf_handle h, uint64_t n_observed[2]) {
  if (!h->pair_fused) {
    uint64_t nb = 0;
    const int rc = tsdf_integrate_collect(h, &nb);
    if (rc) return rc;
    n_observed[0] = h->pair_first_observed, n_observed[1] = nb;
    h->last_observed = h->pair_first_observed + nb;
    h->last_changed_bytes += h->pair_first_changed;
    h->last_implied += h->pair_first_implied;
    h->last_read_bytes += h->pair_first_read;
    return TSDF_HIP_OK;
  }
  if (!h->count_slots) {
    tsdf_set_error("tsdf_integrate_collect2 without a counting launch");
    return TSDF_HIP_E_INVALID;
  }
  unsigned long long c[3072];
  TSDF_HIP_TRY(hipMemcpyAsync(c, h->counter, sizeof c, hipMemcpyDeviceToHost, h->stream));
  TSDF_HIP_TRY(hipStreamSynchronize(h->stream));
  unsigned long long sum[6] = {0, 0, 0, 0, 0, 0};
  for (int i = 0; i < 3072; ++i) sum[i >> 9] += c[i];
  n_observed[0] = sum[0], n_observed[1] = sum[1];
  h->last_observed = sum[2];
  h->last_changed_bytes = sum[3];
  h->last_implied = sum[4];
  h->last_read_bytes = sum[5];
  h->count_slots = 0;
  return TSDF_HIP_OK;
}

extern "C" int tsdf_hip_integrate_device2(tsdf_handle h, const float *d_depth_a, const uint32_t *d_bgra_a, const float cam_from_vol_a[12],
                                          const float *planes_a, const float *d_depth_b, const uint32_t *d_bgra_b,
                                          const float cam_from_vol_b[12], const float *planes_b, uint64_t *n_observed, int32_t *fused) {
  if (!h || !d_depth_a || !d_depth_b || !cam_from_vol_a || !cam_from_vol_b) return TSDF_HIP_E_INVALID;
  if (fused) *fused = 0;
  if (h->multi)
    return tsdf_multi_integrate_device2(h, d_depth_a, d_bgra_a, cam_from_vol_a, planes_a, d_depth_b, d_bgra_b, cam_from_vol_b, planes_b,
                                        n_observed, fused);
  TSDF_ENTER(h);
  bool f = false;
  const int rc = tsdf_integrate_launch2(h, d_depth_a, d_bgra_a, cam_from_vol_a, planes_a, d_depth_b, d_bgra_b, cam_from_vol_b, planes_b,
                                        n_observed != nullptr, &f);
  if (fused) *fused = f ? 1 : 0;
  if (rc || !n_observed) return rc;
  return tsdf_integrate_collect2(h, n_observed);
}

extern "C" int tsdf_hip_last_count_detail(tsdf_handle h, uint64_t out[2]) {
  if (!h || !out) return TSDF_HIP_E_INVALID;
  if (h->multi) return tsdf_multi_last_count_detail(h, out);
  out[0] = h->last_observed;
  out[1] = h->last_changed_bytes;
  return TSDF_HIP_OK;
}

extern "C" int tsdf_hip_last_read_detail(tsdf_handle h, uint64_t out[3]) {
  if (!h || !out) return TSDF_HIP_E_INVALID;
  if (h->multi) return tsdf_multi_last_read_detail(h, out);
  out[0] = h->last_implied;
  out[1] = h->last_implied_on ? 1 : 0;
  out[2] = h->last_read_bytes;
  return TSDF_HIP_OK;
}

extern "C" int tsdf_hip_set_reference_cull(tsdf_handle h, const float planes[24]) {
  if (!h) return TSDF_HIP_E_INVALID;
  if (h->multi) return tsdf_multi_set_reference_cull(h, planes);
  h->ref_cull = planes != nullptr;
  for (int i = 0; i < 24; ++i) h->cull_planes[i] = planes ? planes[i] : 0.f;
  return TSDF_HIP_OK;
}

extern "C" int tsdf_hip_last_launch_info(tsdf_handle h, int32_t out[4]) {
  if (!h || !out) return TSDF_HIP_E_INVALID;
  if (h->multi) h = tsdf_multi_first(h);
  for (int i = 0; i < 4; ++i) out[i] = h->last_launch[i];
  return TSDF_HIP_OK;
}

static int host_expf_fuses_r() {
  volatile float probe = -0x1.f8cbb2p+5f;
  return expf(probe) == 0x1.f45326p-92f ? 1 : 0;
}

static __global__ void k_expf(const float *__restrict__ in, float *__restrict__ out, size_t n, int fused_r) {
  const size_t i = (size_t)blockIdx.x * blockDim.x + threadIdx.x;
  if (i < n) out[i] = tsdf_expf_glibc(in[i], fused_r != 0);
}
static int device_expf(const float *in, size_t n, float *out, int fused_r) {
  float *di = nullptr, *dout = nullptr;
  TSDF_HIP_TRY(hipMalloc(&di, n * 4));
  TSDF_HIP_TRY(hipMalloc(&dout, n * 4));
  TSDF_HIP_TRY(hipMemcpy(di, in, n * 4, hipMemcpyHostToDevice));
  hipLaunchKernelGGL(k_expf, dim3((unsigned)((n + 255) / 256)), dim3(256), 0, 0, di, dout, n, fused_r);
  TSDF_HIP_TRY(hipGetLastError());
  TSDF_HIP_TRY(hipMemcpy(out, dout, n * 4, hipMemcpyDeviceToHost));
  (void)hipFree(di);
  (void)hipFree(dout);
  return TSDF_HIP_OK;
}

static int expf_matches_this_host(int fused_r) {
  static int verdict = -1;
  if (verdict >= 0) return verdict;
  const size_t n = 4096;
  std::vector<float> in(n), dev(n);
  uint32_t s = 0x9e3779b9u;
  for (size_t i = 0; i < n; ++i) {
    s = s * 1664525u + 1013904223u;
    const float u = (float)(s >> 8) * (1.0f / 16777216.0f);
    const float mag = ldexpf(1.0f + u, (int)(i % 34) - 26);
    in[i] = (i & 1) ? mag : -mag;
  }
  if (device_expf(in.data(), n, dev.data(), fused_r) != TSDF_HIP_OK) return -1;
  verdict = 1;
  for (size_t i = 0; i < n; ++i) {
    const volatile float x = in[i];
    const float want = expf(x);
    if (memcmp(&want, &dev[i], 4) != 0 && !(std::isnan(want) && std::isnan(dev[i]))) verdict = 0;
  }
  return verdict;
}

extern "C" int tsdf_hip_set_weighting(tsdf_handle h, int weight_by_depth, int weight_by_variance) {
  if (!h) return TSDF_HIP_E_INVALID;
  if (h->multi) return tsdf_multi_set_weighting(h, weight_by_depth, weight_by_variance);
  if (weight_by_depth && (h->packed || h->cn[0])) {
    tsdf_set_error("weight_by_depth makes weights non-integer: it needs the F32W layout (and TSDF_COLOR_RGB)");
    return TSDF_HIP_E_UNSUPPORTED;
  }
  if (weight_by_variance && (h->packed || h->cn[0])) {
    tsdf_set_error("weight_by_variance needs float weights and TSDF_COLOR_RGB: create / load the volume with TSDF_LAYOUT_F32W");
    return TSDF_HIP_E_UNSUPPORTED;
  }
  TSDF_ENTER(h);
  if (weight_by_variance && !h->vm) {
    const size_t n = (size_t)(h->pitch * h->ny * h->nz_alloc);
    TSDF_HIP_TRY(hipMalloc(&h->vm, n * sizeof(float)));
    TSDF_HIP_TRY(hipMalloc(&h->vn, n * sizeof(int32_t)));
    TSDF_HIP_TRY(hipMemsetAsync(h->vm, 0, n * sizeof(float), h->stream));
    TSDF_HIP_TRY(hipMemsetAsync(h->vn, 0, n * sizeof(int32_t), h->stream));
  }
  h->expf_fused_r = host_expf_fuses_r();
  if (weight_by_variance) {
    TSDF_ON_DEVICE(h->device);
    if (expf_matches_this_host(h->expf_fused_r) == 0) {
// ... 394 lines not shown
  CullArgs c;
  fill_camera(c, *p, cam_from_vol);
  c.nx = p->res[0], c.ny = p->res[1], c.z_global0 = 0;
  c.bx_vox = bx_vox, c.by_rows = by_rows;
  c.gx = (p->res[0] + bx_vox - 1) / bx_vox, c.gy = (p->res[1] + by_rows - 1) / by_rows, c.gz = p->res[2];
  for (int bz = 0; bz < c.gz; ++bz)
    for (int by = 0; by < c.gy; ++by)
      for (int bx = 0; bx < c.gx; ++bx) {
        const int xa = bx * c.bx_vox, xb = std::min(c.nx, xa + c.bx_vox) - 1;
        const int ya = by * c.by_rows, yb = std::min(c.ny, ya + c.by_rows) - 1;
        flags[((size_t)bz * c.gy + by) * c.gx + bx] =
            box_may_be_observed(c, ctr[0][xa], ctr[0][xb], ctr[1][ya], ctr[1][yb], ctr[2][bz]) ? 1 : 0;
      }
  return TSDF_HIP_OK;
}

extern "C" int tsdf_hip_selftest_row_intervals(const tsdf_params *p, const float cam_from_vol[12], const float *planes,
                                               uint32_t *words) {
  if (!p || !cam_from_vol || !words) return TSDF_HIP_E_INVALID;
  std::vector<float> ctr[3];
  int levels[3];
  if (!selftest_centers(*p, ctr, levels)) return TSDF_HIP_E_INVALID;
  if (p->res[0] > 0xfff0) return TSDF_HIP_E_UNSUPPORTED;
  RowArgs c;
  fill_camera(c, *p, cam_from_vol);
  c.nx = p->res[0], c.ny = p->res[1], c.nz = p->res[2], c.z_global0 = 0;
  c.rc = planes ? 1 : 0;
  for (int i = 0; i < 24; ++i) c.cull[i] = planes ? planes[i] : 0.f;
  for (int z = 0; z < c.nz; ++z)
    for (int y = 0; y < c.ny; ++y) words[(size_t)z * c.ny + y] = row_interval(c, ctr[0].data(), ctr[1][y], ctr[2][z]);
  return TSDF_HIP_OK;
}

extern "C" int tsdf_hip_selftest_sweep(tsdf_handle h, uint64_t *bytes_read, uint64_t *bytes_written) {
  if (!h) return TSDF_HIP_E_INVALID;
  TSDF_NOT_ON_MULTI(h, "tsdf_hip_selftest_sweep");
  TSDF_ENTER(h);
  const int64_t plane = h->pitch * h->ny;
  const int64_t first4 = (int64_t)(h->z_begin - h->z_first) * plane / 4;
  const int64_t n4 = (int64_t)(h->z_end - h->z_begin) * plane / 4;
  const unsigned grid = 256u * (unsigned)tsdf_tuning().blocks_per_cu;
  hipLaunchKernelGGL(k_calib_rmw, dim3(grid), dim3(256), 0, h->stream, h->d, h->w, h->rgb, h->k8, first4, n4, 0u);
  TSDF_HIP_TRY(hipGetLastError());
  TSDF_HIP_TRY(hipStreamSynchronize(h->stream));
  const uint64_t bytes_per_quad = 16u + (h->w ? 16u : 0u) + (h->rgb ? 16u : 0u) + (h->k8 ? 4u : 0u);
  if (bytes_read) *bytes_read = bytes_per_quad * (uint64_t)n4;
  if (bytes_written) *bytes_written = bytes_per_quad * (uint64_t)n4;
  return TSDF_HIP_OK;
}

static __global__ void k_selftest_div_count(const float *a, const uint32_t *k, float *out, unsigned char *fast, size_t n) {
  const size_t i = (size_t)blockIdx.x * blockDim.x + threadIdx.x;
  if (i >= n) return;
  const float b = (float)k[i];
  Rcp32 rs;
  rs.nb = -b;
  rs.y = rcp32_prepare(b).y;
  const float q = div32_fast(a[i], rs);
  const bool ok = __builtin_amdgcn_classf(q, 0x108);
  fast[i] = ok ? 1 : 0;
  out[i] = ok ? q : a[i] / b;
}

extern "C" int tsdf_hip_selftest_div_count(const float *a, const uint32_t *k, float *out, uint8_t *fast, size_t n) {
  if (!a || !k || !out || !fast || !n) return TSDF_HIP_E_INVALID;
  float *da = nullptr, *dout = nullptr;
  uint32_t *dk = nullptr;
  unsigned char *df = nullptr;
  TSDF_HIP_TRY(hipMalloc(&da, n * 4));
  TSDF_HIP_TRY(hipMalloc(&dk, n * 4));
  TSDF_HIP_TRY(hipMalloc(&dout, n * 4));
  TSDF_HIP_TRY(hipMalloc(&df, n));
  TSDF_HIP_TRY(hipMemcpy(da, a, n * 4, hipMemcpyHostToDevice));
  TSDF_HIP_TRY(hipMemcpy(dk, k, n * 4, hipMemcpyHostToDevice));
  hipLaunchKernelGGL(k_selftest_div_count, dim3((unsigned)((n + 255) / 256)), dim3(256), 0, 0, da, dk, dout, df, n);
  TSDF_HIP_TRY(hipGetLastError());
  TSDF_HIP_TRY(hipMemcpy(out, dout, n * 4, hipMemcpyDeviceToHost));
  TSDF_HIP_TRY(hipMemcpy(fast, df, n, hipMemcpyDeviceToHost));
  (void)hipFree(da);
  (void)hipFree(dk);
  (void)hipFree(dout);
  (void)hipFree(df);
  return TSDF_HIP_OK;
}

static __global__ void k_selftest_cvt_pk_u8(const float *in, uint32_t *out, size_t n) {
  const size_t i = (size_t)blockIdx.x * blockDim.x + threadIdx.x;
  if (i < n) out[i] = __builtin_amdgcn_cvt_pk_u8_f32(in[i], 1u, 0xAABBCCDDu);
}

extern "C" int tsdf_hip_selftest_cvt_pk_u8(const float *in, size_t n, uint32_t *out) {
  if (!in || !out || !n) return TSDF_HIP_E_INVALID;
  float *d_in = nullptr;
  uint32_t *d_out = nullptr;
  TSDF_HIP_TRY(hipMalloc(&d_in, n * 4));
  TSDF_HIP_TRY(hipMalloc(&d_out, n * 4));
  TSDF_HIP_TRY(hipMemcpy(d_in, in, n * 4, hipMemcpyHostToDevice));
  hipLaunchKernelGGL(k_selftest_cvt_pk_u8, dim3((unsigned)((n + 255) / 256)), dim3(256), 0, 0, d_in, d_out, n);
  TSDF_HIP_TRY(hipGetLastError());
  TSDF_HIP_TRY(hipMemcpy(out, d_out, n * 4, hipMemcpyDeviceToHost));
  (void)hipFree(d_in);
  (void)hipFree(d_out);
  return TSDF_HIP_OK;
}

static __global__ void k_selftest_lab2rgb(const float *lab, uint32_t *rgb, size_t n) {
  const size_t i = (size_t)blockIdx.x * blockDim.x + threadIdx.x;
  if (i < n) rgb[i] = lab_to_rgb(lab[3 * i], lab[3 * i + 1], lab[3 * i + 2]);
}

extern "C" int tsdf_hip_selftest_rgb2lab(const uint8_t *bgra, size_t n, float *lab4) {
  if (!bgra || !lab4 || !n || n > (size_t)1 << 30) return TSDF_HIP_E_INVALID;
  float lut[256];
  tsdf_lab_curve(lut);
  uint32_t *d_px = nullptr;
  float *d_lut = nullptr;
  float4 *d_lab = nullptr;
  TSDF_HIP_TRY(hipMalloc(&d_px, n * 4));
  TSDF_HIP_TRY(hipMalloc(&d_lut, sizeof lut));
  TSDF_HIP_TRY(hipMalloc(&d_lab, n * sizeof(float4)));
  TSDF_HIP_TRY(hipMemcpy(d_px, bgra, n * 4, hipMemcpyHostToDevice));
  TSDF_HIP_TRY(hipMemcpy(d_lut, lut, sizeof lut, hipMemcpyHostToDevice));
  hipLaunchKernelGGL(k_lab_image, dim3((unsigned)((n + 255) / 256)), dim3(256), 0, 0, d_px, d_lut, d_lab, (int)n);
  TSDF_HIP_TRY(hipGetLastError());
  TSDF_HIP_TRY(hipMemcpy(lab4, d_lab, n * sizeof(float4), hipMemcpyDeviceToHost));
  (void)hipFree(d_px);
  (void)hipFree(d_lut);
  (void)hipFree(d_lab);
  return TSDF_HIP_OK;
}

extern "C" int tsdf_hip_selftest_lab2rgb(const float *lab3, size_t n, uint32_t *rgb) {
  if (!lab3 || !rgb || !n) return TSDF_HIP_E_INVALID;
  float *d_lab = nullptr;
  uint32_t *d_rgb = nullptr;
  TSDF_HIP_TRY(hipMalloc(&d_lab, n * 12));
  TSDF_HIP_TRY(hipMalloc(&d_rgb, n * 4));
  TSDF_HIP_TRY(hipMemcpy(d_lab, lab3, n * 12, hipMemcpyHostToDevice));
  hipLaunchKernelGGL(k_selftest_lab2rgb, dim3((unsigned)((n + 255) / 256)), dim3(256), 0, 0, d_lab, d_rgb, n);
  TSDF_HIP_TRY(hipGetLastError());
  TSDF_HIP_TRY(hipMemcpy(rgb, d_rgb, n * 4, hipMemcpyDeviceToHost));
  (void)hipFree(d_lab);
  (void)hipFree(d_rgb);
  return TSDF_HIP_OK;
}

static __global__ void k_selftest_struct_oob(const float *img, int W, int H, unsigned soff, const int *uv, unsigned *out, int n) {
  const int i = blockIdx.x * blockDim.x + threadIdx.x;
  if (i >= n) return;
  const i4_rsrc r = make_rsrc_2d(img, (unsigned)W * 4u, (unsigned)H);
  out[i] = tsdf_struct_buffer_load_u32(r, uv[2 * i + 1], uv[2 * i] * 4, (int)soff, 0);
}

extern "C" int tsdf_hip_selftest_struct_oob(const float *img, int W, int H, int planes, int plane, const int32_t *uv, uint32_t *out,
                                            int n) {
  if (!img || !uv || !out || n <= 0 || W <= 0 || H <= 0 || planes < 1 || plane < 0 || plane >= planes) return TSDF_HIP_E_INVALID;
  float *d_img = nullptr;
  int *d_uv = nullptr;
  unsigned *d_out = nullptr;
  const size_t npx = (size_t)W * H;
  TSDF_HIP_TRY(hipMalloc(&d_img, npx * 4 * planes));
  TSDF_HIP_TRY(hipMalloc(&d_uv, (size_t)n * 8));
  TSDF_HIP_TRY(hipMalloc(&d_out, (size_t)n * 4));
  TSDF_HIP_TRY(hipMemcpy(d_img, img, npx * 4 * planes, hipMemcpyHostToDevice));
  TSDF_HIP_TRY(hipMemcpy(d_uv, uv, (size_t)n * 8, hipMemcpyHostToDevice));
  hipLaunchKernelGGL(k_selftest_struct_oob, dim3((unsigned)((n + 255) / 256)), dim3(256), 0, 0, d_img, W, H,
                     (unsigned)(npx * 4 * plane), d_uv, d_out, n);
  TSDF_HIP_TRY(hipGetLastError());
  TSDF_HIP_TRY(hipMemcpy(out, d_out, (size_t)n * 4, hipMemcpyDeviceToHost));
  (void)hipFree(d_img);
  (void)hipFree(d_uv);
  (void)hipFree(d_out);
  return TSDF_HIP_OK;
}

static __global__ void k_selftest_project(const IntegrateArgs a, const double *cam, const float *g, size_t n, int *pix_fast,
                                          int *pix_exact, unsigned char *ambiguous) {
  const size_t i = (size_t)blockIdx.x * blockDim.x + threadIdx.x;
  if (i >= n) return;
  const float gx = g[3 * i], gy = g[3 * i + 1], gz = g[3 * i + 2];
  bool amb = false;
  int pf = project_fast(a, gx, gy, gz, amb);
  const int pe = project_exact(a, cam, gx, gy, gz);
  if (amb) pf = pe;
  pix_fast[i] = pf;
  pix_exact[i] = pe;
  ambiguous[i] = amb ? 1 : 0;
}

extern "C" int tsdf_hip_selftest_project(tsdf_handle h, const float *g, size_t n, int32_t *pix_fast,
                                         int32_t *pix_exact, uint8_t *ambiguous) {
  if (!h || !g || !n || !pix_fast || !pix_exact || !ambiguous) return TSDF_HIP_E_INVALID;
  if (h->multi) h = tsdf_multi_first(h);
  TSDF_ENTER(h);
  const float ident[12] = {1, 0, 0, 0, 0, 1, 0, 0, 0, 0, 1, 0};
  const IntegrateHost a = make_args(h, ident);
  if (!fast_projection_ok(a, true, true)) {
    tsdf_set_error("fast projection disabled for this camera");
    return TSDF_HIP_E_UNSUPPORTED;
  }
  float *dg = nullptr;
  int *dpf = nullptr, *dpe = nullptr;
  unsigned char *da = nullptr;
  TSDF_HIP_TRY(hipMalloc(&dg, n * 12));
  TSDF_HIP_TRY(hipMalloc(&dpf, n * 4));
  TSDF_HIP_TRY(hipMalloc(&dpe, n * 4));
  TSDF_HIP_TRY(hipMalloc(&da, n));
  TSDF_HIP_TRY(hipMemcpy(dg, g, n * 12, hipMemcpyHostToDevice));
  hipLaunchKernelGGL(k_selftest_project, dim3((unsigned)((n + 255) / 256)), dim3(256), 0, 0, a.a, h->cam64, dg, n, dpf, dpe, da);
  TSDF_HIP_TRY(hipGetLastError());
  TSDF_HIP_TRY(hipMemcpy(pix_fast, dpf, n * 4, hipMemcpyDeviceToHost));
  TSDF_HIP_TRY(hipMemcpy(pix_exact, dpe, n * 4, hipMemcpyDeviceToHost));
  TSDF_HIP_TRY(hipMemcpy(ambiguous, da, n, hipMemcpyDeviceToHost));
  (void)hipFree(dg);
  (void)hipFree(dpf);
  (void)hipFree(dpe);
  (void)hipFree(da);
  return TSDF_HIP_OK;
}
#endif
```

Measured before the change: 660,500.

## Interleave depth and colour into per-pixel records for single 64-bit gathers

Adds a small pre-pass kernel that packs each frame's depth and BGRA planes into interleaved 8-byte pixel records. The colour integration kernels (single, pipelined and fused pair) then fetch depth and colour with one 64-bit struct buffer load instead of two separate 32-bit gathers into distant planes. This is meant to halve the number of scattered frame gathers per voxel and keep both values in one cache line. In exchange it adds an extra launch and a full-frame read and write per frame, plus extra device buffers. It only takes effect when colour integration is on.

```diff
diff --git a/cpu_tsdf_amd/csrc/tsdf_buffer.h b/cpu_tsdf_amd/csrc/tsdf_buffer.h
--- a/cpu_tsdf_amd/csrc/tsdf_buffer.h
+++ b/cpu_tsdf_amd/csrc/tsdf_buffer.h
@@ -36,6 +36,13 @@
 __device__ unsigned tsdf_struct_buffer_load_u32(i4_rsrc rsrc, int vindex, int voffset, int soffset, int aux)
     __asm("llvm.amdgcn.struct.buffer.load.i32");
 
+typedef unsigned u2 __attribute__((ext_vector_type(2)));
+__device__ u2 tsdf_struct_buffer_load_u32x2(i4_rsrc rsrc, int vindex, int voffset, int soffset, int aux)
+    __asm("llvm.amdgcn.struct.buffer.load.v2i32");
+static __device__ __forceinline__ u2 bload64(rsrc_t r, unsigned voff, unsigned soff) {
+  return __builtin_amdgcn_raw_buffer_load_b64(r, (int)voff, (int)soff, 0);
+}
+
 static __device__ __forceinline__ i4_rsrc make_rsrc_2d(const void *p, unsigned row_bytes, unsigned rows) {
   const unsigned long long a = (unsigned long long)p;
   i4_rsrc r;
diff --git a/cpu_tsdf_amd/csrc/tsdf_common.h b/cpu_tsdf_amd/csrc/tsdf_common.h
--- a/cpu_tsdf_amd/csrc/tsdf_common.h
+++ b/cpu_tsdf_amd/csrc/tsdf_common.h
@@ -43,6 +43,7 @@
   std::vector<float> h_ctr[3];
   float *frame_depth = nullptr;
   uint32_t *frame_bgra = nullptr;
+  uint2 *frame_pairs[2] = {nullptr, nullptr};
   char *bounce = nullptr;
   hipEvent_t bounce_ev[2] = {nullptr, nullptr};
   bool bounce_busy[2] = {false, false};
@@ -289,6 +290,7 @@
   int implied_d;
   int pipe;
   int lab_chunk;
+  int frame_pairs;
 };
 const TsdfTuning &tsdf_tuning();
 int tsdf_vol_chunk();
diff --git a/cpu_tsdf_amd/csrc/tsdf_core.hip b/cpu_tsdf_amd/csrc/tsdf_core.hip
--- a/cpu_tsdf_amd/csrc/tsdf_core.hip
+++ b/cpu_tsdf_amd/csrc/tsdf_core.hip
@@ -54,7 +54,7 @@
                          env_int("TSDF_HIP_CULL", 1), std::max(1, env_int("TSDF_HIP_VOL_CHUNK", 256)),
                          env_int("TSDF_HIP_PLAIN_KERNEL", 0), env_int("TSDF_HIP_ALLOC_TRIES", 3), env_int("TSDF_HIP_ALLIN", 1),
                          env_int("TSDF_HIP_REFCULL_PLAIN", 0), env_int("TSDF_HIP_LIVE_LOG2TX", 5), env_int("TSDF_HIP_ZFAST", 1), env_int("TSDF_HIP_FUSE2", 1), env_int("TSDF_HIP_IMPLIED_D", 1),
-                         env_int("TSDF_HIP_PIPE", 1), std::max(1, env_int("TSDF_HIP_LAB_CHUNK", 16 << 20))};
+                         env_int("TSDF_HIP_PIPE", 1), std::max(1, env_int("TSDF_HIP_LAB_CHUNK", 16 << 20)), env_int("TSDF_HIP_FRAME_PAIRS", 1)};
   return t;
 }
 
@@ -104,6 +104,8 @@
     t.zfast = value;
   else if (n == "lab_chunk")
     t.lab_chunk = std::max(1, value);
+  else if (n == "frame_pairs")
+    t.frame_pairs = value;
   else
     return TSDF_HIP_E_INVALID;
   return TSDF_HIP_OK;
@@ -386,6 +388,8 @@
   for (int a = 0; a < 3; ++a)
     if (v->ctr[a]) (void)hipFree(v->ctr[a]);
   if (v->frame_depth) (void)hipFree(v->frame_depth);
+  for (int i = 0; i < 2; ++i)
+    if (v->frame_pairs[i]) (void)hipFree(v->frame_pairs[i]);
   if (v->bounce) (void)hipHostFree(v->bounce);
   for (int i = 0; i < 2; ++i)
     if (v->bounce_ev[i]) (void)hipEventDestroy(v->bounce_ev[i]);
@@ -649,6 +653,8 @@
   const size_t npx = (size_t)p->image_width * p->image_height;
   TRY_OR_BAIL(hipMalloc(&v->frame_depth, 2 * npx * sizeof(float)));
   v->frame_bgra = reinterpret_cast<uint32_t *>(v->frame_depth + npx);
+  if (p->integrate_color)
+    for (int i = 0; i < 2; ++i) TRY_OR_BAIL(hipMalloc(&v->frame_pairs[i], 8 * npx));
   {
     const double cam[4] = {p->fx, p->fy, p->cx, p->cy};
     TRY_OR_BAIL(hipMalloc(&v->cam64, sizeof cam));
diff --git a/cpu_tsdf_amd/csrc/tsdf_integrate.hip b/cpu_tsdf_amd/csrc/tsdf_integrate.hip
--- a/cpu_tsdf_amd/csrc/tsdf_integrate.hip
+++ b/cpu_tsdf_amd/csrc/tsdf_integrate.hip
@@ -307,7 +307,7 @@
 #define TSDF_BAND_STEP 64
 #define TSDF_WPE_OF(ORDER, COLOR, FASTPROJ, COUNT, PACKED, ALLIN) \
   ((ALLIN) && !(COUNT) && (PACKED) && (COLOR) && (FASTPROJ) ? TSDF_WPE_PACKED_COLOR : (ALLIN) && !(COUNT) && ((PACKED) || !(COLOR)) ? TSDF_WPE_PACKED : TSDF_WPE_GENERAL)
-template <int ORDER, bool COLOR, bool FASTPROJ, bool COUNT, bool PACKED, bool ALLIN = false, bool LIVE = false>
+template <int ORDER, bool COLOR, bool FASTPROJ, bool COUNT, bool PACKED, bool ALLIN = false, bool LIVE = false, bool PAIRS = false>
 static __global__ void __launch_bounds__(256) __attribute__((amdgpu_waves_per_eu(TSDF_WPE_OF(ORDER, COLOR, FASTPROJ, COUNT, PACKED, ALLIN) < TSDF_WPE_MAX ? TSDF_WPE_OF(ORDER, COLOR, FASTPROJ, COUNT, PACKED, ALLIN) : TSDF_WPE_MAX, TSDF_WPE_MAX)))
 k_integrate(const IntegrateArgs a, float *__restrict__ D, float *__restrict__ Wt, uint32_t *__restrict__ RGB,
             uint8_t *__restrict__ K8, const float *__restrict__ depth, const double *__restrict__ cam,
@@ -315,6 +315,7 @@
             unsigned long long *__restrict__ n_obs, const uint8_t *__restrict__ live, uint8_t *__restrict__ band,
             const uint32_t *__restrict__ row_iv) {
   static_assert(!(ALLIN && LIVE), "the ALLIN instance knows no row intervals");
+  static_assert(!PAIRS || COLOR, "pixel records carry the colour: the colourless frame is the depth plane itself");
   const BlockCoords bc = tsdf_block_coords(a.zfast);
   bool strad = false;
   if (LIVE) {
@@ -369,8 +370,8 @@
   const rsrc_t rsC = make_rsrc(COLOR ? RGB + e0 : (uint32_t *)D, COLOR ? span * 4u : 0u);
   const rsrc_t rsK = make_rsrc(PACKED && !COLOR ? K8 + e0 : (uint8_t *)D, PACKED && !COLOR ? span : 0u);
   const unsigned npix = (unsigned)a.W * (unsigned)a.H;
-  const rsrc_t rsF = make_rsrc(depth, COLOR ? a.bgra_off + npix * 4u : npix * 4u);
-  const i4_rsrc rsFi = make_rsrc_2d(depth, 4u, 0xffffffffu);
+  const rsrc_t rsF = make_rsrc(depth, PAIRS ? npix * 8u : COLOR ? a.bgra_off + npix * 4u : npix * 4u);
+  const i4_rsrc rsFi = make_rsrc_2d(depth, PAIRS ? 8u : 4u, 0xffffffffu);
   if (xq < a.qpr) {
     const int x4 = xq * 4;
     const float cz = ctrz[a.z_global0 + zl];
@@ -470,7 +471,10 @@
       uint32_t cs[4] = {0u, 0u, 0u, 0u};
 #pragma unroll
       for (int j = 0; j < 4; ++j) {
-        if (ALLIN) {
+        if (PAIRS) {
+          const u2 zc = ALLIN ? tsdf_struct_buffer_load_u32x2(rsFi, pix[j], 0, 0, TSDF_GATHER_AUX) : bload64(rsF, (unsigned)pix[j] << 3, 0u);
+          zs[j] = __uint_as_float(zc.x), cs[j] = zc.y;
+        } else if (ALLIN) {
           zs[j] = __uint_as_float(tsdf_struct_buffer_load_u32(rsFi, pix[j], 0, 0, TSDF_GATHER_AUX));
           if (COLOR) cs[j] = tsdf_struct_buffer_load_u32(rsFi, pix[j], 0, (int)a.bgra_off, TSDF_GATHER_AUX);
         } else {
@@ -906,7 +910,7 @@
   u4 d4;
 };
 
-template <int ORDER, bool COUNT>
+template <int ORDER, bool COUNT, bool PAIRS>
 static __global__ void __launch_bounds__(256) __attribute__((amdgpu_waves_per_eu(TSDF_WPE_PIPEC < TSDF_WPE_MAX ? TSDF_WPE_PIPEC : TSDF_WPE_MAX, TSDF_WPE_MAX)))
 k_integrate_pc(const IntegrateArgs a, float *__restrict__ D, uint32_t *__restrict__ RGB, const float *__restrict__ depth,
                const double *__restrict__ cam, const float *__restrict__ ctrx, const float *__restrict__ ctry,
@@ -946,7 +950,7 @@
   const unsigned span = (unsigned)rows * (unsigned)a.pitch;
   const rsrc_t rsD = make_rsrc(D + e0, span * 4u);
   const rsrc_t rsC = make_rsrc(RGB + e0, span * 4u);
-  const i4_rsrc rsFi = make_rsrc_2d(depth, 4u, 0xffffffffu);
+  const i4_rsrc rsFi = make_rsrc_2d(depth, PAIRS ? 8u : 4u, 0xffffffffu);
   const uint32_t pbits = __float_as_uint(a.pos_over_neg);
   if (xq < a.qpr) {
     const int x4 = xq * 4;
@@ -970,8 +974,13 @@
       R.c4 = bload128(rsC, offp, soff);
 #pragma unroll
       for (int j = 0; j < 4; ++j) {
-        R.z[j] = tsdf_struct_buffer_load_u32(rsFi, pix[j], 0, 0, TSDF_GATHER_AUX);
-        R.cs[j] = tsdf_struct_buffer_load_u32(rsFi, pix[j], 0, (int)a.bgra_off, TSDF_GATHER_AUX);
+        if (PAIRS) {
+          const u2 zc = tsdf_struct_buffer_load_u32x2(rsFi, pix[j], 0, 0, TSDF_GATHER_AUX);
+          R.z[j] = zc.x, R.cs[j] = zc.y;
+        } else {
+          R.z[j] = tsdf_struct_buffer_load_u32(rsFi, pix[j], 0, 0, TSDF_GATHER_AUX);
+          R.cs[j] = tsdf_struct_buffer_load_u32(rsFi, pix[j], 0, (int)a.bgra_off, TSDF_GATHER_AUX);
+        }
       }
       if (COUNT) rdb += pred ? (d_read ? 32u : 16u) : 0u;
     };
@@ -1142,7 +1151,7 @@
   unsigned bgra_off;
 };
 
-template <int ORDER, bool COLOR, bool COUNT>
+template <int ORDER, bool COLOR, bool COUNT, bool PAIRS>
 static __global__ void __launch_bounds__(256) __attribute__((amdgpu_waves_per_eu(TSDF_WPE_K2, TSDF_WPE_MAX)))
 k_integrate2(const IntegrateArgs a, const Frame2 fb, float *__restrict__ D, uint32_t *__restrict__ RGB, uint8_t *__restrict__ K8,
              const float *__restrict__ depthA, const float *__restrict__ depthB, const double *__restrict__ cam,
@@ -1182,7 +1191,9 @@
   const rsrc_t rsD = make_rsrc(D + e0, span * 4u);
   const rsrc_t rsC = make_rsrc(COLOR ? RGB + e0 : (uint32_t *)D, COLOR ? span * 4u : 0u);
   const rsrc_t rsK = make_rsrc(!COLOR ? K8 + e0 : (uint8_t *)D, !COLOR ? span : 0u);
-  const i4_rsrc rsFA = make_rsrc_2d(depthA, 4u, 0xffffffffu), rsFB = make_rsrc_2d(depthB, 4u, 0xffffffffu);
+  static_assert(!PAIRS || COLOR, "pixel records carry the colour");
+  const unsigned fstride = PAIRS ? 8u : 4u;
+  const i4_rsrc rsFA = make_rsrc_2d(depthA, fstride, 0xffffffffu), rsFB = make_rsrc_2d(depthB, fstride, 0xffffffffu);
   const uint32_t hinge_bits = __float_as_uint(a.pos_over_neg);
   if (xq < a.qpr) {
     const int x4 = xq * 4;
@@ -1206,13 +1217,23 @@
       project_quad_allin<ORDER>(a, fb.m, cam, s_cx[tid], s_ytB[ty + r * a.TY], ztB, pixB, L.gzB);
 #pragma unroll
       for (int j = 0; j < 4; ++j) {
-        L.zsA[j] = __uint_as_float(tsdf_struct_buffer_load_u32(rsFA, pixA[j], 0, 0, TSDF_GATHER_AUX));
-        L.csA[j] = COLOR ? tsdf_struct_buffer_load_u32(rsFA, pixA[j], 0, (int)a.bgra_off, TSDF_GATHER_AUX) : 0u;
+        if (PAIRS) {
+          const u2 zc = tsdf_struct_buffer_load_u32x2(rsFA, pixA[j], 0, 0, TSDF_GATHER_AUX);
+          L.zsA[j] = __uint_as_float(zc.x), L.csA[j] = zc.y;
+        } else {
+          L.zsA[j] = __uint_as_float(tsdf_struct_buffer_load_u32(rsFA, pixA[j], 0, 0, TSDF_GATHER_AUX));
+          L.csA[j] = COLOR ? tsdf_struct_buffer_load_u32(rsFA, pixA[j], 0, (int)a.bgra_off, TSDF_GATHER_AUX) : 0u;
+        }
       }
 #pragma unroll
       for (int j = 0; j < 4; ++j) {
-        L.zsB[j] = __uint_as_float(tsdf_struct_buffer_load_u32(rsFB, pixB[j], 0, 0, TSDF_GATHER_AUX));
-        L.csB[j] = COLOR ? tsdf_struct_buffer_load_u32(rsFB, pixB[j], 0, (int)fb.bgra_off, TSDF_GATHER_AUX) : 0u;
+        if (PAIRS) {
+          const u2 zc = tsdf_struct_buffer_load_u32x2(rsFB, pixB[j], 0, 0, TSDF_GATHER_AUX);
+          L.zsB[j] = __uint_as_float(zc.x), L.csB[j] = zc.y;
+        } else {
+          L.zsB[j] = __uint_as_float(tsdf_struct_buffer_load_u32(rsFB, pixB[j], 0, 0, TSDF_GATHER_AUX));
+          L.csB[j] = COLOR ? tsdf_struct_buffer_load_u32(rsFB, pixB[j], 0, (int)fb.bgra_off, TSDF_GATHER_AUX) : 0u;
+        }
       }
       L.d4 = bload128(rsD, voff, soff);
       L.c4 = (u4){0u, 0u, 0u, 0u};
@@ -2033,6 +2054,11 @@
   return true;
 }
 
+static bool frame_is_planar(const tsdf_params &p, const float *d_depth, const uint32_t *d_bgra) {
+  unsigned off;
+  return frame_bgra_offset(p, d_depth, d_bgra, &off);
+}
+
 static int stage_frame(tsdf_handle h, const float **d_depth, const uint32_t *d_bgra, unsigned *bgra_off) {
   if (frame_bgra_offset(h->p, *d_depth, d_bgra, bgra_off)) return TSDF_HIP_OK;
   const size_t npx = (size_t)h->p.image_width * h->p.image_height;
@@ -2045,6 +2071,31 @@
   *bgra_off = (unsigned)(npx * 4);
   return TSDF_HIP_OK;
 }
+
+static __global__ void __launch_bounds__(256)
+k_frame_pairs(const uint32_t *__restrict__ depth, const uint32_t *__restrict__ bgra, uint2 *__restrict__ out, unsigned npix) {
+  const unsigned i = (blockIdx.x * 256u + threadIdx.x) * 2u;
+  if (i + 1u < npix) {
+    const uint4 v = {depth[i], bgra[i], depth[i + 1u], bgra[i + 1u]};
+    *reinterpret_cast<uint4 *>(out + i) = v;
+  } else if (i < npix) {
+    out[i] = make_uint2(depth[i], bgra[i]);
+  }
+}
+
+static int launch_frame_pairs(tsdf_handle h, const float *d_depth, const uint32_t *d_bgra, uint2 *out) {
+  const unsigned npix = (unsigned)h->p.image_width * (unsigned)h->p.image_height;
+  if (!out || !d_depth || !d_bgra) {
+    tsdf_set_error("colour launch without its pixel-record buffer or frame");
+    return TSDF_HIP_E_INVALID;
+  }
+  hipLaunchKernelGGL(k_frame_pairs, dim3((npix + 511u) / 512u), dim3(256), 0, h->stream, reinterpret_cast<const uint32_t *>(d_depth),
+                     d_bgra, out, npix);
+  TSDF_HIP_TRY(hipGetLastError());
+  return TSDF_HIP_OK;
+}
+
+static bool frame_pairs_apply(tsdf_handle h) { return tsdf_tuning().frame_pairs && h->p.integrate_color; }
 
 static int zfast_for(const tsdf_params &p, unsigned gx) {
   const size_t frame_bytes = (size_t)p.image_width * p.image_height * (p.integrate_color ? 8 : 4);
@@ -2252,31 +2303,32 @@
 }
 
 static void dispatch_fast(tsdf_handle h, const LaunchPlan &pl, const float *d_depth, bool count, bool fastproj, bool allin,
-                          bool pipe, uint8_t *band_arg) {
+                          bool pipe, bool pairs, uint8_t *band_arg) {
   const IntegrateArgs &a = pl.a;
   const dim3 grid(a.zfast ? pl.gz : pl.gx, pl.gy, a.zfast ? pl.gx : pl.gz), block(256);
   const bool sse = h->p.xform_order == TSDF_XFORM_PCL_SSE, color = h->p.integrate_color != 0;
+  pairs = pairs && color;
   if (pipe) {
     with_consts(
-        [&](auto SSE, auto COUNT) {
+        [&](auto SSE, auto COUNT, auto PAIRS) {
           if (color)
-            hipLaunchKernelGGL((k_integrate_pc<xform_order_of(SSE), COUNT>), grid, block, 0, h->stream, a, pl.D, pl.RGB, d_depth,
+            hipLaunchKernelGGL((k_integrate_pc<xform_order_of(SSE), COUNT, PAIRS>), grid, block, 0, h->stream, a, pl.D, pl.RGB, d_depth,
                                h->cam64, pl.ctrx, pl.ctry, h->ctr[2], h->counter, band_arg);
-          else
+          else if constexpr (!PAIRS)
             hipLaunchKernelGGL((k_integrate_p<xform_order_of(SSE), COUNT>), grid, block, 0, h->stream, a, pl.D, pl.K8, d_depth,
                                h->cam64, pl.ctrx, pl.ctry, h->ctr[2], h->counter, band_arg);
         },
-        sse, count);
+        sse, count, pairs);
     return;
   }
   with_consts(
-      [&](auto SSE, auto COLOR, auto FASTPROJ, auto COUNT, auto PACKED, auto ALLIN, auto LIVE) {
-        if constexpr (!(ALLIN && (!FASTPROJ || LIVE)))
-          hipLaunchKernelGGL((k_integrate<xform_order_of(SSE), COLOR, FASTPROJ, COUNT, PACKED, ALLIN, LIVE>), grid, block, 0,
+      [&](auto SSE, auto COLOR, auto FASTPROJ, auto COUNT, auto PACKED, auto ALLIN, auto LIVE, auto PAIRS) {
+        if constexpr (!(ALLIN && (!FASTPROJ || LIVE)) && !(PAIRS && !COLOR))
+          hipLaunchKernelGGL((k_integrate<xform_order_of(SSE), COLOR, FASTPROJ, COUNT, PACKED, ALLIN, LIVE, PAIRS>), grid, block, 0,
                              h->stream, a, pl.D, pl.Wt, pl.RGB, pl.K8, d_depth, h->cam64, pl.ctrx, pl.ctry, h->ctr[2], h->counter,
                              pl.live, band_arg, h->row_iv);
       },
-      sse, color, fastproj, count, h->packed, allin, pl.live != nullptr);
+      sse, color, fastproj, count, h->packed, allin, pl.live != nullptr, pairs);
 }
 
 static int validate_launch(tsdf_handle h, const LaunchPlan &pl, const uint32_t *d_bgra) {
@@ -2310,7 +2362,13 @@
     h->band_exact = false;
     return launch_plain_family(h, a, pl.gz, plain_mode, d_depth, d_bgra, T, count);
   }
-  if (const int e = stage_frame(h, &d_depth, d_bgra, &a.bgra_off)) return e;
+  const bool pairs = frame_pairs_apply(h);
+  if (pairs) {
+    if (!frame_is_planar(h->p, d_depth, d_bgra)) h->frame_staged = 0;
+    a.bgra_off = 0;
+  } else if (const int e = stage_frame(h, &d_depth, d_bgra, &a.bgra_off)) {
+    return e;
+  }
   const LaunchKind kind = launch_kind(h, T, a, rc, rc_rows);
   if (kind.live)
     if (const int e = plan_live(h, T, kind.all_inside, rc_rows, pl)) return e;
@@ -2329,7 +2387,11 @@
     h->last_launch[1] = fastproj;
     h->last_launch[2] = live ? (rc_rows ? 2 : 1) : 0;
     h->last_launch[3] = (int)std::min<uint64_t>((uint64_t)pl.gx * pl.gy * pl.gz, 0x7fffffffu);
-    dispatch_fast(h, pl, d_depth, count, fastproj, allin, pipe, band_arg);
+    if (pairs) {
+      if (const int e = launch_frame_pairs(h, d_depth, d_bgra, h->frame_pairs[0])) return e;
+      d_depth = reinterpret_cast<const float *>(h->frame_pairs[0]);
+    }
+    dispatch_fast(h, pl, d_depth, count, fastproj, allin, pipe, pairs, band_arg);
     TSDF_HIP_TRY(hipGetLastError());
   }
   h->count_slots = count ? 4096 : 0;
@@ -2390,11 +2452,13 @@
   IntegrateArgs &a = pl.a;
   Frame2 fb;
   for (int i = 0; i < 12; ++i) fb.m[i] = TB[i];
+  const bool pairs = frame_pairs_apply(h);
+  a.bgra_off = fb.bgra_off = 0;
   const bool pipe_wins = !color && tsdf_tuning().fuse2 == 1 && pipelined_rows_apply(h, a, color, true, true, false);
   const bool ok = tsdf_tuning().fuse2 && !pipe_wins && tsdf_tuning().cull == 1 && tsdf_tuning().allin && h->packed && !h->cn[0] && !h->weight_by_depth &&
                   !h->weight_by_variance && !tsdf_tuning().plain_kernel && (h->nx & 3) == 0 && a.wmax_is_int && (float)h->kmax == p.max_weight &&
-                  pl.gy <= 65535u && pl.gz <= 65535u && pl.gz > 0 && frame_bgra_offset(p, dA, cA, &a.bgra_off) &&
-                  frame_bgra_offset(p, dB, cB, &fb.bgra_off) && fusable_pose(h, hh, TA, planesA) && fusable_pose(h, hh, TB, planesB);
+                  pl.gy <= 65535u && pl.gz <= 65535u && pl.gz > 0 &&
+                  (pairs || (frame_bgra_offset(p, dA, cA, &a.bgra_off) && frame_bgra_offset(p, dB, cB, &fb.bgra_off))) && fusable_pose(h, hh, TA, planesA) && fusable_pose(h, hh, TB, planesB);
   if (fused) *fused = ok;
   if (!ok) {
     int rc = tsdf_hip_set_reference_cull(h, planesA);
@@ -2423,12 +2487,19 @@
   h->last_launch[3] = (int)std::min<uint64_t>((uint64_t)pl.gx * pl.gy * pl.gz, 0x7fffffffu);
   a.zfast = zfast_for(p, pl.gx);
   const dim3 grid(a.zfast ? pl.gz : pl.gx, pl.gy, a.zfast ? pl.gx : pl.gz), block(256);
+  if (pairs) {
+    if (!frame_is_planar(p, dA, cA) || !frame_is_planar(p, dB, cB)) h->frame_staged = 0;
+    if (const int e = launch_frame_pairs(h, dA, cA, h->frame_pairs[0])) return e;
+    if (const int e = launch_frame_pairs(h, dB, cB, h->frame_pairs[1])) return e;
+    dA = reinterpret_cast<const float *>(h->frame_pairs[0]), dB = reinterpret_cast<const float *>(h->frame_pairs[1]);
+  }
   with_consts(
-      [&](auto SSE, auto COLOR, auto COUNT) {
-        hipLaunchKernelGGL((k_integrate2<xform_order_of(SSE), COLOR, COUNT>), grid, block, 0, h->stream, a, fb, h->d, h->rgb, h->k8,
-                           dA, dB, h->cam64, h->ctr[0], h->ctr[1], h->ctr[2], h->counter, band_arg);
+      [&](auto SSE, auto COLOR, auto COUNT, auto PAIRS) {
+        if constexpr (!(PAIRS && !COLOR))
+          hipLaunchKernelGGL((k_integrate2<xform_order_of(SSE), COLOR, COUNT, PAIRS>), grid, block, 0, h->stream, a, fb, h->d, h->rgb, h->k8,
+                             dA, dB, h->cam64, h->ctr[0], h->ctr[1], h->ctr[2], h->counter, band_arg);
       },
-      p.xform_order == TSDF_XFORM_PCL_SSE, color, count);
+      p.xform_order == TSDF_XFORM_PCL_SSE, color, count, pairs);
   TSDF_HIP_TRY(hipGetLastError());
   h->count_slots = count ? 3072 : 0;
   h->count_ran = true;
@@ -3129,9 +3200,61 @@
   out[i] = tsdf_struct_buffer_load_u32(r, uv[2 * i + 1], uv[2 * i] * 4, (int)soff, 0);
 }
 
+static __global__ void k_selftest_record_gather(const uint2 *rec, int W, int H, const int *uv, unsigned *out, int n) {
+  const int i = blockIdx.x * blockDim.x + threadIdx.x;
+  if (i >= n) return;
+  const int u = uv[2 * i], v = uv[2 * i + 1];
+  const int pix = (unsigned)u < (unsigned)W && (unsigned)v < (unsigned)H ? v * W + u : -1;
+  const rsrc_t rs = make_rsrc(rec, (unsigned)W * (unsigned)H * 8u);
+  const u2 zc = bload64(rs, (unsigned)pix << 3, 0u);
+  out[2 * i] = zc.x, out[2 * i + 1] = zc.y;
+}
+
+static int selftest_record_gather(const float *img, int W, int H, const int32_t *uv, uint32_t *out, int n) {
+  const size_t npx = (size_t)W * H;
+  if (npx > (size_t)1 << 24) return TSDF_HIP_E_INVALID;
+  struct DeviceBuffers {
+    void *p[4] = {nullptr, nullptr, nullptr, nullptr};
+    ~DeviceBuffers() {
+      for (void *q : p)
+        if (q) (void)hipFree(q);
+    }
+  } buf;
+  TSDF_HIP_TRY(hipMalloc(&buf.p[0], npx * 8));
+  TSDF_HIP_TRY(hipMalloc(&buf.p[1], (npx + 2) * 8));
+  TSDF_HIP_TRY(hipMalloc(&buf.p[2], (size_t)n * 8));
+  TSDF_HIP_TRY(hipMalloc(&buf.p[3], (size_t)n * 8));
+  uint32_t *d_img = static_cast<uint32_t *>(buf.p[0]);
+  uint2 *d_rec = static_cast<uint2 *>(buf.p[1]);
+  int *d_uv = static_cast<int *>(buf.p[2]);
+  unsigned *d_out = static_cast<unsigned *>(buf.p[3]);
+  TSDF_HIP_TRY(hipMemcpy(d_img, img, npx * 8, hipMemcpyHostToDevice));
+  TSDF_HIP_TRY(hipMemcpy(d_uv, uv, (size_t)n * 8, hipMemcpyHostToDevice));
+  TSDF_HIP_TRY(hipMemset(d_rec, 0xa5, (npx + 2) * 8));
+  hipLaunchKernelGGL(k_frame_pairs, dim3((unsigned)((npx + 511) / 512)), dim3(256), 0, 0, d_img, d_img + npx, d_rec, (unsigned)npx);
+  hipLaunchKernelGGL(k_selftest_record_gather, dim3((unsigned)((n + 255) / 256)), dim3(256), 0, 0, d_rec, W, H, d_uv, d_out, n);
+  TSDF_HIP_TRY(hipGetLastError());
+  TSDF_HIP_TRY(hipMemcpy(out, d_out, (size_t)n * 8, hipMemcpyDeviceToHost));
+  uint32_t guard[4] = {0, 0, 0, 0};
+  TSDF_HIP_TRY(hipMemcpy(guard, d_rec + npx, sizeof guard, hipMemcpyDeviceToHost));
+  std::vector<uint32_t> after(2 * npx);
+  TSDF_HIP_TRY(hipMemcpy(after.data(), d_img, npx * 8, hipMemcpyDeviceToHost));
+  if (guard[0] != 0xa5a5a5a5u || guard[1] != 0xa5a5a5a5u || guard[2] != 0xa5a5a5a5u || guard[3] != 0xa5a5a5a5u) {
+    tsdf_set_error("k_frame_pairs wrote behind the last record");
+    return TSDF_HIP_E_HIP;
+  }
+  if (memcmp(after.data(), img, npx * 8) != 0) {
+    tsdf_set_error("k_frame_pairs changed the images it read");
+    return TSDF_HIP_E_HIP;
+  }
+  return TSDF_HIP_OK;
+}
+
 extern "C" int tsdf_hip_selftest_struct_oob(const float *img, int W, int H, int planes, int plane, const int32_t *uv, uint32_t *out,
                                             int n) {
-  if (!img || !uv || !out || n <= 0 || W <= 0 || H <= 0 || planes < 1 || plane < 0 || plane >= planes) return TSDF_HIP_E_INVALID;
+  const bool records = planes == 2 && plane == -1;
+  if (!img || !uv || !out || n <= 0 || W <= 0 || H <= 0 || planes < 1 || (!records && (plane < 0 || plane >= planes))) return TSDF_HIP_E_INVALID;
+  if (records) return selftest_record_gather(img, W, H, uv, out, n);
   float *d_img = nullptr;
   int *d_uv = nullptr;
   unsigned *d_out = nullptr;
```

Measured after the change: 697,000 (median of 6 runs). 5.5% higher.
